# TomasDelaney/A-Deep-Reinforcement-Learning-Enabled-Soft-Exoskeleton-for-Parkinson-s-Patients

Measured on AMD Instinct MI355X. Metric: env steps/sec (batched exo sim) + TD7 grad-steps/sec at 1/2/4/8 MI355X, higher is better.
Workload: dtype f64 sim + bf16 TD7

## Files before the change

### a-deep-reinforcement-learning-enabled-soft-exoskeleton-for-parkinson-s-patients_amd/csrc/lap.hip

```cpp
#include <hip/hip_runtime.h>

#include <algorithm>
#include <cstdint>
#include <cstdlib>
#include <string>

#include "lap_chain.h"
#include "philox.h"
#include "exo_amd.h"

namespace {

constexpr int UPD_THREADS = 1024;

__device__ __forceinline__ float *stratum_tree(float *tree, int s, int cap) { return tree + (size_t)s * 2 * cap; }

constexpr int TOPN = 8192;
template <int NTOP = TOPN>
__device__ bool propagate_top(float *T, int cap, int levels, const int32_t *slot, int n, float *top) {
    int lv = 1;
    for (; lv <= levels && ((2 * cap) >> lv) > NTOP / 2; ++lv) {
        __syncthreads();
        for (int k = threadIdx.x; k < n; k += blockDim.x) {
            const int node = (cap + slot[k]) >> lv;
            T[node] = T[2 * node] + T[2 * node + 1];
        }
    }
    __syncthreads();
    if (lv > levels) return false;
    const int lim = min(NTOP, 2 * cap);
    if (blockDim.x == UPD_THREADS) {
        constexpr int PER = NTOP / UPD_THREADS;
        float v[PER];
#pragma unroll
        for (int j = 0; j < PER; ++j) {
            const int i = threadIdx.x + j * UPD_THREADS;
            v[j] = i < lim ? T[i] : 0.0f;
        }
#pragma unroll
        for (int j = 0; j < PER; ++j) {
            const int i = threadIdx.x + j * UPD_THREADS;
            if (i < lim) top[i] = v[j];
        }
    } else {
        for (int i = threadIdx.x; i < lim; i += blockDim.x) top[i] = T[i];
    }
    for (; lv <= levels; ++lv) {
        __syncthreads();
        for (int k = threadIdx.x; k < n; k += blockDim.x) {
            const int node = (cap + slot[k]) >> lv;
            top[node] = top[2 * node] + top[2 * node + 1];
        }
    }
    __syncthreads();
    const int wb = min(NTOP / 2, cap);
    for (int i = 1 + threadIdx.x; i < wb; i += blockDim.x) T[i] = top[i];
    __syncthreads();
    return true;
}
__device__ void propagate(float *T, int cap, int levels, const int32_t *slot, int n) {
    __shared__ float top[TOPN];
    propagate_top(T, cap, levels, slot, n, top);
}

__device__ void propagate_span(float *T, int cap, int levels, int capacity, int first, int count) {
    __shared__ float top[TOPN];
    if (count <= 0) return;
    int a0 = first, e0 = first + count, a1 = 0, e1 = 0;
    if (count >= capacity) {
        a0 = 0;
        e0 = capacity;
    } else if (e0 > capacity) {
        e1 = e0 - capacity;
        e0 = capacity;
    }
    int lv = 1;
    for (; lv <= levels && ((2 * cap) >> lv) > TOPN / 2; ++lv) {
        __syncthreads();
        const int lo0 = (cap + a0) >> lv, n0 = ((cap + e0 - 1) >> lv) - lo0 + 1;
        const int lo1 = (cap + a1) >> lv, n1 = e1 > a1 ? ((cap + e1 - 1) >> lv) - lo1 + 1 : 0;
        for (int k = threadIdx.x; k < n0 + n1; k += blockDim.x) {
            const int node = k < n0 ? lo0 + k : lo1 + k - n0;
            T[node] = T[2 * node] + T[2 * node + 1];
        }
    }
    __syncthreads();
    if (lv > levels) return;
    const int lim = min(TOPN, 2 * cap);
    for (int i = threadIdx.x; i < lim; i += blockDim.x) top[i] = T[i];
    for (; lv <= levels; ++lv) {
        __syncthreads();
        const int lo0 = (cap + a0) >> lv, n0 = ((cap + e0 - 1) >> lv) - lo0 + 1;
        const int lo1 = (cap + a1) >> lv, n1 = e1 > a1 ? ((cap + e1 - 1) >> lv) - lo1 + 1 : 0;
        for (int k = threadIdx.x; k < n0 + n1; k += blockDim.x) {
            const int node = k < n0 ? lo0 + k : lo1 + k - n0;
            top[node] = top[2 * node] + top[2 * node + 1];
        }
    }
    __syncthreads();
    const int wb = min(TOPN / 2, cap);
    for (int i = 1 + threadIdx.x; i < wb; i += blockDim.x) T[i] = top[i];
    __syncthreads();
}

constexpr int SPAN_LDS = 4096;
constexpr int SPAN_LEVELS = 32;
__device__ bool propagate_span_lds(float *T, int cap, int levels, int capacity, int first, int count,
                                   float *buf , float *edge ) {
    const int a = cap + first, e = cap + first + count - 1;
    if (count <= 0 || first + count > capacity || count > SPAN_LDS - 2 || levels >= SPAN_LEVELS) return false;
    const int t = threadIdx.x;
    if (t < 2 * levels) {
        const int lv = t >> 1, right = t & 1;
        const int lo = a >> lv, hi = e >> lv;
        if (!right && (lo & 1)) edge[t] = T[lo - 1];
        if (right && !(hi & 1)) edge[t] = T[hi + 1];
    }
    float *A = buf, *B = buf + SPAN_LDS;
    {
        const int base = a & ~1;
        for (int c = a + t; c <= e; c += blockDim.x) A[c - base] = T[c];
    }
    __syncthreads();
    if (t == 0) {
        if (a & 1) A[0] = edge[0];
        if (!(e & 1)) A[(e | 1) - (a & ~1)] = edge[1];
    }
    for (int lv = 1; lv <= levels; ++lv) {
        __syncthreads();
        const int lo = a >> lv, hi = e >> lv, cbase = (a >> (lv - 1)) & ~1, nbase = lo & ~1;
        for (int node = lo + t; node <= hi; node += blockDim.x) {
            const int c = 2 * node - cbase;
            const float v = A[c] + A[c + 1];
            T[node] = v;
            B[node - nbase] = v;
        }
        if (t == 0 && lv < levels) {
            if (lo & 1) B[0] = edge[2 * lv];
            if (!(hi & 1)) B[(hi | 1) - nbase] = edge[2 * lv + 1];
        }
        float *tmp = A;
        A = B;
        B = tmp;
    }
    __syncthreads();
    return true;
}

constexpr int ADD_CHUNK = 4096;
__global__ __launch_bounds__(UPD_THREADS) void lap_add_kernel(float *tree, const float *maxp, int cap, int levels,
                                                              int capacity, const int32_t *stratum,
                                                              const int32_t *slot, int n) {
    const int s = blockIdx.x;
    float *T = stratum_tree(tree, s, cap);
    __shared__ int32_t mine[ADD_CHUNK];
    __shared__ int count;
    const float p = *maxp;
    for (int base = 0; base < n; base += ADD_CHUNK) {
        if (threadIdx.x == 0) count = 0;
        __syncthreads();
        const int end = min(n, base + ADD_CHUNK);
        for (int k = base + threadIdx.x; k < end; k += blockDim.x) {
            if (stratum[k] != s) continue;
            const int sl = slot[k];
            if (sl < 0 || sl >= capacity) continue;
            T[cap + sl] = p;
            mine[atomicAdd(&count, 1)] = sl;
        }
        __syncthreads();
        propagate(T, cap, levels, mine, count);
    }
}

constexpr int MAXLV = 24;
template <class At>
__device__ __forceinline__ float prefix_sum(At at, int cap, int levels, int sz) {
    if (sz >= cap) return at(1);
    float v[MAXLV];
#pragma unroll
    for (int j = 0; j < MAXLV; ++j) {
        v[j] = 0.0f;
        if (j < levels) {
            const int lv = levels - 1 - j;
            const float x = at(2 * ((1 << j) | (sz >> (lv + 1))));
            v[j] = ((sz >> lv) & 1) ? x : 0.0f;
        }
    }
    float acc = 0.0f;
#pragma unroll
    for (int j = 0; j < MAXLV; ++j)
        if (j < levels) acc += v[j];
    return acc;
}
__device__ __forceinline__ float prefix_total(const float *T, int cap, int levels, int sz) {
    return prefix_sum([T](int n) { return T[n]; }, cap, levels, sz);
}

__device__ __forceinline__ float sel4(int r, float a, float b, float c, float d) {
    return r == 0 ? a : r == 1 ? b : r == 2 ? c : d;
}

template <class At>
__device__ __forceinline__ int descend_from(At at, float val, int node, int lv, int levels) {
    while (lv < levels) {
        const int k = levels - lv >= 3 ? 3 : levels - lv;
        const int n1 = 2 * node, n2 = 4 * node, n3 = 8 * node;
        const float a0 = at(n1), a1 = at(n1 + 1);
        float b0 = 0.f, b1 = 0.f, b2 = 0.f, b3 = 0.f, c0 = 0.f, c1 = 0.f, c2 = 0.f, c3 = 0.f;
        float c4 = 0.f, c5 = 0.f, c6 = 0.f, c7 = 0.f;
        if (k >= 2) b0 = at(n2), b1 = at(n2 + 1), b2 = at(n2 + 2), b3 = at(n2 + 3);
        if (k >= 3) {
            c0 = at(n3), c1 = at(n3 + 1), c2 = at(n3 + 2), c3 = at(n3 + 3);
            c4 = at(n3 + 4), c5 = at(n3 + 5), c6 = at(n3 + 6), c7 = at(n3 + 7);
        }
        int r;
        if (val <= a0 || a1 <= 0.0f) {
            r = 0;
        } else {
            val -= a0;
            r = 1;
        }
        if (k >= 2) {
            const float l = r ? b2 : b0, rt = r ? b3 : b1;
            if (val <= l || rt <= 0.0f) {
                r = 2 * r;
            } else {
                val -= l;
                r = 2 * r + 1;
            }
            if (k >= 3) {
                const float l3 = sel4(r, c0, c2, c4, c6), r3 = sel4(r, c1, c3, c5, c7);
                if (val <= l3 || r3 <= 0.0f) {
                    r = 2 * r;
                } else {
                    val -= l3;
                    r = 2 * r + 1;
                }
            }
        }
        node = (node << k) + r;
        lv += k;
    }
    return node;
}

__global__ void lap_sample_kernel(const float *tree, int cap, int levels, const float *u, const int32_t *size,
                                  int batch, int32_t *idx) {
    const int s = blockIdx.y;
    const int b = blockIdx.x * blockDim.x + threadIdx.x;
    if (b >= batch) return;
    const float *T = tree + (size_t)s * 2 * cap;
    const int sz = size[s];
    const float val = u[(size_t)s * batch + b] * prefix_total(T, cap, levels, sz);
    const int node = descend_from([T](int n) { return T[n]; }, val, 1, 0, levels);
    int i = node - cap;
    if (i >= sz) i = sz > 0 ? sz - 1 : 0;
    idx[(size_t)s * batch + b] = i;
}

__global__ __launch_bounds__(UPD_THREADS) void lap_update_kernel(float *tree, float *maxp, int cap, int levels,
                                                                 const int32_t *idx, const float *prio,
                                                                 int batch) {
    const int s = blockIdx.x;
    float *T = stratum_tree(tree, s, cap);
    const int32_t *I = idx + (size_t)s * batch;
    const float *P = prio + (size_t)s * batch;
    __shared__ float red[UPD_THREADS / 64];
    __shared__ int32_t li[UPD_THREADS];
    float mx = 0.0f;
    for (int b0 = 0; b0 < batch; b0 += UPD_THREADS) {
        const int nb = min(UPD_THREADS, batch - b0);
        __syncthreads();
        if ((int)threadIdx.x < nb) li[threadIdx.x] = I[b0 + threadIdx.x];
        __syncthreads();
        const int b = b0 + threadIdx.x;
        if (b < batch) {
            const int me = li[threadIdx.x];
            bool last = true;
            for (int k = threadIdx.x + 1; k < nb; ++k) last &= (li[k] != me);
            for (int b2 = b0 + nb; b2 < batch; ++b2) last &= (I[b2] != me);
            if (last) T[cap + me] = P[b];
            mx = fmaxf(mx, P[b]);
        }
    }
    for (int o = 32; o > 0; o >>= 1) mx = fmaxf(mx, __shfl_xor(mx, o, 64));
    if ((threadIdx.x & 63) == 0) red[threadIdx.x >> 6] = mx;
    propagate(T, cap, levels, I, batch);
    if (threadIdx.x == 0) {
        for (int w = 1; w < (int)(blockDim.x >> 6); ++w) mx = fmaxf(mx, red[w]);
        atomicMax(reinterpret_cast<int *>(maxp), __float_as_int(mx));
    }
}

__global__ void lap_reset_max_kernel(const float *tree, float *maxp, int cap, int n_strata) {
    __shared__ float red[16];
    float mx = 0.0f;
    const size_t total = (size_t)n_strata * cap;
    for (size_t k = (size_t)blockIdx.x * blockDim.x + threadIdx.x; k < total; k += (size_t)gridDim.x * blockDim.x) {
        const size_t s = k / cap, i = k % cap;
        mx = fmaxf(mx, tree[s * 2 * cap + cap + i]);
    }
    for (int o = 32; o > 0; o >>= 1) mx = fmaxf(mx, __shfl_xor(mx, o, 64));
    if ((threadIdx.x & 63) == 0) red[threadIdx.x >> 6] = mx;
    __syncthreads();
    if (threadIdx.x == 0) {
        for (int w = 1; w < (int)(blockDim.x >> 6); ++w) mx = fmaxf(mx, red[w]);
        atomicMax(reinterpret_cast<int *>(maxp), __float_as_int(mx));
    }
}

__global__ void lap_totals_kernel(const float *tree, int cap, int n_strata, float *out) {
    const int s = blockIdx.x * blockDim.x + threadIdx.x;
    if (s < n_strata) out[s] = tree[(size_t)s * 2 * cap + 1];
}

__global__ void lap_init_kernel(float *maxp) { *maxp = 1.0f; }


constexpr int STORE_CHUNK = UPD_THREADS * 4;

template <int RANK_RPT>
__global__ __launch_bounds__(UPD_THREADS) void lap_store_rank_kernel(float *tree, const float *maxp, int cap,
                                                                     int levels, int capacity, int32_t *ring_ptr,
                                                                     int32_t *ring_size, const int32_t *strata,
                                                                     const uint8_t *active, int n, int32_t *row_of) {
    const int s = blockIdx.x, t = threadIdx.x, lane = t & 63, wv = t >> 6;
    float *T = stratum_tree(tree, s, cap);
    __shared__ int wsum[UPD_THREADS / 64];
    __shared__ int chunk_total;
    const float p = *maxp;
    const int ptr0 = ring_ptr[s];
    const int row0 = s * (capacity + 1);
    int offset = 0;
    for (int base = 0; base < n; base += RANK_RPT * UPD_THREADS) {
        int st[RANK_RPT], cnt = 0;
        bool f[RANK_RPT];
#pragma unroll
        for (int k = 0; k < RANK_RPT; ++k) {
            const int i = base + RANK_RPT * t + k;
            st[k] = i < n ? strata[i] : -1;
            f[k] = i < n && (!active || active[i]);
        }
#pragma unroll
        for (int k = 0; k < RANK_RPT; ++k) {
            f[k] = f[k] && st[k] == s;
            cnt += f[k];
        }
        int incl = cnt;
#pragma unroll
        for (int o = 1; o < 64; o <<= 1) {
            const int v = __shfl_up(incl, o, 64);
            if (lane >= o) incl += v;
        }
        if (lane == 63) wsum[wv] = incl;
        __syncthreads();
        if (t == 0) {
            int acc = 0;
            for (int k = 0; k < UPD_THREADS / 64; ++k) {
                const int v = wsum[k];
                wsum[k] = acc;
                acc += v;
            }
            chunk_total = acc;
        }
        __syncthreads();
        int rank = offset + wsum[wv] + incl - cnt;
#pragma unroll
        for (int k = 0; k < RANK_RPT; ++k) {
            const int i = base + RANK_RPT * t + k;
            if (i >= n) continue;
            if (s == 0 && (st[k] < 0 || st[k] >= (int)gridDim.x)) row_of[i] = -1;
            if (st[k] != s) continue;
            if (f[k]) {
                const int slot = (ptr0 + rank) % capacity;
                row_of[i] = row0 + slot;
                T[cap + slot] = p;
                ++rank;
            } else {
                row_of[i] = row0 + capacity;
            }
        }
        const int total = chunk_total;
        __syncthreads();
        offset += total;
    }
    propagate_span(T, cap, levels, capacity, ptr0, offset);
    if (t == 0) {
        ring_ptr[s] = (ptr0 + offset) % capacity;
        ring_size[s] = min(ring_size[s] + offset, capacity);
    }
}

__device__ __forceinline__ long long mult_below(long long x, int E) { return (x + E - 1) / E; }

__global__ __launch_bounds__(UPD_THREADS) void lap_store_ref_slots_kernel(int capacity, int E, long long *ref,
                                                                          int32_t *ring_size,
                                                                          const int32_t *strata,
                                                                          const uint8_t *active, int n,
                                                                          int32_t *rank_row, int32_t *slot_of,
                                                                          int32_t *row_of) {
    const int t = threadIdx.x, lane = t & 63, wv = t >> 6;
    __shared__ int wsum[UPD_THREADS / 64];
    __shared__ int chunk_total;
    const long long ptr0 = ref[0], count0 = ref[1], size0 = ref[2];
    const long long m0 = mult_below(count0, E);
    int offset = 0;
    for (int base = 0; base < n; base += STORE_CHUNK) {
        int f[4], cnt = 0;
#pragma unroll
        for (int k = 0; k < 4; ++k) {
            const int i = base + 4 * t + k;
            f[k] = (i < n && strata[i] >= 0 && strata[i] < E && (!active || active[i])) ? 1 : 0;
            cnt += f[k];
        }
        int incl = cnt;
#pragma unroll
        for (int o = 1; o < 64; o <<= 1) {
            const int v = __shfl_up(incl, o, 64);
            if (lane >= o) incl += v;
        }
        if (lane == 63) wsum[wv] = incl;
        __syncthreads();
        if (t == 0) {
            int acc = 0;
            for (int k = 0; k < UPD_THREADS / 64; ++k) {
                const int v = wsum[k];
                wsum[k] = acc;
                acc += v;
            }
            chunk_total = acc;
        }
        __syncthreads();
        int rank = offset + wsum[wv] + incl - cnt;
#pragma unroll
        for (int k = 0; k < 4; ++k) {
            const int i = base + 4 * t + k;
            if (i >= n) continue;
            if (f[k]) {
                rank_row[rank] = strata[i];
                row_of[i] = rank;
                ++rank;
            } else {
                row_of[i] = -1;
                slot_of[i] = -1;
            }
        }
        offset += chunk_total;
        __syncthreads();
    }
    __threadfence_block();
    __syncthreads();
    const int n_act = offset;
    for (int i = t; i < n; i += blockDim.x) {
        const int r = row_of[i];
        if (r < 0) continue;
        const long long mr = mult_below(count0 + r, E);
        const int s = strata[i];
        bool win = true;
        const long long qend = mr * E - count0;
        const int qmax = (int)min((long long)min(r + E, n_act) - 1, qend);
        for (int q = r + 1; q <= qmax; ++q) win &= rank_row[q] != s;
        long long v = ptr0 + (mr - m0);
        if (v >= capacity) v -= capacity;
        if (v >= capacity) v %= capacity;
        const int slot = (int)v;
        slot_of[i] = win ? slot : -1;
        row_of[i] = win ? s * (capacity + 1) + slot : -1;
    }
    __syncthreads();
    const long long adv = mult_below(count0 + n_act, E) - m0;
    const long long size = min(size0 + adv, (long long)capacity);
    for (int s = t; s < E; s += blockDim.x) ring_size[s] = (int32_t)size;
    if (t == 0) {
        ref[0] = (ptr0 + adv) % capacity;
        ref[1] = count0 + n_act;
        ref[2] = size;
    }
}

__device__ __forceinline__ float4 ld4(const float *p) { return *reinterpret_cast<const float4 *>(p); }
__device__ __forceinline__ void st4(float *p, float4 v) { *reinterpret_cast<float4 *>(p) = v; }

template <bool VEC>
__device__ __forceinline__ void copy_rows(const lap_storage_desc &st, const float *state, const float *action,
                                          const float *next_state, const float *reward, const uint8_t *done,
                                          float action_scale, const int32_t *ri, const int32_t *sl, int s,
                                          int capacity, int j0, int step, int m, int t, int nt) {
    const int sd = st.state_dim, ad = st.action_dim;
    const int sdv = VEC ? sd / 4 : sd;
    const int per = 2 * sdv + ad + 2;
    const int nrows = j0 < m ? (m - j0 + step - 1) / step : 0;
    const int items = nrows * per;
    constexpr int U = 4;
    for (int it0 = t; it0 < items; it0 += U * nt) {
        float4 v[U];
        long dst[U];
        int kind[U];
#pragma unroll
        for (int u = 0; u < U; ++u) {
            const int it = it0 + u * nt;
            kind[u] = -1;
            if (it >= items) continue;
            const int q = it / per, c = it - q * per, j = j0 + q * step;
            const int slot = sl[j];
            if (slot < 0) continue;
            const long r = (long)s * (capacity + 1) + slot;
            const long i = ri[j];
            if (c < 2 * sdv) {
                const bool nx = c >= sdv;
                const int e = nx ? c - sdv : c;
                const float *src = (nx ? next_state : state) + i * sd;
                if (VEC) {
                    v[u] = ld4(src + 4 * e);
                    dst[u] = r * sd + 4 * e;
                } else {
                    v[u].x = src[e];
                    dst[u] = r * sd + e;
                }
                kind[u] = nx ? 1 : 0;
            } else if (c < 2 * sdv + ad) {
                const int e = c - 2 * sdv;
                v[u].x = action[i * ad + e] / action_scale;
                dst[u] = r * ad + e;
                kind[u] = 2;
            } else if (c == 2 * sdv + ad) {
                v[u].x = reward[i];
                dst[u] = r;
                kind[u] = 3;
            } else {
                v[u].x = 1.0f - (done[i] ? 1.0f : 0.0f);
                dst[u] = r;
                kind[u] = 4;
            }
        }
#pragma unroll
        for (int u = 0; u < U; ++u) {
            switch (kind[u]) {
            case 0:
                if (VEC) st4(st.state + dst[u], v[u]); else st.state[dst[u]] = v[u].x;
                break;
            case 1:
                if (VEC) st4(st.next_state + dst[u], v[u]); else st.next_state[dst[u]] = v[u].x;
                break;
            case 2: st.action[dst[u]] = v[u].x; break;
            case 3: st.reward[dst[u]] = v[u].x; break;
            case 4: st.not_done[dst[u]] = v[u].x; break;
            default: break;
            }
        }
    }
}

constexpr int STORE_FUSED_MAX = 8192;

template <bool VEC>
__global__ __launch_bounds__(UPD_THREADS) void lap_store_fused_kernel(
    float *tree, const float *maxp, int cap, int levels, int capacity, int32_t *ring_ptr, int32_t *ring_size,
    const int32_t *strata, const uint8_t *active, int n, int32_t *row_of, lap_storage_desc st, const float *state,
    const float *action, const float *next_state, const float *reward, const uint8_t *done, float action_scale) {
    constexpr int RPT = 4;
    const int s = blockIdx.x, t = threadIdx.x, lane = t & 63, wv = t >> 6;
    float *T = stratum_tree(tree, s, cap);
    __shared__ int wsum[UPD_THREADS / 64];
    __shared__ int chunk_total;
    __shared__ int32_t ri[STORE_FUSED_MAX];
    const float p = *maxp;
    const int ptr0 = ring_ptr[s];
    const int row0 = s * (capacity + 1);
    int offset = 0;
    for (int base = 0; base < n; base += RPT * UPD_THREADS) {
        int stk[RPT], cnt = 0;
        bool f[RPT];
#pragma unroll
        for (int k = 0; k < RPT; ++k) {
            const int i = base + RPT * t + k;
            stk[k] = i < n ? strata[i] : -1;
            f[k] = i < n && (!active || active[i]) && stk[k] == s;
            cnt += f[k];
        }
        int incl = cnt;
#pragma unroll
        for (int o = 1; o < 64; o <<= 1) {
            const int v = __shfl_up(incl, o, 64);
            if (lane >= o) incl += v;
        }
        if (lane == 63) wsum[wv] = incl;
        __syncthreads();
        if (t == 0) {
            int acc = 0;
            for (int k = 0; k < UPD_THREADS / 64; ++k) {
                const int v = wsum[k];
                wsum[k] = acc;
                acc += v;
            }
            chunk_total = acc;
        }
        __syncthreads();
        int rank = offset + wsum[wv] + incl - cnt;
#pragma unroll
        for (int k = 0; k < RPT; ++k) {
            const int i = base + RPT * t + k;
            if (i >= n) continue;
            if (s == 0 && (stk[k] < 0 || stk[k] >= (int)gridDim.x)) row_of[i] = -1;
            if (stk[k] != s) continue;
            if (f[k]) {
                const int slot = (ptr0 + rank) % capacity;
                row_of[i] = row0 + slot;
                T[cap + slot] = p;
                ri[rank] = i;
                ++rank;
            } else {
                row_of[i] = row0 + capacity;
            }
        }
        const int total = chunk_total;
        __syncthreads();
        offset += total;
    }
    {
        const int sd = st.state_dim, ad = st.action_dim;
        const int sdv = VEC ? sd / 4 : sd;
        const int per = 2 * sdv + ad + 2;
        const int items = offset * per;
        constexpr int U = 8;
        for (int it0 = t; it0 < items; it0 += U * UPD_THREADS) {
            float4 v[U];
            long dst[U];
            int kind[U];
#pragma unroll
            for (int u = 0; u < U; ++u) {
                const int it = it0 + u * UPD_THREADS;
                kind[u] = -1;
                if (it >= items) continue;
                const int q = it / per, c = it - q * per;
                const long r = (long)row0 + (ptr0 + q) % capacity;
                const long i = ri[q];
                if (c < 2 * sdv) {
                    const bool nx = c >= sdv;
                    const int e = nx ? c - sdv : c;
                    const float *src = (nx ? next_state : state) + i * sd;
                    if (VEC) {
                        v[u] = ld4(src + 4 * e);
                        dst[u] = r * sd + 4 * e;
                    } else {
                        v[u].x = src[e];
                        dst[u] = r * sd + e;
                    }
                    kind[u] = nx ? 1 : 0;
                } else if (c < 2 * sdv + ad) {
                    const int e = c - 2 * sdv;
                    v[u].x = action[i * ad + e] / action_scale;
                    dst[u] = r * ad + e;
                    kind[u] = 2;
                } else if (c == 2 * sdv + ad) {
                    v[u].x = reward[i];
                    dst[u] = r;
                    kind[u] = 3;
                } else {
                    v[u].x = 1.0f - (done[i] ? 1.0f : 0.0f);
                    dst[u] = r;
                    kind[u] = 4;
                }
            }
#pragma unroll
            for (int u = 0; u < U; ++u) {
                switch (kind[u]) {
                case 0:
                    if (VEC) st4(st.state + dst[u], v[u]); else st.state[dst[u]] = v[u].x;
                    break;
                case 1:
                    if (VEC) st4(st.next_state + dst[u], v[u]); else st.next_state[dst[u]] = v[u].x;
                    break;
                case 2: st.action[dst[u]] = v[u].x; break;
                case 3: st.reward[dst[u]] = v[u].x; break;
                case 4: st.not_done[dst[u]] = v[u].x; break;
                default: break;
                }
            }
        }
    }
    propagate_span(T, cap, levels, capacity, ptr0, offset);
    if (t == 0) {
        ring_ptr[s] = (ptr0 + offset) % capacity;
        ring_size[s] = min(ring_size[s] + offset, capacity);
    }
}

struct MaskAdvance {
    const uint8_t *table;
    int rows;
    long long *k;
    uint8_t *active;
    int32_t *count;
// ... 317 lines not shown
    const long long i = (long long)blockIdx.x * blockDim.x + threadIdx.x;
    if (i >= entries) return;
    const int c = plan[i];
    if (c < 0) return;
    const long long ptr0 = ref[0], count0 = ref[1];
    const long long m0 = mult_below(count0, E), mr = mult_below(count0 + c, E);
    const long long qend = min(mr * E - count0, total - 1);
    const int s = add_s[c];
    bool win = true;
    for (long long q = c + 1; q <= qend; ++q) win &= add_s[q] != s;
    long long v = ptr0 + (mr - m0);
    if (v >= capacity) v -= capacity;
    if (v >= capacity) v %= capacity;
    plan[i] = win ? (int32_t)v : -1;
}

__global__ __launch_bounds__(256) void lap_ref_step_kernel(lap_storage_desc st, const int32_t *plan, int rows, int n,
                                                           long long *kk, int par, long long *k_dev,
                                                           const int32_t *strata, int capacity, const float *state,
                                                           const float *action, const float *next_state,
                                                           const float *reward, const uint8_t *done,
                                                           float action_scale, const uint8_t *table,
                                                           uint8_t *active, int32_t *count,
                                                           const int32_t *counts_table, double *score) {
    const long long k = kk[par];
    const long long k1 = k + 1 < rows ? k + 1 : rows - 1;
    const int e = blockIdx.x * 4 + (threadIdx.x >> 6), lane = threadIdx.x & 63;
    if (blockIdx.x == 0 && threadIdx.x == 0) {
        kk[par ^ 1] = k1;
        if (k_dev) *k_dev = k1;
        if (count) *count = counts_table[k1];
    }
    if (e >= n) return;
    const int slot = k < rows ? plan[(size_t)k * n + e] : -1;
    if (slot >= 0) {
        const long r = (long)strata[e] * (capacity + 1) + slot;
        const int sd = st.state_dim, ad = st.action_dim;
        for (int q = lane; q < sd; q += 64) {
            st.state[r * sd + q] = state[(long)e * sd + q];
            st.next_state[r * sd + q] = next_state[(long)e * sd + q];
        }
        for (int q = lane; q < ad; q += 64) st.action[r * ad + q] = action[(long)e * ad + q] / action_scale;
        if (lane == 0) {
            st.reward[r] = reward[e];
            st.not_done[r] = 1.0f - (done[e] ? 1.0f : 0.0f);
        }
    }
    if (lane == 0) {
        if (score) score[e] += active[e] ? (double)reward[e] : 0.0;
        active[e] = table[(size_t)k1 * n + e];
    }
}

__global__ __launch_bounds__(256) void lap_ref_commit_leaves_kernel(const int32_t *plan, long long entries, int n,
                                                                    const int32_t *strata, float *tree, int cap,
                                                                    const float *maxp) {
    const long long i = (long long)blockIdx.x * blockDim.x + threadIdx.x;
    if (i >= entries) return;
    const int slot = plan[i];
    if (slot < 0) return;
    stratum_tree(tree, strata[i % n], cap)[cap + slot] = *maxp;
}

__global__ __launch_bounds__(UPD_THREADS) void lap_ref_commit_tree_kernel(float *tree, int cap, int levels,
                                                                          int capacity, const long long *ref,
                                                                          long long total, int E) {
    const long long ptr0 = ref[0], count0 = ref[1];
    if (total <= 0) return;
    const long long last = mult_below(count0 + total - 1, E) - mult_below(count0, E);
    propagate_span(stratum_tree(tree, blockIdx.x, cap), cap, levels, capacity, (int)ptr0,
                   (int)min(last + 1, (long long)capacity));
}

__global__ void lap_ref_commit_ref_kernel(long long *ref, long long total, int E, int capacity, int32_t *ring_size) {
    const long long ptr0 = ref[0], count0 = ref[1], size0 = ref[2];
    const long long adv = mult_below(count0 + total, E) - mult_below(count0, E);
    const long long size = min(size0 + adv, (long long)capacity);
    for (int s = 0; s < E; ++s) ring_size[s] = (int32_t)size;
    ref[0] = (ptr0 + adv) % capacity;
    ref[1] = count0 + total;
    ref[2] = size;
}

constexpr int GATHER_DRAWS = 16;
__global__ __launch_bounds__(256) void lap_gather_kernel(lap_storage_desc st, int capacity, const int32_t *idx,
                                                         int batch, int total, float *o_state, float *o_action,
                                                         float *o_next, float *o_reward, float *o_not_done) {
    const int sd = st.state_dim, ad = st.action_dim;
    const bool v4 = (sd & 3) == 0 && ((reinterpret_cast<uintptr_t>(st.state) | reinterpret_cast<uintptr_t>(st.next_state) |
                                       reinterpret_cast<uintptr_t>(o_state) | reinterpret_cast<uintptr_t>(o_next)) & 15) == 0;
    const int sv = v4 ? sd / 4 : sd, per = 2 * sv + ad + 2;
    const int d0 = blockIdx.x * GATHER_DRAWS;
    const int nd = min(GATHER_DRAWS, total - d0);
    const int items = nd * per;
    constexpr int GU = 4;
    for (int it0 = threadIdx.x; it0 < items; it0 += GU * 256) {
        float4 v[GU];
        float *dst[GU];
        bool wide[GU];
#pragma unroll
        for (int u = 0; u < GU; ++u) {
            const int it = it0 + u * 256;
            dst[u] = nullptr;
            wide[u] = false;
            if (it >= items) continue;
            const int q = it / per, c = it - q * per;
            const long d = d0 + q;
            const long row = (long)(d / batch) * (capacity + 1) + idx[d];
            if (c < 2 * sv) {
                const bool nx = c >= sv;
                const int e = nx ? c - sv : c;
                const float *src = (nx ? st.next_state : st.state) + row * sd;
                float *o = (nx ? o_next : o_state) + d * sd;
                if (v4) {
                    v[u] = ld4(src + 4 * e);
                    dst[u] = o + 4 * e;
                    wide[u] = true;
                } else {
                    v[u].x = src[e];
                    dst[u] = o + e;
                }
            } else if (c < 2 * sv + ad) {
                const int e = c - 2 * sv;
                v[u].x = st.action[row * ad + e];
                dst[u] = o_action + d * ad + e;
            } else if (c == 2 * sv + ad) {
                v[u].x = st.reward[row];
                dst[u] = o_reward + d;
            } else {
                v[u].x = st.not_done[row];
                dst[u] = o_not_done + d;
            }
        }
#pragma unroll
        for (int u = 0; u < GU; ++u) {
            if (!dst[u]) continue;
            if (wide[u]) st4(dst[u], v[u]);
            else *dst[u] = v[u].x;
        }
    }
}

struct TdPrio {
    const float *td;
    float alpha, minp;
    float *out;
};

__device__ __forceinline__ void gather_picked(const lap_storage_desc &st, int capacity, int s, int batch,
                                              const int32_t *pick, float *o_state, float *o_action, float *o_next,
                                              float *o_reward, float *o_not_done) {
    const int sd = st.state_dim, ad = st.action_dim;
    const bool v4 = (sd & 3) == 0 && ((reinterpret_cast<uintptr_t>(st.state) | reinterpret_cast<uintptr_t>(st.next_state) |
                                       reinterpret_cast<uintptr_t>(o_state) | reinterpret_cast<uintptr_t>(o_next)) & 15) == 0;
    const int sv = v4 ? sd / 4 : sd, per = 2 * sv + ad + 2;
    const int items = min(batch, UPD_THREADS) * per;
    constexpr int GU = 8;
    for (int it0 = threadIdx.x; it0 < items; it0 += GU * UPD_THREADS) {
        float4 v[GU];
        float *dst[GU];
        bool wide[GU];
#pragma unroll
        for (int u = 0; u < GU; ++u) {
            const int it = it0 + u * UPD_THREADS;
            dst[u] = nullptr;
            wide[u] = false;
            if (it >= items) continue;
            const int b = it / per, c = it - b * per;
            const long d = (long)s * batch + b;
            const long row = (long)s * (capacity + 1) + pick[b];
            if (c < 2 * sv) {
                const bool nx = c >= sv;
                const int e = nx ? c - sv : c;
                const float *src = (nx ? st.next_state : st.state) + row * sd;
                float *o = (nx ? o_next : o_state) + d * sd;
                if (v4) {
                    v[u] = ld4(src + 4 * e);
                    dst[u] = o + 4 * e;
                    wide[u] = true;
                } else {
                    v[u].x = src[e];
                    dst[u] = o + e;
                }
            } else if (c < 2 * sv + ad) {
                const int e = c - 2 * sv;
                v[u].x = st.action[row * ad + e];
                dst[u] = o_action + d * ad + e;
            } else if (c == 2 * sv + ad) {
                v[u].x = st.reward[row];
                dst[u] = o_reward + d;
            } else {
                v[u].x = st.not_done[row];
                dst[u] = o_not_done + d;
            }
        }
#pragma unroll
        for (int u = 0; u < GU; ++u) {
            if (!dst[u]) continue;
            if (wide[u]) st4(dst[u], v[u]);
            else *dst[u] = v[u].x;
        }
    }
}

__global__ __launch_bounds__(UPD_THREADS) void lap_update_sample_kernel(float *tree, float *maxp, int cap, int levels,
                                                                        int capacity, const int32_t *idx_in,
                                                                        const float *prio, int batch,
                                                                        const int32_t *size, lap_storage_desc st,
                                                                        SampleRng rng, int32_t *idx_out,
                                                                        float *o_state, float *o_action, float *o_next,
                                                                        float *o_reward, float *o_not_done,
                                                                        TdPrio tp, bool gather) {
    const int s = blockIdx.x;
    float *T = stratum_tree(tree, s, cap);
    const int32_t *I = idx_in + (size_t)s * batch;
    const float *P = prio + (size_t)s * batch;
    __shared__ float red[UPD_THREADS / 64];
    __shared__ int32_t li[UPD_THREADS];
    __shared__ float top[TOPN_US];
    __shared__ int32_t pick[UPD_THREADS];
    const unsigned long long call = *rng.counter;
    float mx = 0.0f;
    for (int b0 = 0; b0 < batch; b0 += UPD_THREADS) {
        const int nb = min(UPD_THREADS, batch - b0);
        __syncthreads();
        if ((int)threadIdx.x < nb) li[threadIdx.x] = I[b0 + threadIdx.x];
        __syncthreads();
        const int b = b0 + threadIdx.x;
        if (b < batch) {
            const int me = li[threadIdx.x];
            bool last = true;
            for (int k = threadIdx.x + 1; k < nb; ++k) last &= (li[k] != me);
            for (int b2 = b0 + nb; b2 < batch; ++b2) last &= (I[b2] != me);
            float pb;
            if (tp.td) {
                const long d = (long)s * batch + b;
                pb = powf(fmaxf(fmaxf(tp.td[2 * d], tp.td[2 * d + 1]), tp.minp), tp.alpha);
                if (tp.out) tp.out[d] = pb;
            } else {
                pb = P[b];
            }
            if (last) T[cap + me] = pb;
            mx = fmaxf(mx, pb);
        }
    }
    for (int o = 32; o > 0; o >>= 1) mx = fmaxf(mx, __shfl_xor(mx, o, 64));
    if ((threadIdx.x & 63) == 0) red[threadIdx.x >> 6] = mx;
    const bool staged = propagate_top<TOPN_US>(T, cap, levels, I, batch, top);
    if (threadIdx.x == 0) {
        for (int w = 1; w < (int)(blockDim.x >> 6); ++w) mx = fmaxf(mx, red[w]);
        atomicMax(reinterpret_cast<int *>(maxp), __float_as_int(mx));
    }
    const int lim = staged ? min(TOPN_US, 2 * cap) : 0;
    auto node_at = [&](int node) { return node < lim ? top[node] : T[node]; };
    const int sz = size[s];
    const float tot = prefix_sum(node_at, cap, levels, sz);
    for (int b = threadIdx.x; b < batch; b += UPD_THREADS) {
        const int d = s * batch + b;
        uint32_t r[4];
        philox_block(rng.seed, rng.tag, call, (uint32_t)d, r);
        float val = u01_open_hi(r[0]) * tot;
        int node = 1, lv = 0;
        for (; lv < levels && 2 * node + 1 < lim; ++lv) {
            const float left = top[2 * node], right = top[2 * node + 1];
            if (val <= left || right <= 0.0f) {
                node = 2 * node;
            } else {
                val -= left;
                node = 2 * node + 1;
            }
        }
        node = descend_from([T](int n) { return T[n]; }, val, node, lv, levels);
        int i = node - cap;
        if (i >= sz) i = sz > 0 ? sz - 1 : 0;
        idx_out[d] = i;
        if (b < UPD_THREADS) pick[b] = i;
    }
    __syncthreads();
    if (!gather) {
        if (threadIdx.x == 0 && atomicAdd(rng.ticket, 1u) == gridDim.x - 1) {
            *rng.counter = call + 1ull;
            *rng.ticket = 0u;
        }
        return;
    }
    gather_picked(st, capacity, s, batch, pick, o_state, o_action, o_next, o_reward, o_not_done);
    __syncthreads();
    if (threadIdx.x == 0) {
        if (atomicAdd(rng.ticket, 1u) == gridDim.x - 1) {
            *rng.counter = call + 1ull;
            *rng.ticket = 0u;
        }
    }
}

constexpr int CHAIN_MAXB = 256;
constexpr int CHAIN_MAXG = 12;
constexpr int CHAIN_ROW = CHAIN_MAXB + 1;
constexpr int CHAIN_TOPLV = 12;
static_assert((2 << CHAIN_TOPLV) >= TOPN_US, "CHAIN_TOPLV: the staged top's levels");
constexpr int CHAIN_PAD = 0x40000000;
constexpr int CHAIN_RNG0 = 640;

__device__ __forceinline__ void lds_barrier() { asm volatile("s_waitcnt lgkmcnt(0)\n\ts_barrier" ::: "memory"); }

__global__ __launch_bounds__(UPD_THREADS) void lap_update_sample_chain_kernel(
    float *tree, float *maxp, int cap, int levels, int capacity, const int32_t *idx_in,
    const float *__restrict__ prio, int batch, const int32_t *__restrict__ size, lap_storage_desc st, SampleRng rng,
    int32_t *idx_out, float *o_state, float *o_action, float *o_next, float *o_reward, float *o_not_done, TdPrio tp,
    bool gather) {
    const int s = blockIdx.x, t = threadIdx.x;
    float *T = stratum_tree(tree, s, cap);
    __shared__ float red[UPD_THREADS / 64];
    __shared__ __attribute__((aligned(16))) int32_t li[CHAIN_MAXB + 4];
    __shared__ int32_t lsz;
    __shared__ float uni[CHAIN_MAXB];
    __shared__ int32_t later[CHAIN_MAXB];
    __shared__ int32_t partner[CHAIN_MAXG * CHAIN_ROW];
    __shared__ float chain[2][CHAIN_MAXB];
    __shared__ float lowval[CHAIN_MAXG];
    __shared__ float top[TOPN_US];
    __shared__ int32_t pick[CHAIN_MAXB];
    const int G = lap_chain::global_levels(levels, TOPN_US);
    const int lim = min(TOPN_US, 2 * cap);
    const bool draw = t < batch;
    const long d = (long)s * batch + (draw ? t : 0);
    const unsigned long long call = *rng.counter;
    const int sz = size[s];
    const int me = idx_in[d];
    const float *pp = tp.td ? tp.td + 2 * d : prio + d;
    const float p0 = pp[0], p1 = pp[tp.td ? 1 : 0];
    constexpr int PER = TOPN_US / UPD_THREADS;
    float stage[PER];
#pragma unroll
    for (int j = 0; j < PER; ++j) stage[j] = T[min(t + j * UPD_THREADS, lim - 1)];
    for (int i = t; i < G * CHAIN_ROW; i += UPD_THREADS) partner[i] = -1;
    if (t < CHAIN_MAXB + 4) li[t] = draw ? me : CHAIN_PAD;
    if (draw) later[t] = 0;
    if (t >= CHAIN_RNG0 && t < CHAIN_RNG0 + batch) {
        uint32_t r[4];
        philox_block(rng.seed, rng.tag, call, (uint32_t)(s * batch + t - CHAIN_RNG0), r);
        uni[t - CHAIN_RNG0] = u01_open_hi(r[0]);
    }
    const int szl = min(sz, cap - 1);
    const int leaf = t == batch ? szl : me;
    if (t == batch) lsz = szl;
    float sib[CHAIN_MAXG];
#pragma unroll
    for (int lv = 0; lv < CHAIN_MAXG; ++lv) sib[lv] = 0.0f;
    if (t <= batch) {
#pragma unroll
        for (int lv = 0; lv < CHAIN_MAXG; ++lv) sib[lv] = T[lap_chain::sibling_of(cap, leaf, min(lv, max(G - 1, 0)))];
    }
    lds_barrier();
    {
        int lp = 0;
        while (((batch + 1) << (lp + 1)) <= UPD_THREADS) ++lp;
        const int b = t >> lp, part = t & ((1 << lp) - 1);
        const int chunk = (((batch + 3) >> 2) + (1 << lp) - 1) >> lp;
        if (b <= batch) {
            const int mine = b < batch ? li[b] : lsz;
            const unsigned near = 1u << G;
            bool sup = false;
            for (int q = part * chunk; q < (part + 1) * chunk && 4 * q < batch; ++q) {
                const int4 o = *reinterpret_cast<const int4 *>(&li[4 * q]);
                const int other[4] = {o.x, o.y, o.z, o.w};
#pragma unroll
                for (int j = 0; j < 4; ++j) {
                    const int k = 4 * q + j;
                    if ((unsigned)(mine ^ other[j]) >= near) continue;
                    const int lv = lap_chain::partner_level(mine, other[j]);
                    if (lv < 0) sup |= b < batch && lap_chain::superseded_by(b, mine, k, other[j]);
                    else atomicMax(&partner[lv * CHAIN_ROW + b], k);
                }
            }
            if (sup) later[b] = 1;
        }
    }
    const float pb = !draw ? 0.0f : tp.td ? powf(fmaxf(fmaxf(p0, p1), tp.minp), tp.alpha) : p0;
    float mx = pb;
    for (int o = 32; o > 0; o >>= 1) mx = fmaxf(mx, __shfl_xor(mx, o, 64));
    if ((t & 63) == 0) red[t >> 6] = mx;
#pragma unroll
    for (int j = 0; j < PER; ++j) {
        const int i = t + j * UPD_THREADS;
        if (i < lim) top[i] = stage[j];
    }
    lds_barrier();
    const bool carry = draw && !later[t];
    if (draw && tp.td && tp.out) tp.out[d] = pb;
    float cur = pb;
    if (carry) {
        T[cap + me] = pb;
        chain[0][t] = pb;
    }
    if (t == batch) {
#pragma unroll
        for (int lv = 0; lv < CHAIN_MAXG; ++lv)
            if (lv < G && partner[lv * CHAIN_ROW + batch] < 0) lowval[lv] = sib[lv];
    }
#pragma unroll
    for (int lv = 0; lv < CHAIN_MAXG; ++lv) {
        if (lv < G) lds_barrier();
        if (lv < G && carry) {
            if (partner[lv * CHAIN_ROW + batch] == t) lowval[lv] = cur;
            const int node = lap_chain::node_of(cap, me, lv), k = partner[lv * CHAIN_ROW + t];
            cur = lap_chain::chain_step(node, cur, k >= 0 ? chain[lv & 1][k] : sib[lv]);
            T[node >> 1] = cur;
            chain[(lv + 1) & 1][t] = cur;
        }
    }
    if (carry) top[lap_chain::node_of(cap, me, G)] = cur;
    for (int lv = G + 1; lv <= levels; ++lv) {
        lds_barrier();
        if (draw) {
            const int node = lap_chain::node_of(cap, me, lv);
            top[node] = top[2 * node] + top[2 * node + 1];
        }
    }
    __syncthreads();
    const int wb = min(TOPN_US / 2, cap);
    for (int i = 1 + t; i < wb; i += UPD_THREADS) T[i] = top[i];
    if (t >= UPD_THREADS - 64) {
        float m = red[t & (UPD_THREADS / 64 - 1)];
        for (int o = UPD_THREADS / 128; o > 0; o >>= 1) m = fmaxf(m, __shfl_xor(m, o, 64));
        if (t == UPD_THREADS - 64) atomicMax(reinterpret_cast<int *>(maxp), __float_as_int(m));
    }
    if (draw) {
        const int ltop = levels - G;
        float tot;
        if (sz >= cap) {
            tot = top[1];
        } else {
            float x[CHAIN_TOPLV];
#pragma unroll
            for (int j = 0; j < CHAIN_TOPLV; ++j) {
                const int lv = levels - 1 - j;
                x[j] = j < ltop ? top[2 * ((1 << j) | (sz >> (lv + 1)))] : 0.0f;
            }
            tot = 0.0f;
#pragma unroll
            for (int j = 0; j < CHAIN_TOPLV; ++j)
                if (j < ltop) tot += ((sz >> (levels - 1 - j)) & 1) ? x[j] : 0.0f;
#pragma unroll
            for (int lv = CHAIN_MAXG - 1; lv >= 0; --lv) {
                if (lv >= G) continue;
                tot += ((sz >> lv) & 1) ? lowval[lv] : 0.0f;
            }
        }
        float val = uni[t] * tot;
        int node = 1;
        for (int lv = 0; lv < ltop; ++lv) {
            const float left = top[2 * node], right = top[2 * node + 1];
            if (val <= left || right <= 0.0f) {
                node = 2 * node;
            } else {
                val -= left;
                node = 2 * node + 1;
            }
        }
        node = descend_from([T](int n) { return T[n]; }, val, node, ltop, levels);
        int i = node - cap;
        if (i >= sz) i = sz > 0 ? sz - 1 : 0;
        idx_out[d] = i;
        pick[t] = i;
    }
    __syncthreads();
    if (gather) {
        gather_picked(st, capacity, s, batch, pick, o_state, o_action, o_next, o_reward, o_not_done);
        __syncthreads();
    }
    if (t == 0 && atomicAdd(rng.ticket, 1u) == gridDim.x - 1) {
        *rng.counter = call + 1ull;
        *rng.ticket = 0u;
    }
}

int rc(hipError_t e) { return e == hipSuccess ? EXO_OK : EXO_EDEVICE; }

int levels_of(const lap_tree_desc *t) {
    int lv = 0;
    while ((1 << lv) < t->cap) ++lv;
    return lv;
}

bool gather_split() {
    static const bool on = [] {
        const char *e = getenv("EXO_LAP_GATHER_SPLIT");
        return !(e && e[0] == '0');
    }();
    return on;
}

void launch_update_sample(const lap_tree_desc *t, const lap_storage_desc *st, const int32_t *idx_in, const float *prio,
                          int batch, SampleRng rng, int32_t *idx_out, float *o_state, float *o_action, float *o_next,
                          float *o_reward, float *o_not_done, TdPrio tp, bool gather, void *stream) {
    const char *e = getenv("EXO_LAP_CHAIN");
    const int levels = levels_of(t);
    const bool chain = !(e && e[0] == '0') && batch <= CHAIN_MAXB && levels >= 1 &&
                       lap_chain::global_levels(levels, TOPN_US) <= CHAIN_MAXG;
    if (chain)
        hipLaunchKernelGGL(lap_update_sample_chain_kernel, dim3(t->n_strata), dim3(UPD_THREADS), 0, (hipStream_t)stream,
                           t->tree, t->max_priority, t->cap, levels, t->capacity, idx_in, prio, batch, st->size, *st,
                           rng, idx_out, o_state, o_action, o_next, o_reward, o_not_done, tp, gather);
    else
        hipLaunchKernelGGL(lap_update_sample_kernel, dim3(t->n_strata), dim3(UPD_THREADS), 0, (hipStream_t)stream,
                           t->tree, t->max_priority, t->cap, levels, t->capacity, idx_in, prio, batch, st->size, *st,
                           rng, idx_out, o_state, o_action, o_next, o_reward, o_not_done, tp, gather);
}

int gather_after(const lap_tree_desc *t, const lap_storage_desc *st, int batch, const int32_t *idx, float *o_state,
                 float *o_action, float *o_next, float *o_reward, float *o_not_done, void *stream) {
    if (hipGetLastError() != hipSuccess) return EXO_EDEVICE;
    if (!gather_split()) return EXO_OK;
    const int total = t->n_strata * batch;
    hipLaunchKernelGGL(lap_gather_kernel, dim3((total + GATHER_DRAWS - 1) / GATHER_DRAWS), dim3(256), 0,
                       (hipStream_t)stream, *st, t->capacity, idx, batch, total, o_state, o_action, o_next, o_reward,
                       o_not_done);
    return hipGetLastError() == hipSuccess ? EXO_OK : EXO_EDEVICE;
}

bool valid(const lap_tree_desc *t) {
    return t && t->tree && t->max_priority && t->n_strata > 0 && t->capacity > 0 && t->cap >= t->capacity &&
           (t->cap & (t->cap - 1)) == 0 && t->cap <= (1 << MAXLV);
}

}

extern "C" {

int32_t lap_tree_floats(int32_t n_strata, int32_t capacity) {
    int cap = 1;
    while (cap < capacity) cap <<= 1;
    return n_strata * 2 * cap;
}

int lap_init(const lap_tree_desc *t, void *stream) {
    if (!valid(t)) return EXO_EINVAL;
    hipError_t e = hipMemsetAsync(t->tree, 0, (size_t)t->n_strata * 2 * t->cap * sizeof(float), (hipStream_t)stream);
    if (e != hipSuccess) return EXO_EDEVICE;
    hipLaunchKernelGGL(lap_init_kernel, dim3(1), dim3(1), 0, (hipStream_t)stream, t->max_priority);
    return rc(hipGetLastError());
}

int lap_add(const lap_tree_desc *t, const int32_t *stratum, const int32_t *slot, int32_t n, void *stream) {
    if (!valid(t) || !stratum || !slot || n < 0) return EXO_EINVAL;
    if (n == 0) return EXO_OK;
    hipLaunchKernelGGL(lap_add_kernel, dim3(t->n_strata), dim3(UPD_THREADS), 0, (hipStream_t)stream, t->tree,
                       t->max_priority, t->cap, levels_of(t), t->capacity, stratum, slot, n);
    return rc(hipGetLastError());
}

int lap_sample(const lap_tree_desc *t, const float *u, const int32_t *size, int32_t batch, int32_t *idx, void *stream) {
    if (!valid(t) || !u || !size || !idx || batch <= 0) return EXO_EINVAL;
    const int th = 128;
    hipLaunchKernelGGL(lap_sample_kernel, dim3((batch + th - 1) / th, t->n_strata), dim3(th), 0, (hipStream_t)stream,
                       t->tree, t->cap, levels_of(t), u, size, batch, idx);
    return rc(hipGetLastError());
}

int lap_update(const lap_tree_desc *t, const int32_t *idx, const float *prio, int32_t batch, void *stream) {
    if (!valid(t) || !idx || !prio || batch <= 0) return EXO_EINVAL;
    hipLaunchKernelGGL(lap_update_kernel, dim3(t->n_strata), dim3(UPD_THREADS), 0, (hipStream_t)stream, t->tree,
                       t->max_priority, t->cap, levels_of(t), idx, prio, batch);
    return rc(hipGetLastError());
}

int lap_reset_max(const lap_tree_desc *t, void *stream) {
    if (!valid(t)) return EXO_EINVAL;
    hipError_t e = hipMemsetAsync(t->max_priority, 0, sizeof(float), (hipStream_t)stream);
    if (e != hipSuccess) return EXO_EDEVICE;
    hipLaunchKernelGGL(lap_reset_max_kernel, dim3(256), dim3(1024), 0, (hipStream_t)stream, t->tree, t->max_priority,
                       t->cap, t->n_strata);
    return rc(hipGetLastError());
}

int lap_totals(const lap_tree_desc *t, float *out, void *stream) {
    if (!valid(t) || !out) return EXO_EINVAL;
    hipLaunchKernelGGL(lap_totals_kernel, dim3((t->n_strata + 63) / 64), dim3(64), 0, (hipStream_t)stream, t->tree,
                       t->cap, t->n_strata, out);
    return rc(hipGetLastError());
}

int lap_store_batch(const lap_tree_desc *t, const lap_storage_desc *st, const float *state, const float *action,
                    const float *next_state, const float *reward, const uint8_t *done, const int32_t *strata,
                    const uint8_t *active, float action_scale, int32_t n, int32_t *row_ws, void *stream) {
    if (!valid(t) || !st || !st->state || !st->action || !st->next_state || !st->reward || !st->not_done ||
        !st->ptr || !st->size || st->state_dim <= 0 || st->action_dim <= 0 || !state || !action || !next_state ||
        !reward || !done || !strata || !row_ws || n < 0 || action_scale == 0.0f)
        return EXO_EINVAL;
    if (n == 0) return EXO_OK;
    const char *fused_var = getenv("EXO_LAP_STORE_FUSED");
    const bool fused_env = fused_var && fused_var[0] == '1';
    if (fused_env && n <= STORE_FUSED_MAX && n <= t->capacity) {
        const bool vec = (st->state_dim & 3) == 0 &&
                         ((reinterpret_cast<uintptr_t>(state) | reinterpret_cast<uintptr_t>(next_state) |
                           reinterpret_cast<uintptr_t>(st->state) | reinterpret_cast<uintptr_t>(st->next_state)) &
                          15) == 0;
        if (vec)
            hipLaunchKernelGGL(lap_store_fused_kernel<true>, dim3(t->n_strata), dim3(UPD_THREADS), 0,
                               (hipStream_t)stream, t->tree, t->max_priority, t->cap, levels_of(t), t->capacity,
                               st->ptr, st->size, strata, active, n, row_ws, *st, state, action, next_state, reward,
                               done, action_scale);
        else
            hipLaunchKernelGGL(lap_store_fused_kernel<false>, dim3(t->n_strata), dim3(UPD_THREADS), 0,
                               (hipStream_t)stream, t->tree, t->max_priority, t->cap, levels_of(t), t->capacity,
                               st->ptr, st->size, strata, active, n, row_ws, *st, state, action, next_state, reward,
                               done, action_scale);
        return rc(hipGetLastError());
    }
    if (n > 4 * STORE_CHUNK)
        hipLaunchKernelGGL(lap_store_rank_kernel<16>, dim3(t->n_strata), dim3(UPD_THREADS), 0, (hipStream_t)stream,
                           t->tree, t->max_priority, t->cap, levels_of(t), t->capacity, st->ptr, st->size, strata,
                           active, n, row_ws);
    else
        hipLaunchKernelGGL(lap_store_rank_kernel<4>, dim3(t->n_strata), dim3(UPD_THREADS), 0, (hipStream_t)stream,
                           t->tree, t->max_priority, t->cap, levels_of(t), t->capacity, st->ptr, st->size, strata,
                           active, n, row_ws);
    if (hipGetLastError() != hipSuccess) return EXO_EDEVICE;
    hipLaunchKernelGGL(lap_store_copy_kernel, dim3((n + 3) / 4), dim3(256), 0, (hipStream_t)stream, *st, state,
                       action, next_state, reward, done, action_scale, n, row_ws);
    return rc(hipGetLastError());
}

int lap_store_batch_ref(const lap_tree_desc *t, const lap_storage_desc *st, int64_t *ref_dev, const float *state,
                        const float *action, const float *next_state, const float *reward, const uint8_t *done,
                        const int32_t *strata, const uint8_t *active, float action_scale, int32_t n,
                        int32_t *ws_dev, void *stream) {
    if (!valid(t) || !st || !st->state || !st->action || !st->next_state || !st->reward || !st->not_done ||
        !st->size || st->state_dim <= 0 || st->action_dim <= 0 || !ref_dev || !state || !action || !next_state ||
        !reward || !done || !strata || !ws_dev || n < 0 || action_scale == 0.0f)
        return EXO_EINVAL;
    if (n == 0) return EXO_OK;
    int32_t *rank_row = ws_dev, *slot_of = ws_dev + n, *row_of = ws_dev + 2 * n;
    hipLaunchKernelGGL(lap_store_ref_slots_kernel, dim3(1), dim3(UPD_THREADS), 0, (hipStream_t)stream, t->capacity,
                       t->n_strata, (long long *)ref_dev, st->size, strata, active, n, rank_row, slot_of, row_of);
    if (hipGetLastError() != hipSuccess) return EXO_EDEVICE;
    hipLaunchKernelGGL(lap_add_kernel, dim3(t->n_strata), dim3(UPD_THREADS), 0, (hipStream_t)stream, t->tree,
                       t->max_priority, t->cap, levels_of(t), t->capacity, strata, slot_of, n);
    if (hipGetLastError() != hipSuccess) return EXO_EDEVICE;
    hipLaunchKernelGGL(lap_store_copy_kernel, dim3((n + 3) / 4), dim3(256), 0, (hipStream_t)stream, *st, state,
                       action, next_state, reward, done, action_scale, n, row_of);
    return rc(hipGetLastError());
}

static int store_ref_fused(const lap_tree_desc *t, const lap_storage_desc *st, int64_t *ref_dev,
                           const float *state, const float *action, const float *next_state, const float *reward,
                           const uint8_t *done, const int32_t *strata, const uint8_t *active, float action_scale,
                           int32_t n, uint32_t *ticket_dev, const MaskAdvance &adv, void *stream) {
    if (!valid(t) || !st || !st->state || !st->action || !st->next_state || !st->reward || !st->not_done ||
        !st->size || st->state_dim <= 0 || st->action_dim <= 0 || !ref_dev || !state || !action || !next_state ||
        !reward || !done || !strata || !ticket_dev || n < 0 || action_scale == 0.0f)
        return EXO_EINVAL;
    if (n == 0) return EXO_OK;
    const int E = t->n_strata;
    const int K = 1 + std::max(1, std::min(15, (n + E * 64 - 1) / (E * 64)));
    auto al16 = [](const void *p) { return ((uintptr_t)p & 15u) == 0; };
    const bool vec = st->state_dim % 4 == 0 && al16(state) && al16(next_state) && al16(st->state) &&
                     al16(st->next_state);
    if (vec)
        hipLaunchKernelGGL(lap_store_ref_fused_kernel<true>, dim3(E, K), dim3(UPD_THREADS), 0, (hipStream_t)stream,
                           t->tree, t->max_priority, t->cap, levels_of(t), t->capacity, E, (long long *)ref_dev,
                           st->size, *st, state, action, next_state, reward, done, action_scale, strata, active, n,
                           ticket_dev, adv);
    else
        hipLaunchKernelGGL(lap_store_ref_fused_kernel<false>, dim3(E, K), dim3(UPD_THREADS), 0, (hipStream_t)stream,
                           t->tree, t->max_priority, t->cap, levels_of(t), t->capacity, E, (long long *)ref_dev,
                           st->size, *st, state, action, next_state, reward, done, action_scale, strata, active, n,
                           ticket_dev, adv);
    return rc(hipGetLastError());
}

int lap_store_batch_ref_fused(const lap_tree_desc *t, const lap_storage_desc *st, int64_t *ref_dev,
                              const float *state, const float *action, const float *next_state, const float *reward,
                              const uint8_t *done, const int32_t *strata, const uint8_t *active, float action_scale,
                              int32_t n, uint32_t *ticket_dev, void *stream) {
    return store_ref_fused(t, st, ref_dev, state, action, next_state, reward, done, strata, active, action_scale, n,
                           ticket_dev, MaskAdvance{}, stream);
}

int lap_store_batch_ref_fused_adv(const lap_tree_desc *t, const lap_storage_desc *st, int64_t *ref_dev,
                                  const float *state, const float *action, const float *next_state,
                                  const float *reward, const uint8_t *done, const int32_t *strata, uint8_t *active,
                                  float action_scale, int32_t n, uint32_t *ticket_dev, const uint8_t *table,
                                  int32_t rows, int64_t *k_dev, int32_t *count_dev, double *score_dev, void *stream) {
    if (!table || rows <= 0 || !k_dev || !active) return EXO_EINVAL;
    return store_ref_fused(t, st, ref_dev, state, action, next_state, reward, done, strata, active, action_scale, n,
                           ticket_dev, MaskAdvance{table, rows, (long long *)k_dev, active, count_dev, score_dev},
                           stream);
}

int lap_sample_gather(const lap_tree_desc *t, const lap_storage_desc *st, const float *u, int32_t batch,
                      int32_t *idx, float *out_state, float *out_action, float *out_next_state, float *out_reward,
                      float *out_not_done, void *stream) {
    if (!valid(t) || !st || !st->size || !u || !idx || batch <= 0 || !out_state || !out_action ||
        !out_next_state || !out_reward || !out_not_done)
        return EXO_EINVAL;
    const int total = t->n_strata * batch;
    hipLaunchKernelGGL(lap_sample_gather_kernel, dim3((total + 3) / 4), dim3(256), 0, (hipStream_t)stream, t->tree,
                       t->cap, levels_of(t), t->capacity, u, st->size, batch, total, idx, *st, out_state, out_action,
                       out_next_state, out_reward, out_not_done, SampleRng{0, 0, nullptr, nullptr});
    return rc(hipGetLastError());
}

int lap_update_sample_rng(const lap_tree_desc *t, const lap_storage_desc *st, const int32_t *idx_in,
                          const float *prio, int32_t batch, uint64_t seed, uint32_t tag, unsigned long long *counter,
                          uint32_t *ticket, int32_t *idx_out, float *out_state, float *out_action,
                          float *out_next_state, float *out_reward, float *out_not_done, void *stream) {
    if (!valid(t) || !st || !st->size || !idx_in || !prio || !counter || !ticket || !idx_out || batch <= 0 ||
        batch > UPD_THREADS || !out_state || !out_action || !out_next_state || !out_reward || !out_not_done)
        return EXO_EINVAL;
    launch_update_sample(t, st, idx_in, prio, batch, SampleRng{seed, tag, counter, ticket}, idx_out, out_state,
                         out_action, out_next_state, out_reward, out_not_done, TdPrio{nullptr, 0.f, 0.f, nullptr},
                         !gather_split(), stream);
    return gather_after(t, st, batch, idx_out, out_state, out_action, out_next_state, out_reward, out_not_done, stream);
}

int lap_update_sample_idx(const lap_tree_desc *t, const lap_storage_desc *st, const int32_t *idx_in,
                          const float *prio, int32_t batch, uint64_t seed, uint32_t tag, unsigned long long *counter,
                          uint32_t *ticket, int32_t *idx_out, void *stream) {
    if (!valid(t) || !st || !st->size || !idx_in || !prio || !counter || !ticket || !idx_out || batch <= 0 ||
        batch > UPD_THREADS)
        return EXO_EINVAL;
    launch_update_sample(t, st, idx_in, prio, batch, SampleRng{seed, tag, counter, ticket}, idx_out, nullptr, nullptr,
                         nullptr, nullptr, nullptr, TdPrio{nullptr, 0.f, 0.f, nullptr}, false, stream);
    return rc(hipGetLastError());
}

int lap_gather_rows(const lap_tree_desc *t, const lap_storage_desc *st, int32_t batch, const int32_t *idx,
                    float *out_state, float *out_action, float *out_next_state, float *out_reward,
                    float *out_not_done, void *stream) {
    if (!valid(t) || !st || !st->state || !st->action || !st->next_state || !st->reward || !st->not_done || !idx ||
        batch <= 0 || !out_state || !out_action || !out_next_state || !out_reward || !out_not_done)
        return EXO_EINVAL;
    const int total = t->n_strata * batch;
    hipLaunchKernelGGL(lap_gather_kernel, dim3((total + GATHER_DRAWS - 1) / GATHER_DRAWS), dim3(256), 0,
                       (hipStream_t)stream, *st, t->capacity, idx, batch, total, out_state, out_action,
                       out_next_state, out_reward, out_not_done);
    return rc(hipGetLastError());
}

int lap_update_sample_td(const lap_tree_desc *t, const lap_storage_desc *st, const int32_t *idx_in, const float *td,
                         float alpha, float min_priority, float *prio_out, int32_t batch, uint64_t seed, uint32_t tag,
                         unsigned long long *counter, uint32_t *ticket, int32_t *idx_out, float *out_state,
                         float *out_action, float *out_next_state, float *out_reward, float *out_not_done,
                         void *stream) {
    if (!valid(t) || !st || !st->size || !idx_in || !td || !counter || !ticket || !idx_out || batch <= 0 ||
        batch > UPD_THREADS || !out_state || !out_action || !out_next_state || !out_reward || !out_not_done)
        return EXO_EINVAL;
    launch_update_sample(t, st, idx_in, nullptr, batch, SampleRng{seed, tag, counter, ticket}, idx_out, out_state,
                         out_action, out_next_state, out_reward, out_not_done,
                         TdPrio{td, alpha, min_priority, prio_out}, !gather_split(), stream);
    return gather_after(t, st, batch, idx_out, out_state, out_action, out_next_state, out_reward, out_not_done, stream);
}

int lap_sample_gather_rng(const lap_tree_desc *t, const lap_storage_desc *st, uint64_t seed, uint32_t tag,
                          unsigned long long *counter, uint32_t *ticket, int32_t batch, int32_t *idx,
                          float *out_state, float *out_action, float *out_next_state, float *out_reward,
                          float *out_not_done, void *stream) {
    if (!valid(t) || !st || !st->size || !counter || !ticket || !idx || batch <= 0 || !out_state || !out_action ||
        !out_next_state || !out_reward || !out_not_done)
        return EXO_EINVAL;
    const int total = t->n_strata * batch;
    hipLaunchKernelGGL(lap_sample_gather_kernel, dim3((total + 3) / 4), dim3(256), 0, (hipStream_t)stream, t->tree,
                       t->cap, levels_of(t), t->capacity, nullptr, st->size, batch, total, idx, *st, out_state,
                       out_action, out_next_state, out_reward, out_not_done, SampleRng{seed, tag, counter, ticket});
    return rc(hipGetLastError());
}


int lap_ref_plan(const lap_tree_desc *t, const int64_t *ref_dev, const uint8_t *table_dev, int32_t rows, int32_t n,
                 const int32_t *strata_dev, const int64_t *offs_dev, int64_t total, int32_t *add_ws_dev,
                 int32_t *plan_dev, void *stream) {
    if (!valid(t) || !ref_dev || !table_dev || rows <= 0 || n <= 0 || !strata_dev || !offs_dev || total < 0 ||
        (total > 0 && !add_ws_dev) || !plan_dev)
        return EXO_EINVAL;
    hipStream_t s = (hipStream_t)stream;
    hipLaunchKernelGGL(lap_ref_plan_scan_kernel, dim3(rows), dim3(UPD_THREADS), 0, s, table_dev, n, strata_dev,
                       t->n_strata, (const long long *)offs_dev, add_ws_dev, plan_dev);
    if (hipGetLastError() != hipSuccess) return EXO_EDEVICE;
    const long long entries = (long long)rows * n;
    hipLaunchKernelGGL(lap_ref_plan_slots_kernel, dim3((unsigned)((entries + 255) / 256)), dim3(256), 0, s, plan_dev,
                       entries, add_ws_dev, (long long)total, (const long long *)ref_dev, t->n_strata, t->capacity);
    return rc(hipGetLastError());
}

int lap_ref_step(const lap_tree_desc *t, const lap_storage_desc *st, const int32_t *plan_dev, int32_t rows,
                 int32_t n, int64_t *kk_dev, int32_t par, int64_t *k_dev, const int32_t *strata_dev,
                 const float *state, const float *action, const float *next_state, const float *reward,
                 const uint8_t *done, float action_scale, const uint8_t *table_dev, uint8_t *active_dev,
                 int32_t *count_dev, const int32_t *counts_table_dev, double *score_dev, void *stream) {
    if (!valid(t) || !st || !st->state || !st->action || !st->next_state || !st->reward || !st->not_done ||
        !plan_dev || rows <= 0 || n <= 0 || !kk_dev || (par != 0 && par != 1) || !strata_dev || !state || !action ||
        !next_state || !reward || !done || action_scale == 0.0f || !table_dev || !active_dev ||
        (count_dev && !counts_table_dev))
        return EXO_EINVAL;
    hipLaunchKernelGGL(lap_ref_step_kernel, dim3((n + 3) / 4), dim3(256), 0, (hipStream_t)stream, *st, plan_dev,
                       rows, n, (long long *)kk_dev, par, (long long *)k_dev, strata_dev, t->capacity, state, action,
                       next_state, reward, done, action_scale, table_dev, active_dev, count_dev, counts_table_dev,
                       score_dev);
    return rc(hipGetLastError());
}

int lap_ref_commit(const lap_tree_desc *t, const lap_storage_desc *st, int64_t *ref_dev, const int32_t *plan_dev,
                   int32_t rows, int32_t n, const int32_t *strata_dev, int64_t total, void *stream) {
    if (!valid(t) || !st || !st->size || !ref_dev || !plan_dev || rows <= 0 || n <= 0 || !strata_dev || total < 0)
        return EXO_EINVAL;
    hipStream_t s = (hipStream_t)stream;
    const long long entries = (long long)rows * n;
    hipLaunchKernelGGL(lap_ref_commit_leaves_kernel, dim3((unsigned)((entries + 255) / 256)), dim3(256), 0, s,
                       plan_dev, entries, n, strata_dev, t->tree, t->cap, t->max_priority);
    hipLaunchKernelGGL(lap_ref_commit_tree_kernel, dim3(t->n_strata), dim3(UPD_THREADS), 0, s, t->tree, t->cap,
                       levels_of(t), t->capacity, (const long long *)ref_dev, (long long)total, t->n_strata);
    hipLaunchKernelGGL(lap_ref_commit_ref_kernel, dim3(1), dim3(1), 0, s, (long long *)ref_dev, (long long)total,
                       t->n_strata, t->capacity, st->size);
    return rc(hipGetLastError());
}

}
```

### a-deep-reinforcement-learning-enabled-soft-exoskeleton-for-parkinson-s-patients_amd/exo_amd/_native.py

```python
import ctypes
import os
import subprocess

import torch

HERE = os.path.dirname(os.path.abspath(__file__))
PKG_ROOT = os.path.dirname(HERE)
LIB_PATH = os.path.join(HERE, "_lib", os.environ.get("EXO_AMD_LIB", "libexo_amd.so"))
CSRC = os.path.join(PKG_ROOT, "csrc")

EXO_OK = 0
ERRORS = {-22: "EINVAL", -12: "ENOMEM", -5: "EDEVICE", -34: "ERANGE"}

c_int32, c_double, c_void_p, c_uint64 = ctypes.c_int32, ctypes.c_double, ctypes.c_void_p, ctypes.c_uint64
c_long = ctypes.c_long
P = ctypes.POINTER


class LapTreeDesc(ctypes.Structure):
    _fields_ = [("tree", c_void_p), ("max_priority", c_void_p), ("n_strata", c_int32), ("capacity", c_int32),
                ("cap", c_int32)]


class LapStorageDesc(ctypes.Structure):
    _fields_ = [("state", c_void_p), ("action", c_void_p), ("next_state", c_void_p), ("reward", c_void_p),
                ("not_done", c_void_p), ("state_dim", c_int32), ("action_dim", c_int32), ("ptr", c_void_p),
                ("size", c_void_p)]


class ExoEnvConfig(ctypes.Structure):
    _fields_ = [("motion", c_int32), ("tremor_sequence", c_int32 * 7),
                ("tremor_amplitude_range", c_double * 2), ("first_harmonics_interval", c_double * 2),
                ("second_harmonics_interval", c_double * 2), ("max_force_shoulder", c_double),
                ("max_force_elbow", c_double), ("dr_actuator_end_pos_shift", c_double),
                ("dr_actuator_range", c_double), ("matrix_noise_fraction", c_double)]


class ExoMbParams(ctypes.Structure):
    _fields_ = [(n, c_double) for n in ("gravity", "kp", "kd", "motor_impulse", "passive_impulse", "limit_impulse",
                                        "erp", "lin_damp", "ang_damp", "max_vel")] + [("iters", c_int32)]


class TD7FLin(ctypes.Structure):
    _fields_ = [("wf", c_void_p), ("wb", c_void_p), ("b", c_void_p), ("n_out", c_int32), ("n_in", c_int32),
                ("ksf", c_int32), ("ksb", c_int32), ("w", c_void_p), ("ldw", ctypes.c_int64)]


class TD7FPackJob(ctypes.Structure):
    _fields_ = [("w", c_void_p), ("ld", ctypes.c_int64), ("n_out", c_int32), ("n_in", c_int32), ("wf", c_void_p),
                ("wb", c_void_p), ("ksf", c_int32), ("ntf", c_int32), ("ksb", c_int32), ("ntb", c_int32)]


class TD7FNoise(ctypes.Structure):
    _fields_ = [("seed", c_uint64), ("tag", ctypes.c_uint32), ("pad0", ctypes.c_uint32), ("counter", c_void_p),
                ("ticket", c_void_p), ("sigma", c_void_p), ("sigma_dec", ctypes.c_float), ("clip", ctypes.c_float),
                ("scale", ctypes.c_float), ("pad1", c_int32), ("z", c_void_p),
                ("dec_count", c_void_p)]


class TD7FNoiseRow(ctypes.Structure):
    _fields_ = [("seed", c_uint64), ("tag", ctypes.c_uint32), ("pad0", ctypes.c_uint32), ("counter", c_void_p),
                ("sigma", c_void_p), ("sigma_dec", ctypes.c_float), ("clip", ctypes.c_float)]


class TD7FXT(ctypes.Structure):
    _fields_ = [("x", c_void_p), ("dp", c_void_p), ("part", c_void_p)]


class TD7FActorBufs(ctypes.Structure):
    _fields_ = [("act_out", c_void_p), ("zsa_out", c_void_p), ("h0", c_void_p), ("mean0", c_void_p),
                ("ya", c_void_p * 2), ("yz", c_void_p * 2), ("yc", c_void_p * 2), ("da", c_void_p),
                ("dzsa", c_void_p)]


class TD7FWgJob(ctypes.Structure):
    _fields_ = [("dp", c_void_p), ("x", c_void_p), ("part", c_void_p), ("dw", c_void_p), ("db", c_void_p),
                ("n", c_int32), ("k", c_int32), ("row_tiles", c_int32)]


class TD7FWgAdam(ctypes.Structure):
    _fields_ = [("opt", c_int32), ("w_off", ctypes.c_int64), ("b_off", ctypes.c_int64), ("wf", c_void_p),
                ("wb", c_void_p), ("ksf", c_int32), ("ksb", c_int32)]


EXPORTS = {
    "exo_create": (c_int32, [P(ExoEnvConfig), c_int32, P(c_double), P(c_int32), c_int32, c_int32, c_uint64, c_int32,
                             P(c_void_p)]),
    "exo_reset": (c_int32, [c_void_p, c_void_p, c_void_p, c_void_p]),
    "exo_reset_from_draws": (c_int32, [c_void_p, P(c_int32), c_int32, P(c_double), c_void_p, c_void_p]),
    "exo_step": (c_int32, [c_void_p] * 8),
    "exo_num_envs": (c_int32, [c_void_p]),
    "exo_episode_length": (c_int32, [c_void_p, c_int32, P(c_int32)]),
    "exo_tremor_host": (c_int32, [c_void_p, c_int32, P(c_double)]),
    "exo_original_joint_angles_host": (c_int32, [c_void_p, c_int32, P(c_double)]),
    "exo_episode_host": (c_int32, [c_void_p, c_int32, P(c_double), P(c_double), P(c_double), P(c_double),
                                   P(c_double)]),
    "exo_get_state_host": (c_int32, [c_void_p, c_int32, P(c_double)]),
    "exo_set_state_host": (c_int32, [c_void_p, c_int32, P(c_double)]),
    "exo_set_seed": (c_int32, [c_void_p, c_uint64]),
    "exo_restart": (c_int32, [c_void_p, c_uint64, c_void_p]),
    "exo_set_step_variant": (c_int32, [c_void_p, c_int32]),
    "exo_set_step_budget": (c_int32, [c_void_p, c_int32]),
    "exo_step_carry": (c_int32, [c_void_p] * 9),
    "exo_budget_advance": (c_int32, [c_void_p] * 6),
    "exo_episode_advance": (c_int32, [c_void_p] * 7),
    "exo_reset_mask": (c_int32, [c_void_p] * 4),
    "exo_multibody_default_params": (None, [P(ExoMbParams)]),
    "exo_set_physics": (c_int32, [c_void_p, c_int32, P(ExoMbParams)]),
    "exo_multibody_advance": (c_int32, [c_void_p, c_void_p, c_void_p, c_void_p]),
    "exo_get_multibody_state_host": (c_int32, [c_void_p, c_int32, P(c_double), P(c_double)]),
    "exo_set_multibody_state_host": (c_int32, [c_void_p, c_int32, P(c_double), P(c_double)]),
    "exo_last_error": (ctypes.c_char_p, [c_void_p]),
    "exo_destroy": (None, [c_void_p]),
    "exo_tremor_metrics": (c_int32, [c_void_p, c_void_p, c_void_p, c_double, c_double, c_double, c_int32, c_void_p,
                                     c_void_p, c_void_p]),
    "exo_set_tremor_model": (c_int32, [c_void_p, c_void_p, c_int32]),
    "exo_set_step_clock": (c_int32, [c_void_p, c_void_p, c_void_p]),
    "exo_active_advance": (c_int32, [c_void_p, c_int32, c_int32, c_void_p, c_void_p, c_void_p, c_void_p]),
    "exo_active_advance_score": (c_int32, [c_void_p, c_int32, c_int32, c_void_p, c_void_p, c_void_p, c_void_p, c_void_p,
                                           c_void_p]),
    "exo_eval_metrics": (c_int32, [c_void_p, c_void_p, c_void_p, c_double, c_double, c_void_p, c_void_p]),
    "lap_tree_floats": (c_int32, [c_int32, c_int32]),
    "lap_init": (c_int32, [c_void_p, c_void_p]),
    "lap_add": (c_int32, [c_void_p, c_void_p, c_void_p, c_int32, c_void_p]),
    "lap_sample": (c_int32, [c_void_p, c_void_p, c_void_p, c_int32, c_void_p, c_void_p]),
    "lap_update": (c_int32, [c_void_p, c_void_p, c_void_p, c_int32, c_void_p]),
    "lap_reset_max": (c_int32, [c_void_p, c_void_p]),
    "lap_totals": (c_int32, [c_void_p, c_void_p, c_void_p]),
    "exo_stream_ballast": (c_int32, [c_int32]),
    "td7_dense_set_xl": (c_int32, [c_int32]),
    "exo_graph_branch_bound": (c_int32, [c_void_p, c_void_p]),
    "lap_store_batch": (c_int32, [c_void_p, c_void_p, c_void_p, c_void_p, c_void_p, c_void_p, c_void_p, c_void_p,
                                  c_void_p, ctypes.c_float, c_int32, c_void_p, c_void_p]),
    "lap_store_batch_ref": (c_int32, [c_void_p, c_void_p, c_void_p, c_void_p, c_void_p, c_void_p, c_void_p,
                                      c_void_p, c_void_p, c_void_p, ctypes.c_float, c_int32, c_void_p, c_void_p]),
    "lap_store_batch_ref_fused": (c_int32, [c_void_p, c_void_p, c_void_p, c_void_p, c_void_p, c_void_p, c_void_p,
                                            c_void_p, c_void_p, c_void_p, ctypes.c_float, c_int32, c_void_p,
                                            c_void_p]),
    "lap_store_batch_ref_fused_adv": (c_int32, [c_void_p] * 10 + [ctypes.c_float, c_int32, c_void_p, c_void_p,
                                                                 c_int32, c_void_p, c_void_p, c_void_p, c_void_p]),
    "lap_ref_plan": (c_int32, [c_void_p, c_void_p, c_void_p, c_int32, c_int32, c_void_p, c_void_p, ctypes.c_int64,
                               c_void_p, c_void_p, c_void_p]),
    "lap_ref_step": (c_int32, [c_void_p, c_void_p, c_void_p, c_int32, c_int32, c_void_p, c_int32, c_void_p, c_void_p]
                     + [c_void_p] * 5 + [ctypes.c_float, c_void_p, c_void_p, c_void_p, c_void_p, c_void_p, c_void_p]),
    "lap_ref_commit": (c_int32, [c_void_p, c_void_p, c_void_p, c_void_p, c_int32, c_int32, c_void_p, ctypes.c_int64,
                                 c_void_p]),
    "lap_update_sample_rng": (c_int32, [c_void_p, c_void_p, c_void_p, c_void_p, c_int32, ctypes.c_uint64,
                                        ctypes.c_uint32, c_void_p, c_void_p, c_void_p, c_void_p, c_void_p, c_void_p,
                                        c_void_p, c_void_p, c_void_p]),
    "lap_update_sample_idx": (c_int32, [c_void_p, c_void_p, c_void_p, c_void_p, c_int32, ctypes.c_uint64,
                                        ctypes.c_uint32, c_void_p, c_void_p, c_void_p, c_void_p]),
    "lap_gather_rows": (c_int32, [c_void_p, c_void_p, c_int32, c_void_p, c_void_p, c_void_p, c_void_p, c_void_p,
                                  c_void_p, c_void_p]),
    "lap_update_sample_td": (c_int32, [c_void_p, c_void_p, c_void_p, c_void_p, ctypes.c_float, ctypes.c_float,
                                       c_void_p, c_int32, ctypes.c_uint64, ctypes.c_uint32, c_void_p, c_void_p,
                                       c_void_p, c_void_p, c_void_p, c_void_p, c_void_p, c_void_p, c_void_p]),
    "lap_sample_gather_rng": (c_int32, [c_void_p, c_void_p, ctypes.c_uint64, ctypes.c_uint32, c_void_p, c_void_p,
                                        c_int32, c_void_p, c_void_p, c_void_p, c_void_p, c_void_p, c_void_p,
                                        c_void_p]),
    "lap_sample_gather": (c_int32, [c_void_p, c_void_p, c_void_p, c_int32, c_void_p, c_void_p, c_void_p, c_void_p,
                                    c_void_p, c_void_p, c_void_p]),
    "td7_adam_step": (c_int32, [c_void_p, c_void_p, c_void_p, c_void_p, c_void_p, c_void_p, ctypes.c_int64,
                                ctypes.c_float, ctypes.c_float, ctypes.c_float, ctypes.c_float, ctypes.c_float,
                                ctypes.c_float, c_void_p]),
    "td7_q_target": (c_int32, [c_void_p, c_long, c_long, c_void_p, c_void_p, ctypes.c_float, c_void_p, c_void_p,
                               c_void_p, c_void_p, c_void_p, c_int32, c_void_p]),
    "td7_critic_loss": (c_int32, [c_void_p, c_long, c_long, c_void_p, c_void_p, c_void_p, c_void_p, ctypes.c_float,
                                  ctypes.c_float, c_int32, c_void_p]),
    "td7_critic_loss_strided": (c_int32, [c_void_p, c_long, c_long, c_void_p, c_void_p, c_void_p, c_void_p, c_long,
                                          c_long, ctypes.c_float, ctypes.c_float, c_int32, c_void_p]),
    "td7_noisy_action": (c_int32, [c_void_p, c_void_p, c_void_p, ctypes.c_float, ctypes.c_float, ctypes.c_float,
                                   c_void_p, c_int32, c_void_p]),
    "td7_mse_fwd": (c_int32, [c_void_p, c_void_p, ctypes.c_int64, c_void_p, c_void_p, c_void_p]),
    "td7_mse_bwd": (c_int32, [c_void_p, c_void_p, c_void_p, ctypes.c_int64, c_void_p, c_void_p]),
    "td7_avgl1norm_fwd": (c_int32, [c_void_p, c_void_p, c_void_p, c_int32, c_int32, ctypes.c_float, c_void_p]),
    "td7_avgl1norm_fwd_h": (c_int32, [c_void_p, c_void_p, c_void_p, c_int32, c_int32, ctypes.c_float, c_int32,
                                      c_void_p]),
    "td7_avgl1norm_bwd": (c_int32, [c_void_p, c_void_p, c_void_p, c_void_p, c_int32, c_int32, ctypes.c_float,
                                    c_void_p]),
    "td7_dense_fwd": (c_int32, [c_void_p, c_long, c_long, c_void_p, c_void_p, c_void_p, c_long, c_long,
                                c_int32, c_int32, c_int32, c_int32, c_int32, c_void_p]),
    "td7_dense_bwd_data": (c_int32, [c_void_p, c_long, c_long, c_void_p, c_long, c_long, c_void_p, c_void_p,
                                     c_long, c_long, c_int32, c_int32, c_int32, c_int32, c_int32, c_int32,
                                     c_void_p]),
    "td7_dense_bwd_data_cols": (c_int32, [c_void_p, c_long, c_long, c_void_p, c_long, c_long, c_void_p, c_void_p,
                                          c_long, c_long, c_int32, c_int32, c_int32, c_int32, c_int32, c_int32, c_int32,
                                          c_int32, c_void_p]),
    "td7_dense_fwd_cat": (c_int32, [c_int32, c_void_p, c_void_p, c_void_p, c_void_p, c_void_p, c_void_p, c_void_p,
                                    c_long, c_long, c_int32, c_int32, c_int32, c_int32, c_void_p]),
    "td7_dense_fwd_w16": (c_int32, [c_void_p, c_long, c_long, c_void_p, c_void_p, c_void_p, c_long, c_long,
                                    c_int32, c_int32, c_int32, c_int32, c_int32, c_void_p, c_void_p]),
    "td7_dense_fwd_cat_w16": (c_int32, [c_int32, c_void_p, c_void_p, c_void_p, c_void_p, c_void_p, c_void_p,
                                        c_void_p, c_long, c_long, c_int32, c_int32, c_int32, c_int32, c_void_p,
                                        c_void_p]),
    "td7_dense_fwd_h": (c_int32, [c_void_p, c_void_p, c_long, c_long, c_void_p, c_void_p, c_void_p, c_void_p,
                                  c_long, c_long, c_int32, c_int32, c_int32, c_int32, c_int32, c_void_p, c_void_p]),
    "td7_dense_fwd_cat_h": (c_int32, [c_int32, c_void_p, c_int32, c_void_p, c_void_p, c_void_p, c_void_p, c_void_p,
                                      c_void_p, c_long, c_long, c_int32, c_int32, c_int32, c_int32, c_void_p,
                                      c_void_p]),
    "td7_dense_bwd_weight_cat": (c_int32, [c_void_p, c_long, c_long, c_void_p, c_long, c_long, c_int32, c_void_p,
                                           c_void_p, c_void_p, c_void_p, c_void_p, c_void_p, c_int32, c_int32, c_int32,
                                           c_int32, c_void_p]),
    "td7_adam_step_multi": (c_int32, [c_int32, c_void_p, c_void_p, c_void_p, c_void_p, c_void_p, c_void_p, c_void_p,
                                      c_void_p, c_void_p, c_int32, c_void_p, c_void_p, c_void_p, c_void_p, c_void_p,
                                      c_void_p]),
    "td7_dense_fwd_norm": (c_int32, [c_void_p, c_long, c_long, c_void_p, c_void_p, c_void_p, c_void_p, c_void_p,
                                     c_long, c_long, c_int32, c_int32, c_int32, c_int32, c_int32, ctypes.c_float,
                                     c_void_p]),
    "td7_dense_fwd_norm_cat": (c_int32, [c_int32, c_void_p, c_void_p, c_void_p, c_void_p, c_void_p, c_void_p, c_void_p,
                                         c_void_p, c_void_p, c_long, c_long, c_int32, c_int32, c_int32, c_int32,
                                         ctypes.c_float, c_void_p]),
    "td7_noisy_action_rng": (c_int32, [c_void_p, ctypes.c_uint64, ctypes.c_uint32, c_void_p, c_void_p, c_void_p,
                                       ctypes.c_float, ctypes.c_float, ctypes.c_float, c_void_p, c_int32, c_void_p,
                                       c_void_p]),
    "td7_dense_bwd_weight": (c_int32, [c_void_p, c_long, c_long, c_void_p, c_long, c_long, c_void_p, c_long,
                                       c_long, c_void_p, c_void_p, c_int32, c_int32, c_int32, c_int32, c_int32,
                                       c_void_p]),
    "td7f_pack": (c_int32, [c_int32, c_int32, P(TD7FPackJob), c_void_p]),
    "td7f_adam_pack": (c_int32, [c_int32, c_int32, c_void_p, c_void_p, c_void_p, c_void_p, c_void_p, c_void_p,
                                 c_void_p, c_void_p, c_void_p, c_int32, c_void_p, c_void_p, c_void_p, c_void_p,
                                 c_int32, P(TD7FPackJob), c_void_p, c_void_p, c_void_p]),
    "td7f_probe": (c_int32, [c_int32]),
    "td7f_select": (c_int32, [c_int32, P(c_int32), P(TD7FLin), P(TD7FLin), c_void_p, c_int32, P(TD7FNoise), c_void_p,
                              c_int32, c_int32, c_void_p]),
    "td7f_select_part": (c_int32, [c_int32, P(c_int32), P(TD7FLin), P(TD7FLin), c_void_p, c_int32, P(TD7FNoise),
                                   c_void_p, c_int32, c_int32, c_void_p, c_int32, c_void_p]),
    "td7f_select_seq": (c_int32, [c_int32, P(c_int32), P(TD7FLin), P(TD7FLin), c_void_p, c_int32, P(TD7FNoise),
                                  c_void_p, c_void_p, c_int32, c_void_p, c_int32, c_int32, c_void_p, c_int32,
                                  c_void_p]),
    "td7f_select_multi": (c_int32, [c_int32, P(c_int32), c_int32, P(TD7FLin), P(TD7FLin), c_void_p, P(c_int32),
                                    c_void_p, c_int32, c_void_p, c_int32, P(TD7FNoise), c_void_p, ctypes.c_float,
                                    c_void_p]),
    "td7f_multi_tiles": (c_int32, [c_int32, P(c_int32), P(c_int32), c_int32]),
    "td7f_multi_policy_table": (c_int32, [c_int32, P(TD7FLin), P(TD7FLin), P(TD7FLin)]),
    "td7f_select_multi_noise": (c_int32, [c_int32, P(c_int32), c_int32, P(TD7FLin), P(TD7FLin), c_void_p, P(c_int32),
                                          c_void_p, c_int32, c_void_p, c_int32, P(TD7FNoiseRow), c_void_p, c_void_p,
                                          c_void_p, c_void_p, c_void_p, ctypes.c_float, c_void_p]),
    "td7f_multi_noise_table": (c_int32, [c_int32, P(TD7FNoise), P(TD7FNoiseRow)]),
    "td7f_pink_advance": (c_int32, [c_int32, P(c_int32), c_int32, c_int32, c_int32, c_int32, P(c_int32)]
                          + [c_void_p] * 9 + [P(TD7FNoiseRow)] + [c_void_p] * 6),
    "td7f_select_multi_seq": (c_int32, [c_int32, P(c_int32), c_int32, P(TD7FLin), P(TD7FLin), c_void_p, P(c_int32),
                                        c_void_p, c_int32, c_void_p, c_int32, P(TD7FNoiseRow), c_void_p, c_void_p,
                                        c_void_p, c_void_p, c_void_p, c_int32, c_void_p, ctypes.c_float, c_void_p]),
    "td7f_target": (c_int32, [c_int32, P(c_int32), P(TD7FLin), P(TD7FLin), P(TD7FLin), c_void_p, c_int32,
                              P(TD7FNoise), c_void_p, c_void_p, c_void_p]),
    "td7f_fixed": (c_int32, [c_int32, P(c_int32), P(TD7FLin), c_void_p, c_void_p, c_int32, c_void_p, c_void_p,
                             c_void_p]),
    "td7f_critic": (c_int32, [c_int32, P(c_int32), P(TD7FLin)] + [c_void_p] * 7 + [ctypes.c_float]
                    + [c_void_p] * 4 + [c_int32] * 3 + [c_void_p] * 4 + [P(TD7FXT), ctypes.c_int64, c_void_p]),
    "td7f_critic_phase": (c_int32, [c_int32, c_int32, P(c_int32), P(TD7FLin)] + [c_void_p] * 7 + [ctypes.c_float]
                          + [c_void_p] * 4 + [c_int32] * 3 + [c_void_p] * 4
                          + [P(TD7FXT), ctypes.c_int64, c_void_p, c_void_p, c_void_p, c_void_p]),
    "td7f_encoder": (c_int32, [c_int32, P(c_int32), P(TD7FLin), c_void_p, c_void_p, c_void_p, c_int32, P(c_void_p),
                               P(TD7FXT), ctypes.c_int64, c_void_p, c_void_p, c_void_p]),
    "td7f_actor": (c_int32, [c_int32, c_int32, P(c_int32), P(TD7FLin), P(TD7FLin), P(TD7FLin), c_void_p, c_void_p,
                             c_int32, P(TD7FActorBufs), P(TD7FXT), ctypes.c_int64, c_void_p]),
    "td7f_actor_bc": (c_int32, [c_int32, c_int32, P(c_int32), P(TD7FLin), P(TD7FLin), P(TD7FLin), c_void_p, c_void_p,
                                c_void_p, ctypes.c_float, c_void_p, c_int32, P(TD7FActorBufs), P(TD7FXT),
                                ctypes.c_int64, c_void_p]),
    "td7f_wgrad": (c_int32, [c_int32, c_int32, P(TD7FWgJob), ctypes.c_int64, c_int32, c_void_p, c_void_p, c_int32,
                             ctypes.c_float, ctypes.c_float, c_void_p]),
    "td7f_wgrad_adam": (c_int32, [c_int32, c_int32, P(TD7FWgJob), ctypes.c_int64, c_int32, c_void_p, c_void_p,
                                  c_int32, ctypes.c_float, ctypes.c_float, c_int32, c_void_p, c_void_p, c_void_p,
                                  c_void_p, c_void_p, c_void_p, c_void_p, c_void_p, c_void_p, P(TD7FWgAdam), c_void_p,
                                  c_void_p]),
}

_lib = None


def build(force=False):
    if force:
        subprocess.run(["make", "-s", "-C", CSRC, "clean"], check=True)
    subprocess.run(["make", "-s", "-j4", "-C", CSRC], check=True)


def lib():
    global _lib
    if _lib is None:
        if not os.path.exists(LIB_PATH):
            raise ImportError(f"{LIB_PATH} is missing: build it with `make -C {CSRC}` (hipcc, gfx950)")
        L = ctypes.CDLL(LIB_PATH)
        for name, (res, args) in EXPORTS.items():
            fn = getattr(L, name)
            fn.restype, fn.argtypes = res, args
        _lib = L
    return _lib


def check(rc, what, ctx=None):
    if rc != EXO_OK:
        msg = ""
        if ctx is not None:
            m = lib().exo_last_error(ctx)
            msg = m.decode() if m else ""
        raise RuntimeError(f"{what} failed: {ERRORS.get(rc, rc)} {msg}")


def require_gpu(device):
    if not torch.cuda.is_available():
        raise RuntimeError("exo_amd runs on an MI355X (HIP) device; no GPU is visible and there is no CPU fallback")
    dev = torch.device(device if device is not None else "cuda")
    if dev.type != "cuda":
        raise RuntimeError(f"exo_amd tensors live on the GPU, got device {dev}")
    if dev.index is None:
        dev = torch.device("cuda", torch.cuda.current_device())
    return dev


def stream_ptr(device):
    return ctypes.c_void_p(torch.cuda.current_stream(device).cuda_stream)


def ptr(t):
    return ctypes.c_void_p(t.data_ptr()) if t is not None else None
```

### a-deep-reinforcement-learning-enabled-soft-exoskeleton-for-parkinson-s-patients_amd/exo_amd/replay.py

```python
import ctypes
import os

import numpy as np
import torch

from . import _native as nat


class LAP:
    def __init__(self, state_dim, action_dim, device, num_envs, max_size=1e6, batch_size=64, max_action=1,
                 normalize_actions=True, prioritized=True):
        if not prioritized:
            raise NotImplementedError("only the prioritized LAP buffer of the TD7 agent is implemented")
        self.device = nat.require_gpu(device)
        self.max_size = int(max_size)
        self.max_action = max_action
        self.batch_size = int(batch_size)
        self.num_envs = int(num_envs)
        self.state_dim, self.action_dim = state_dim, action_dim
        self.normalize_actions = max_action if normalize_actions else 1
        self.prioritized = True
        E, C = self.num_envs, self.max_size
        if C > 1 << 24:
            raise ValueError(f"LAP: max_size {C} above 2^24 rows per stratum")
        f32 = dict(device=self.device, dtype=torch.float32)
        self.state = torch.zeros((E, C + 1, state_dim), **f32)
        self.action = torch.zeros((E, C + 1, action_dim), **f32)
        self.next_state = torch.zeros((E, C + 1, state_dim), **f32)
        self.reward = torch.zeros((E, C + 1, 1), **f32)
        self.not_done = torch.zeros((E, C + 1, 1), **f32)
        cap = 1
        while cap < C:
            cap <<= 1
        self._tree = torch.zeros((E, 2 * cap), **f32)
        self._maxp = torch.ones((1,), **f32)
        self._desc = nat.LapTreeDesc(self._tree.data_ptr(), self._maxp.data_ptr(), E, C, cap)
        self._cap = cap
        self.ptr = 0
        self.count = 0
        self.size = 0
        i32 = dict(device=self.device, dtype=torch.int32)
        self.ptr_s = torch.zeros((E,), **i32)
        self.size_s = torch.zeros((E,), **i32)
        self._row0 = (torch.arange(E, device=self.device, dtype=torch.int64) * (C + 1))
        self.ind = None
        self.ref_state = torch.zeros((3,), dtype=torch.int64, device=self.device)
        self._ref_ws = None
        self.ref_insert_fused = os.environ.get("EXO_REF_INSERT_FUSED", "1") != "0"
        self._u = torch.empty((E, self.batch_size), **f32)
        from .ops import DeviceRNG
        self.device_rng = os.environ.get("EXO_DEVICE_RNG", "1") != "0"
        self._rng = DeviceRNG(self.device, 3)
        self._idx = torch.empty((E, self.batch_size), **i32)
        self._store = nat.LapStorageDesc(self.state.data_ptr(), self.action.data_ptr(), self.next_state.data_ptr(),
                                         self.reward.data_ptr(), self.not_done.data_ptr(), state_dim, action_dim,
                                         self.ptr_s.data_ptr(), self.size_s.data_ptr())
        B = E * self.batch_size
        sn = torch.empty((2, B, state_dim), **f32)
        self._batch = (sn[0], torch.empty((B, action_dim), **f32), sn[1], torch.empty((B, 1), **f32),
                       torch.empty((B, 1), **f32))
        self._row_ws = None
        self._init_tree()

    def _stream(self):
        return nat.stream_ptr(self.device)

    def _init_tree(self):
        nat.check(nat.lib().lap_init(ctypes.byref(self._desc), self._stream()), "lap_init")

    @property
    def priority(self):
        return self._tree[:, self._cap:self._cap + self.max_size]

    @property
    def max_priority(self):
        return float(self._maxp)

    @property
    def totals(self):
        return self._tree[:, 1]

    def add(self, state, action, next_state, reward, done, tremor_num):
        s, p = int(tremor_num), self.ptr
        dev = self.device
        self.state[s, p] = torch.as_tensor(np.asarray(state, dtype=np.float32), device=dev)
        self.action[s, p] = torch.as_tensor(np.asarray(action, dtype=np.float32) / self.normalize_actions, device=dev)
        self.next_state[s, p] = torch.as_tensor(np.asarray(next_state, dtype=np.float32), device=dev)
        self.reward[s, p] = float(reward)
        self.not_done[s, p] = 1.0 - float(done)
        st = torch.tensor([s], dtype=torch.int32, device=dev)
        sl = torch.tensor([p], dtype=torch.int32, device=dev)
        nat.check(nat.lib().lap_add(ctypes.byref(self._desc), nat.ptr(st), nat.ptr(sl), 1, self._stream()), "lap_add")
        if self.count % self.num_envs == 0:
            self.ptr = (self.ptr + 1) % self.max_size
            self.size = min(self.size + 1, self.max_size)
        self.count += 1
        self.size_s.fill_(self.size)

    def add_batch(self, state, action, next_state, reward, done, strata, active=None):
        n = state.shape[0]
        if self._row_ws is None or self._row_ws.numel() < n:
            self._row_ws = torch.empty((n,), dtype=torch.int32, device=self.device)

        def f32(t, shape):
            t = t.to(device=self.device, dtype=torch.float32).reshape(shape)
            return t if t.is_contiguous() else t.contiguous()

        st = f32(state, (n, self.state_dim))
        nx = f32(next_state, (n, self.state_dim))
        ac = f32(action, (n, self.action_dim))
        rw = f32(reward, (n,))
        dn = done if done.dtype == torch.uint8 else (done.view(torch.uint8) if done.dtype == torch.bool
                                                     else done.to(torch.uint8))
        dn = dn.reshape(n).contiguous()
        sr = strata if strata.dtype == torch.int32 else strata.to(torch.int32)
        act = None
        if active is not None:
            act = active.view(torch.uint8) if active.dtype == torch.bool else active.to(torch.uint8)
            act = act.contiguous()
        nat.check(nat.lib().lap_store_batch(ctypes.byref(self._desc), ctypes.byref(self._store), nat.ptr(st),
                                            nat.ptr(ac), nat.ptr(nx), nat.ptr(rw), nat.ptr(dn), nat.ptr(sr.contiguous()),
                                            nat.ptr(act), float(self.normalize_actions), n, nat.ptr(self._row_ws),
                                            self._stream()), "lap_store_batch")

    def load_dataset(self, state, action, next_state, reward, done, strata, chunk=65536):
        cpu = lambda t: torch.as_tensor(t)
        sr = cpu(strata).to(torch.int64).reshape(-1).cpu()
        n = sr.numel()
        if n and (int(sr.min()) < 0 or int(sr.max()) >= self.num_envs):
            raise ValueError(f"load_dataset: strata outside 0..{self.num_envs - 1}")
        cols = [cpu(state).reshape(n, self.state_dim), cpu(action).reshape(n, self.action_dim),
                cpu(next_state).reshape(n, self.state_dim), cpu(reward).reshape(n), cpu(done).reshape(n)]
        cols[4] = cols[4].to(torch.uint8) if cols[4].dtype != torch.bool else cols[4]
        for lo, hi in self._dataset_chunks(sr, int(chunk)):
            s, a, s2, r, d = (c[lo:hi].to(self.device) for c in cols)
            self.add_batch(s, a, s2, r, d, sr[lo:hi].to(device=self.device, dtype=torch.int32))
        empty = (self.size_s == 0).nonzero().reshape(-1).tolist()
        if empty:
            raise ValueError(f"load_dataset: no rows for strata {empty} (every stratum is sampled)")

    def _dataset_chunks(self, strata, chunk):
        n, C = strata.numel(), self.max_size
        if n == 0:
            return []
        rank = torch.zeros(n, dtype=torch.int64)
        for s in range(self.num_envs):
            m = strata == s
            rank[m] = torch.arange(int(m.sum()))
        out, lo = [], 0
        base = torch.zeros(self.num_envs, dtype=torch.int64)
        while lo < n:
            hi = min(lo + max(chunk, 1), n)
            over = (rank[lo:hi] - base[strata[lo:hi]] >= C).nonzero()
            if over.numel():
                hi = lo + int(over[0])
            out.append((lo, hi))
            base.scatter_reduce_(0, strata[lo:hi], rank[lo:hi] + 1, "amax")
            lo = hi
        return out

    def export_dataset(self):
        C = self.max_size
        size, ptr = self.size_s.cpu().tolist(), self.ptr_s.cpu().tolist()
        rows, strata = [], []
        for s in range(self.num_envs):
            slots = (ptr[s] - size[s] + torch.arange(size[s], dtype=torch.int64)) % C
            rows.append(s * (C + 1) + slots)
            strata.append(torch.full((size[s],), s, dtype=torch.int32))
        rows = torch.cat(rows).to(self.device)
        take = lambda t: t.reshape(-1, t.shape[-1]).index_select(0, rows).cpu()
        return dict(state=take(self.state), action=take(self.action) * self.normalize_actions,
                    next_state=take(self.next_state), reward=take(self.reward).reshape(-1),
                    done=(1.0 - take(self.not_done).reshape(-1)).to(torch.uint8), strata=torch.cat(strata))

    def add_batch_ref(self, state, action, next_state, reward, done, strata, active=None, advance=None):
        n = state.shape[0]
        if self._ref_ws is None or self._ref_ws.numel() < 3 * n:
            self._ref_ws = torch.zeros((3 * n,), dtype=torch.int32, device=self.device)

        def f32(t, shape):
            t = t.to(device=self.device, dtype=torch.float32).reshape(shape)
            return t if t.is_contiguous() else t.contiguous()

        st = f32(state, (n, self.state_dim))
        nx = f32(next_state, (n, self.state_dim))
        ac = f32(action, (n, self.action_dim))
        rw = f32(reward, (n,))
        dn = done if done.dtype == torch.uint8 else (done.view(torch.uint8) if done.dtype == torch.bool
                                                     else done.to(torch.uint8))
        dn = dn.reshape(n).contiguous()
        sr = (strata if strata.dtype == torch.int32 else strata.to(torch.int32)).contiguous()
        act = None
        if active is not None:
            act = (active.view(torch.uint8) if active.dtype == torch.bool else active.to(torch.uint8)).contiguous()
        if advance is not None:
            if not self.ref_insert_fused or act is None or act.data_ptr() != active.data_ptr():
                raise ValueError("add_batch_ref(advance=...): the fused insert and an in-place uint8/bool mask only")
            table, k, count, score = advance
            nat.check(nat.lib().lap_store_batch_ref_fused_adv(
                ctypes.byref(self._desc), ctypes.byref(self._store), nat.ptr(self.ref_state), nat.ptr(st),
                nat.ptr(ac), nat.ptr(nx), nat.ptr(rw), nat.ptr(dn), nat.ptr(sr), nat.ptr(act),
                float(self.normalize_actions), n, nat.ptr(self._ref_ws), nat.ptr(table), table.shape[0], nat.ptr(k),
                nat.ptr(count), nat.ptr(score), self._stream()), "lap_store_batch_ref_fused_adv")
            return
        fn = "lap_store_batch_ref_fused" if self.ref_insert_fused else "lap_store_batch_ref"
        nat.check(getattr(nat.lib(), fn)(ctypes.byref(self._desc), ctypes.byref(self._store),
                                         nat.ptr(self.ref_state), nat.ptr(st), nat.ptr(ac), nat.ptr(nx),
                                         nat.ptr(rw), nat.ptr(dn), nat.ptr(sr), nat.ptr(act),
                                         float(self.normalize_actions), n, nat.ptr(self._ref_ws),
                                         self._stream()), fn)

    def ref_plan(self, table, strata, offs, total, plan):
        rows, n = table.shape
        if getattr(self, "_ref_add_ws", None) is None or self._ref_add_ws.numel() < max(int(total), 1):
            self._ref_add_ws = torch.empty((max(int(total), 1),), dtype=torch.int32, device=self.device)
        tb = table.view(torch.uint8) if table.dtype == torch.bool else table
        sr = (strata if strata.dtype == torch.int32 else strata.to(torch.int32)).contiguous()
        nat.check(nat.lib().lap_ref_plan(ctypes.byref(self._desc), nat.ptr(self.ref_state), nat.ptr(tb), rows, n,
                                         nat.ptr(sr), nat.ptr(offs), int(total), nat.ptr(self._ref_add_ws),
                                         nat.ptr(plan), self._stream()), "lap_ref_plan")

    def ref_step(self, plan, table, kk, par, state, action, next_state, reward, done, strata, active,
                 k_dev=None, count=None, counts_table=None, score=None):
        rows, n = plan.shape
        tb = table.view(torch.uint8) if table.dtype == torch.bool else table
        dn = done.view(torch.uint8) if done.dtype == torch.bool else done.to(torch.uint8)
        act = active.view(torch.uint8) if active.dtype == torch.bool else active
        nat.check(nat.lib().lap_ref_step(
            ctypes.byref(self._desc), ctypes.byref(self._store), nat.ptr(plan), rows, n, nat.ptr(kk), int(par),
            nat.ptr(k_dev), nat.ptr(strata), nat.ptr(state.contiguous()), nat.ptr(action.contiguous()),
            nat.ptr(next_state.contiguous()), nat.ptr(reward.contiguous()), nat.ptr(dn.contiguous()),
            float(self.normalize_actions), nat.ptr(tb), nat.ptr(act), nat.ptr(count), nat.ptr(counts_table),
            nat.ptr(score), self._stream()), "lap_ref_step")

    def ref_commit(self, plan, strata, total):
        rows, n = plan.shape
        nat.check(nat.lib().lap_ref_commit(ctypes.byref(self._desc), ctypes.byref(self._store),
                                           nat.ptr(self.ref_state), nat.ptr(plan), rows, n, nat.ptr(strata),
                                           int(total), self._stream()), "lap_ref_commit")

    def ref_pointer(self):
        return tuple(int(v) for v in self.ref_state.cpu())

    def _slot(self, slot):
        if slot is None:
            return self._batch, self._idx
        if not hasattr(self, "_slots"):
            self._slots = {}
        if slot not in self._slots:
            f32 = dict(device=self.device, dtype=torch.float32)
            B, (S, A) = self._batch[0].shape[0], (self._batch[0].shape[1], self._batch[1].shape[1])
            sn = torch.empty((2, B, S), **f32)
            self._slots[slot] = ((sn[0], torch.empty((B, A), **f32), sn[1], torch.empty((B, 1), **f32),
                                  torch.empty((B, 1), **f32)), torch.empty_like(self._idx))
        return self._slots[slot]

    def sample(self, slot=None):
        batch, idx = self._slot(slot)
        if self.device_rng:
            r = self._rng
            nat.check(nat.lib().lap_sample_gather_rng(ctypes.byref(self._desc), ctypes.byref(self._store), r.seed,
                                                      r.tag, r.counter_ptr, r.ticket_ptr, self.batch_size,
                                                      nat.ptr(idx), *[nat.ptr(t) for t in batch],
                                                      self._stream()), "lap_sample_gather_rng")
        else:
            self._u.uniform_()
            nat.check(nat.lib().lap_sample_gather(ctypes.byref(self._desc), ctypes.byref(self._store),
                                                  nat.ptr(self._u), self.batch_size, nat.ptr(idx),
                                                  *[nat.ptr(t) for t in batch], self._stream()),
                      "lap_sample_gather")
        self.ind = idx
        return batch

    def sample_indices(self, u):
        u = u.to(device=self.device, dtype=torch.float32).contiguous()
        idx = torch.empty(u.shape, dtype=torch.int32, device=self.device)
        nat.check(nat.lib().lap_sample(ctypes.byref(self._desc), nat.ptr(u), nat.ptr(self.size_s), u.shape[1],
                                       nat.ptr(idx), self._stream()), "lap_sample")
        return idx

    def update_priority(self, priority, ind=None):
        ind = self.ind if ind is None else ind
        pr = priority.detach().to(torch.float32).reshape(-1).contiguous()
        assert pr.numel() == ind.numel()
        nat.check(nat.lib().lap_update(ctypes.byref(self._desc), nat.ptr(ind), nat.ptr(pr), ind.shape[1],
                                       self._stream()), "lap_update")

    fuse_update_sample = os.environ.get("EXO_LAP_FUSED", "1") != "0"

    def update_priority_and_sample(self, priority, ind=None, slot=None, before_gather=None):
        ind = self.ind if ind is None else ind
        if not (self.device_rng and self.fuse_update_sample and self.batch_size <= 1024):
            self.update_priority(priority, ind)
            if before_gather is not None:
                before_gather()
            return self.sample(slot)
        pr = priority.detach().to(torch.float32).reshape(-1).contiguous()
        assert pr.numel() == ind.numel()
        batch, idx = self._slot(slot)
        r = self._rng
        if before_gather is not None:
            nat.check(nat.lib().lap_update_sample_idx(ctypes.byref(self._desc), ctypes.byref(self._store), nat.ptr(ind),
                                                      nat.ptr(pr), ind.shape[1], r.seed, r.tag, r.counter_ptr,
                                                      r.ticket_ptr, nat.ptr(idx), self._stream()),
                      "lap_update_sample_idx")
            before_gather()
            nat.check(nat.lib().lap_gather_rows(ctypes.byref(self._desc), ctypes.byref(self._store), ind.shape[1],
                                                nat.ptr(idx), *[nat.ptr(t) for t in batch], self._stream()),
                      "lap_gather_rows")
            self.ind = idx
            return batch
        nat.check(nat.lib().lap_update_sample_rng(ctypes.byref(self._desc), ctypes.byref(self._store), nat.ptr(ind),
                                                  nat.ptr(pr), ind.shape[1], r.seed, r.tag, r.counter_ptr,
                                                  r.ticket_ptr, nat.ptr(idx), *[nat.ptr(t) for t in batch],
                                                  self._stream()), "lap_update_sample_rng")
        self.ind = idx
        return batch

    def update_priority_and_sample_td(self, td, alpha, min_priority, ind, slot, prio_out=None):
        if not (self.device_rng and self.batch_size <= 1024):
            raise RuntimeError("update_priority_and_sample_td: the device RNG and batch <= 1024 only")
        batch, idx = self._slot(slot)
        r = self._rng
        nat.check(nat.lib().lap_update_sample_td(ctypes.byref(self._desc), ctypes.byref(self._store), nat.ptr(ind),
                                                 nat.ptr(td), float(alpha), float(min_priority), nat.ptr(prio_out),
                                                 ind.shape[1], r.seed, r.tag, r.counter_ptr, r.ticket_ptr,
                                                 nat.ptr(idx), *[nat.ptr(t) for t in batch], self._stream()),
                  "lap_update_sample_td")
        self.ind = idx
        return batch

    def reset_max_priority(self):
        nat.check(nat.lib().lap_reset_max(ctypes.byref(self._desc), self._stream()), "lap_reset_max")

    def reset_buffer(self):
        self.ptr = self.count = self.size = 0
        for t in (self.state, self.action, self.next_state, self.reward, self.not_done):
            t.zero_()
        self.ptr_s.zero_()
        self.size_s.zero_()
        self.ref_state.zero_()
        self._init_tree()
```

### a-deep-reinforcement-learning-enabled-soft-exoskeleton-for-parkinson-s-patients_amd/exo_amd/rollout.py

```python
import contextlib
import os
import threading

import numpy as np
import torch

from . import _native as nat
from .graphs import capture, new_graph
from . import td7 as _td7
from .td7 import ENC_STEP_BRANCH


def graph_reductions_ok(device, rows=1024, cols=300, replays=3):
    gen = torch.Generator(device=device).manual_seed(0)
    x = torch.randn(rows, cols, device=device, generator=gen)
    s = torch.cuda.Stream(device=device)
    s.wait_stream(torch.cuda.current_stream(device))
    with torch.cuda.stream(s):
        x.sum(0)
        g = new_graph()
        with capture(g, stream=s):
            out = x.sum(0)
    torch.cuda.current_stream(device).wait_stream(s)
    for _ in range(replays):
        x.mul_(1.5)
        g.replay()
        if not torch.allclose(out, x.sum(0), rtol=1e-4, atol=1e-3):
            raise RuntimeError(
                "HIP graph replay of torch reductions is wrong in this process (ROCm CLR graph packet "
                "capture). Set DEBUG_CLR_GRAPH_PACKET_CAPTURE=0 before the first GPU call -- importing "
                "exo_amd before touching the GPU does it -- or use VecTrainer(use_graphs=False).")
    return True


def retire_graphs(trainer):
    from .graphs import release_graphs
    objs = []
    for name in ("graphs", "_round_graphs"):
        g = getattr(trainer, name, None)
        if isinstance(g, dict) and g:
            objs.append(dict(g))
            g.clear()
    if trainer.__dict__.get("_refresh_graph") is not None:
        objs.append(trainer._refresh_graph)
        trainer._refresh_graph = None
    return release_graphs(*objs)


def _np_median(x):
    v = x.sort().values
    n = v.numel()
    return v[n // 2] if n % 2 else (v[n // 2 - 1] + v[n // 2]) / 2


class CaptureForkError(RuntimeError):
    pass


def unjoined_streams(events, origin):
    def key(st):
        return st.cuda_stream
    captured, last_use = {key(origin)}, {}
    joins = {}
    objs = {}
    for t, ev in enumerate(events):
        if ev[0] == "wait":
            _, w, x = ev
            objs[key(w)], objs[key(x)] = w, x
            if key(x) in captured and key(w) not in captured:
                captured.add(key(w))
                last_use.setdefault(key(w), t)
            if key(x) in captured and key(x) != key(origin):
                joins.setdefault(key(x), []).append((t, key(w)))
        else:
            objs[key(ev[1])] = ev[1]
            if key(ev[1]) in captured:
                last_use[key(ev[1])] = t

    def ordered(s, t, seen=()):
        if s == key(origin):
            return True
        return any(tj >= t and w not in seen and ordered(w, tj, seen + (s,)) for tj, w in joins.get(s, ()))

    return [objs[s] for s in captured if s != key(origin) and not ordered(s, last_use.get(s, 0))]


class ForkJoinAudit:

    _lock = threading.Lock()
    _depth = 0
    _orig = None
    _open = []

    def __init__(self, origin):
        self.origin = origin
        self.events = []
        self._thread = None

    @classmethod
    def _record(cls, ev):
        me = threading.get_ident()
        for audit in list(cls._open):
            if audit._thread == me:
                audit.events.append(ev)

    def __enter__(self):
        cls = ForkJoinAudit
        self._thread = threading.get_ident()
        with cls._lock:
            if cls._depth == 0:
                wait0, exit0 = torch.cuda.Stream.wait_stream, torch.cuda.StreamContext.__exit__
                cls._orig = (wait0, exit0)

                def wait_stream(st, other):
                    cls._record(("wait", st, other))
                    return wait0(st, other)

                def ctx_exit(ctx, *a):
                    if ctx.stream is not None:
                        cls._record(("use", ctx.stream))
                    return exit0(ctx, *a)

                torch.cuda.Stream.wait_stream = wait_stream
                torch.cuda.StreamContext.__exit__ = ctx_exit
            cls._depth += 1
            cls._open.append(self)
        return self

    def __exit__(self, exc_type, exc, tb):
        cls = ForkJoinAudit
        with cls._lock:
            cls._open.remove(self)
            cls._depth -= 1
            if cls._depth == 0:
                torch.cuda.Stream.wait_stream, torch.cuda.StreamContext.__exit__ = cls._orig
                cls._orig = None
        if exc_type is not None:
            return False
        bad = unjoined_streams(self.events, self.origin)
        if bad:
            for st in bad:
                self.origin.wait_stream(st)
            raise CaptureForkError(f"{len(bad)} stream(s) forked from the capture stream were not joined back "
                                   "before capture end")
        return False


ROLLOUT_AFTER = os.environ.get("EXO_ROLLOUT_AFTER", "")
TRAIN_FIRST = os.environ.get("EXO_TRAIN_FIRST", "1") == "1"
EARLY_LAP = os.environ.get("EXO_EARLY_LAP", "1") == "1"
PAIR_CRITIC_AFTER_SELECT = os.environ.get("EXO_PAIR_CRITIC_AFTER_SELECT", "0") == "1"


class VecTrainer:
    def __init__(self, env, agent, strata=None, use_graphs=True, warmup_eager=3, exploration="gaussian",
                 shared_step=True, episodes=None):
        self.env, self.agent = env, agent
        self.device = env.device
        self.n = env.n
        Ls = env.lengths_host
        self.round_len = int(Ls.max()) - 3
        self.active_table = torch.as_tensor(np.stack([Ls - 3 > k for k in range(self.round_len)]),
                                            device=self.device)
        self.active_counts = self.active_table.sum(1).cpu().numpy()
        self.strata = (torch.as_tensor(env.motions % agent.env_num, dtype=torch.int32, device=self.device)
                       if strata is None else strata)
        o0 = env.reset()
        self._obs = [o0, torch.empty_like(o0)]
        outs = [env.new_outputs(True), env.new_outputs(True)]
        self._outs = [(self._obs[1], *outs[0][1:]), (self._obs[0], *outs[1][1:])]
        self._cur = 0
        self._table_ext = torch.cat([self.active_table, torch.zeros_like(self.active_table[:1])]).contiguous()
        self.active = self.active_table[0].clone()
        self.active_count = torch.full((1,), int(self.active_counts[0]), dtype=torch.int32, device=self.device)
        self.k = 0
        self.use_graphs = use_graphs
        self.warmup_eager = warmup_eager
        self.iters = 0
        self.resets = 0
        self.graphs = {}
        self.dp = agent.sync.active
        self.dp_inline = bool(self.dp and use_graphs and agent.sync.graph_capturable(self.device))
        if (shared_step and getattr(env, "step_variant", None) == "auto" and env.n <= 16384
                and os.environ.get("EXO_TRAIN_STEP_SHARED", "0") == "1"):
            env.set_step_variant("rows_shared")
        self.last_actions = None
        if exploration not in ("gaussian", "pink", "pink_env"):
            raise ValueError(f"exploration must be 'gaussian', 'pink' or 'pink_env', not {exploration!r}")
        self.exploration = exploration
        self.k_dev = torch.zeros((1,), dtype=torch.int64, device=self.device)
        self.budget = int(getattr(env, "step_budget", 0))
        if self.budget:
            if exploration == "pink":
                raise ValueError("Pink exploration indexes its noise by the round's step: not with a step budget")
            self._remaining = torch.zeros((1,), dtype=torch.int32, device=self.device)
            self._steps_total = torch.zeros((1,), dtype=torch.int64, device=self.device)
        if episodes is None:
            episodes = os.environ.get("EXO_EPISODES", "sync")
        if episodes not in ("sync", "async"):
            raise ValueError(f"episodes must be 'sync' or 'async', not {episodes!r}")
        self.episodes = episodes
        if episodes == "async":
            if exploration == "pink":
                raise ValueError("Pink exploration indexes its noise by the round's step: not with async episodes")
            self.active.fill_(True)
            self.active_count.fill_(self.n)
            if not self.budget:
                self._steps_total = torch.zeros((1,), dtype=torch.int64, device=self.device)
        if exploration == "pink":
            agent.init_episode_noise_device(self.round_len)
        self.pink = None
        if exploration == "pink_env":
            if episodes != "async":
                raise ValueError("exploration='pink_env' keeps a noise sequence per env and episode: it needs "
                                 "episodes='async' (synchronous rounds: exploration='pink')")
            if self.dp:
                raise ValueError("exploration='pink_env' is not available under data parallelism")
            if agent.learner.fused is None or self.device.type != "cuda":
                raise ValueError("exploration='pink_env' needs a learner with the fused passes on the GPU")
            from .fused import PinkNoise
            self.pink = PinkNoise.for_learner(agent.learner.fused, Ls)
            self._pink_stepped = torch.ones(self.n, dtype=torch.bool, device=self.device)
            self._pink_done = torch.zeros(self.n, dtype=torch.bool, device=self.device)
        if use_graphs and os.environ.get("EXO_GRAPH_CHECK", "1") != "0":
            graph_reductions_ok(self.device)

    def _select_cap(self):
        env = os.environ.get("EXO_LOOP_SELECT_CAP")
        if env is not None:
            return int(env)
        return 128 if self.agent.learner.precision == "fp32" else None

    loop_select_rt = int(os.environ.get("EXO_LOOP_SELECT_RT", "2"))

    def _select_rt(self):
        if self.agent.learner.precision == "fp32":
            return None
        return self.loop_select_rt or None

    split_select = os.environ.get("EXO_SPLIT_SELECT", "auto")

    def _split_select_ok(self):
        L = self.agent.learner
        on = self.split_select == "1" or (self.split_select == "auto" and L.precision == "fp32")
        return on and L.fused is not None and self.exploration in ("gaussian", "pink_env") and self.obs.is_cuda

    def _select_zs(self):
        cap = os.environ.get("EXO_SPLIT_ZS_CAP")
        return self.agent.learner.fused.select_zs(self.obs, wg_cap=int(cap) if cap is not None else self._select_cap(),
                                                  rt=self._select_rt())

    def _rollout(self, zs_img=None):
        ag = self.agent
        obs = self.obs
        act = ag.select_action_batch(obs, timestep=self.k_dev if self.exploration == "pink" else None,
                                     dec_count=self.active_count, wg_cap=self._select_cap(), rt=self._select_rt(),
                                     zs_img=zs_img, pink=self.pink)
        if self._overlap_wait is not None and PAIR_CRITIC_AFTER_SELECT:
            self._select_done = torch.cuda.Event()
            self._select_done.record(torch.cuda.current_stream(self.device))
        nobs, rew, done, info = self.env.step(act, active=self.active, out=self._outs[self._cur],
                                              obs_cur=obs if self.budget else None)
        ag.replay_buffer.add_batch(obs, act, nobs, rew, done, self.strata, self.active)
        if self._early_on:
            self._ins_ev = torch.cuda.Event()
            self._ins_ev.record(torch.cuda.current_stream(self.device))
        if self.pink is None:
            self._advance()
        elif not self.budget:
            self.pink.advance(self.active, done)
            self._advance()
        else:
            self._pink_stepped.copy_(self.active)
            self._advance()
            self.env.reset_mask(self._pink_done)
            self.pink.advance(self._pink_stepped, self._pink_done)
        self.last_actions = act

    def _advance(self, rew=None, score=None):
        if self.episodes == "async":
            self.env.episode_advance(self.active, self.active_count, self._outs[self._cur][0], self._steps_total)
            return
        if self.budget:
            self.env.budget_advance(self.active, self.active_count, self._remaining, self._steps_total)
            return
        if score is not None:
            nat.check(nat.lib().exo_active_advance_score(
                nat.ptr(self._table_ext), self._table_ext.shape[0], self.n, nat.ptr(self.k_dev), nat.ptr(self.active),
                nat.ptr(self.active_count), nat.ptr(rew), nat.ptr(score), nat.stream_ptr(self.device)),
                "exo_active_advance_score")
            return
        nat.check(nat.lib().exo_active_advance(nat.ptr(self._table_ext), self._table_ext.shape[0], self.n,
                                               nat.ptr(self.k_dev), nat.ptr(self.active), nat.ptr(self.active_count),
                                               nat.stream_ptr(self.device)), "exo_active_advance")

    def _round_start(self):
        self.k = 0
        self.k_dev.zero_()
        self.active.copy_(self.active_table[0])
        self.active_count.fill_(int(self.active_counts[0]))

    @property
    def obs(self):
        return self._obs[self._cur]

    @property
    def out(self):
        return self._outs[self._cur]

    overlap_rollout = os.environ.get("EXO_ROLLOUT_OVERLAP", "1") == "1"
    prefetch_sample = os.environ.get("EXO_SAMPLE_PREFETCH", "1") == "1"

    def _prefetching(self):
        return self.prefetch_sample and self.overlap_rollout

    prefetch_targets = os.environ.get("EXO_TARGET_PREFETCH", "0") == "1"
    _pre_in = _pre_out = False

    def _target_prefetch_flags(self):
        L = self.agent.learner
        ok = (self.prefetch_targets and self._prefetching() and L.fused_train and self.iters > 0
              and (not self.dp or self.dp_inline))
        pre_in = ok and L.prefetch_ready(self._cur)
        pre_out = ok and L.training_steps % L.hp.target_update_rate != 0
        return pre_in, pre_out

    def _pre(self, rollout=True):
        ag = self.agent
        self._early_on = False
        ag.learner.defer_side_join = ENC_STEP_BRANCH and (not self.dp or self.dp_inline)
        rb = ag.replay_buffer
        if not rollout:
            if self._train_pin:
                self._batch, self._ind = rb._slot(self._bslot)
            else:
                self._batch = rb.sample(self._bslot if self._train_pout else None)
                self._ind = rb.ind
            self._prio = ag.learner.phase_grads(*self._batch)
            return
        slot = self._cur if self._prefetching() else None
        if self.iters == 0 or not self.overlap_rollout:
            self._rollout()
            self._batch = rb.sample(slot)
            self._ind = rb.ind
            self._prio = ag.learner.phase_grads(*self._batch)
            return
        self._early_on = self._early_lap()
        if self._prefetching():
            self._batch, self._ind = rb._slot(slot)
            if self._pre_in:
                ag.learner.pre_in = slot
        else:
            self._batch = rb.sample()
            self._ind = rb.ind
        cur = torch.cuda.current_stream(self.device)
        if getattr(self, "_rollout_stream", None) is None:
            self._rollout_stream = torch.cuda.Stream(device=self.device)
        br = self._rollout_stream

        split = self._overlap_wait is not None and self._split_select_ok()

        def rollout_branch(cur=cur, br=br):
            br.wait_stream(cur)
            zimg = None
            if split:
                with torch.cuda.stream(br):
                    zimg = self._select_zs()
            if self._overlap_wait is not None:
                br.wait_stream(self._overlap_wait)
            with torch.cuda.stream(br):
                self._rollout(zs_img=zimg)
        L = ag.learner
        late = (ROLLOUT_AFTER == "fixed" and L.fused_train and L.pre_in is None and not self._pre_in
                and not _td7.TARGET_ON_MAIN)
        first = (TRAIN_FIRST and not late and L.fused_train and L.pre_in is None and not self._pre_in
                 and not _td7.TARGET_ON_MAIN and L.overlap)
        if late:
            L.after_fixed = rollout_branch
        elif first:
            ev0 = torch.cuda.Event()
            ev0.record(cur)

            def rollout_from_start(ev0=ev0, br=br):
                br.wait_event(ev0)
                zimg = None
                if split:
                    with torch.cuda.stream(br):
                        zimg = self._select_zs()
                if self._overlap_wait is not None:
                    br.wait_stream(self._overlap_wait)
                with torch.cuda.stream(br):
                    self._rollout(zs_img=zimg)
            L.after_target = rollout_from_start
        else:
            rollout_branch()
        if self._overlap_wait is not None and PAIR_CRITIC_AFTER_SELECT:
            def critic_after_select():
                torch.cuda.current_stream(self.device).wait_event(self._select_done)
            L.before_critic = critic_after_select
        self._us_done = False
        if self._us_after_critic():
            def fork(td, cur=cur, br=br):
                L = ag.learner
                ps = self._prio_stream_get()
                ps.wait_stream(cur)
                ps.wait_stream(br)
                with torch.cuda.stream(ps):
                    ag.replay_buffer.update_priority_and_sample_td(td, L.hp.alpha, L.hp.min_priority, self._ind,
                                                                   1 - self._cur)
                self._pside = ps
                self._us_done = True
            ag.learner.after_critic = fork
        self._prio = ag.learner.phase_grads(*self._batch)
        ag.learner.after_critic = None
        if ag.learner.after_fixed is not None or ag.learner.after_target is not None:
            raise RuntimeError("VecTrainer: the rollout branch was not forked (no fixed / target pass in phase_grads)")
        ag.learner.before_critic = None
        if self._early_on:
            self._br_pending = br
        else:
            cur.wait_stream(br)

    prio_branch = os.environ.get("EXO_PRIO_BRANCH", "1") == "1"
    prio_branch_all = os.environ.get("EXO_PRIO_BRANCH_ALL", "0") == "1"

    us_after_critic = os.environ.get("EXO_US_AFTER_CRITIC", "0") == "1"
    _us_done = False

    def _us_after_critic(self):
        L = self.agent.learner
        rb = self.agent.replay_buffer
        return (self.us_after_critic and not self.dp and self._prefetching() and not self._pre_out
                and L.fused_train and rb.device_rng and rb.batch_size <= 1024)

    def _prio_stream_get(self):
        if getattr(self, "_prio_stream", None) is None:
            self._prio_stream = torch.cuda.Stream(device=self.device)
        return self._prio_stream

    _early_on = False
    _br_pending = None
    _ins_ev = None

    def _early_lap(self):
        rb = self.agent.replay_buffer
        return (EARLY_LAP and not self.dp and self._prefetching() and not self._us_after_critic()
                and not self._pre_out and rb.device_rng and rb.fuse_update_sample and rb.batch_size <= 1024)

    def _join_rollout(self):
        if self._br_pending is not None:
            torch.cuda.current_stream(self.device).wait_stream(self._br_pending)
            self._br_pending = None

    def _mid(self, update_actor, flat_grad=None, grad_scale=1.0, rollout=True):
        ag = self.agent
        self._mid_rollout = rollout
        if update_actor:
            self._join_rollout()
        if self._us_done:
            self._us_done = False
            ag.learner.phase_steps(flat_grad, grad_scale)
            if update_actor:
                with self._actor_ctx():
                    ag.learner.phase_actor_grads(self._batch[0], self._batch[1])
            return
        self._pside = None
        if update_actor and self._actor_stream is not None:
            ag.learner.phase_steps(flat_grad, grad_scale)
            with self._actor_ctx():
                ag.learner.phase_actor_grads(self._batch[0], self._batch[1])
            cur = torch.cuda.current_stream(self.device)
            if getattr(self, "_prio_stream", None) is None:
                self._prio_stream = torch.cuda.Stream(device=self.device)
            self._pside = self._prio_stream
            self._pside.wait_stream(cur)
            with torch.cuda.stream(self._pside):
                self._update_and_sample_next()
            return
        if self.prio_branch and not self.dp and (update_actor or self.prio_branch_all):
            cur = torch.cuda.current_stream(self.device)
            if getattr(self, "_prio_stream", None) is None:
                self._prio_stream = torch.cuda.Stream(device=self.device)
            self._pside = self._prio_stream
            self._pside.wait_stream(cur)
            with torch.cuda.stream(self._pside):
                self._update_and_sample_next()
            ag.learner.phase_steps(flat_grad, grad_scale)
        else:
            ag.learner.phase_steps(flat_grad, grad_scale)
            self._update_and_sample_next()
        if update_actor:
            with self._actor_ctx():
                ag.learner.phase_actor_grads(self._batch[0], self._batch[1])

    _actor_stream = None
    _overlap_wait = None

    def _actor_ctx(self):
        st = self._actor_stream
        cur = torch.cuda.current_stream(self.device)
        if st is None or cur.cuda_stream == st.cuda_stream:
            return contextlib.nullcontext()
        st.wait_stream(cur)
        return torch.cuda.stream(st)

    def _update_and_sample_next(self):
        rb = self.agent.replay_buffer
        if not self._mid_rollout and self._train_pout:
            rb.update_priority_and_sample(self._prio, self._ind, 1 - self._bslot)
        elif self._prefetching() and self._mid_rollout:
            if self._br_pending is not None and self._ins_ev is not None:
                torch.cuda.current_stream(self.device).wait_event(self._ins_ev)
                rb.update_priority_and_sample(self._prio, self._ind, 1 - self._cur, before_gather=self._join_rollout)
            else:
                self._join_rollout()
                rb.update_priority_and_sample(self._prio, self._ind, 1 - self._cur)
            if self._pre_out:
                b = rb._slot(1 - self._cur)[0]
                self.agent.learner.prefetch_targets(b[0], b[1], b[2], 1 - self._cur)
        else:
            rb.update_priority(self._prio, self._ind)

    def _join_prio(self):
        self._join_rollout()
        if getattr(self, "_pside", None) is not None:
            torch.cuda.current_stream(self.device).wait_stream(self._pside)
            self._pside = None
        L = self.agent.learner
        L.join_side()
        L.join_prefetch()
        L.defer_side_join = False

    def _post(self, update_actor, flat_grad=None, grad_scale=1.0):
        if update_actor:
            with self._actor_ctx():
                self.agent.learner.phase_actor_step(flat_grad, grad_scale)

    def _inline(self, update_actor, rollout=True):
        ag, L, S = self.agent, self.agent.learner, self.agent.sync
        L.dp_inline = True
        try:
            self._pre(rollout)
            self._mid_rollout = rollout
            cur = torch.cuda.current_stream(self.device)
            if getattr(self, "_prio_stream", None) is None:
                self._prio_stream = torch.cuda.Stream(device=self.device)
            self._pside = self._prio_stream
            if update_actor and self._actor_stream is not None:
                flat_c = L.allreduce_phase_grads(self._batch[0].shape[0])
                L.phase_steps(flat_c, 1.0)
                with self._actor_ctx():
                    L.phase_actor_grads(self._batch[0], self._batch[1])
                    flat_a = L.allreduce_actor_grads()
                    self._post(update_actor, flat_a, 1.0)
                self._pside.wait_stream(cur)
                with torch.cuda.stream(self._pside):
                    self._update_and_sample_next()
                    S.max_(ag.replay_buffer._maxp)
                self._join_prio()
                return
            self._pside.wait_stream(cur)
            with torch.cuda.stream(self._pside):
                self._update_and_sample_next()
            flat_c = L.allreduce_phase_grads(self._batch[0].shape[0])
            with torch.cuda.stream(self._pside):
                S.max_(ag.replay_buffer._maxp)
            L.phase_steps(flat_c, 1.0)
            flat_a = None
            if update_actor:
                L.phase_actor_grads(self._batch[0], self._batch[1])
                flat_a = L.allreduce_actor_grads()
            self._post(update_actor, flat_a, 1.0)
            self._join_prio()
        finally:
            L.dp_inline = False

    def _eager(self, update_actor, rollout=True):
        if self.dp_inline:
            self._inline(update_actor, rollout)
            return
        L = self.agent.learner
        self._pre(rollout)
        L.sync.allreduce_grads(L.grad_params())
        self._mid(update_actor, rollout=rollout)
        self.agent.sync.max_(self.agent.replay_buffer._maxp)
        if update_actor:
            L.sync.allreduce_grads(L.grad_params(actor=True))
        self._post(update_actor)
        self._join_prio()

    def _key(self, update_actor, rollout):
        if rollout:
            return update_actor, self._cur, self._pre_in, self._pre_out
        if self._train_pin or self._train_pout:
            return "train", update_actor, self._train_pin, self._train_pout, self._bslot
        return "train", update_actor

    _train_pin = _train_pout = False
    _bslot = 0

    def _capture(self, update_actor, rollout=True):
        self._capture_graph(update_actor, rollout)
        self._replay(update_actor, rollout)

    def _capture_graph(self, update_actor, rollout=True):
        s = torch.cuda.Stream(device=self.device)
        s.wait_stream(torch.cuda.current_stream(self.device))
        pool = None
        parts = []
        with torch.cuda.stream(s):
            if not self.dp or self.dp_inline:
                g = new_graph()
                with capture(g, pool=pool, stream=s), ForkJoinAudit(s):
                    if self.dp_inline:
                        self._inline(update_actor, rollout)
                    else:
                        self._pre(rollout)
                        self._mid(update_actor, rollout=rollout)
                        self._post(update_actor)
                        self._join_prio()
                parts = [g]
            else:
                L, S = self.agent.learner, self.agent.sync
                g1, g2, g3 = new_graph(), new_graph(), new_graph()
                with capture(g1, pool=pool, stream=s), ForkJoinAudit(s):
                    self._pre(rollout)
                    flat_c = S.pack(L.grad_params())
                pool = g1.pool()
                flat_a = None
                scale = 1.0 / S.world
                with capture(g2, pool=pool, stream=s), ForkJoinAudit(s):
                    self._mid(update_actor, flat_c, scale, rollout)
                    if update_actor:
                        flat_a = S.pack(L.grad_params(actor=True))
                if update_actor:
                    with capture(g3, pool=pool, stream=s), ForkJoinAudit(s):
                        self._post(update_actor, flat_a, scale)
                else:
                    g3 = None
                parts = [g1, g2, g3, flat_c, flat_a]
        torch.cuda.current_stream(self.device).wait_stream(s)
        self.graphs[self._key(update_actor, rollout)] = parts
        if self._graph_refresh() and self._refresh_graph is None:
            self._capture_refresh()

    def _replay(self, update_actor, rollout=True):
        parts = self.graphs[self._key(update_actor, rollout)]
        if not self.dp or self.dp_inline:
            parts[0].replay()
            return
        S = self.agent.sync
        g1, g2, g3, flat_c, flat_a = parts
        g1.replay()
        S.allreduce_flat(flat_c)
        g2.replay()
        S.max_(self.agent.replay_buffer._maxp)
        if update_actor:
            S.allreduce_flat(flat_a)
            g3.replay()

    pair_graphs = os.environ.get("EXO_PAIR_GRAPHS", "0") == "1"
    overlap_pairs = os.environ.get("EXO_OVERLAP_PAIRS", "1") == "1"
    _pair_second = False

    def _pair_ok(self):
        L = self.agent.learner
        if self.overlap_pairs and not self.pair_graphs:
            if not (L.fused_train and L.training_steps % L.hp.policy_freq == 0 and L.hp.policy_freq == 2):
                return False
        elif not self.pair_graphs:
            return False
        return (self.use_graphs and (not self.dp or (self.dp_inline and self.overlap_pairs and not self.pair_graphs))
                and self.iters >= self.warmup_eager
                and not (self._pre_in or self._pre_out)
                and L.training_steps % L.hp.target_update_rate != 0
                and (self.episodes == "async" or self.k + 1 < self.round_len))

    def _pair_key(self, ua, ua2, overlap=False):
        return ("pair", ua, ua2, self._cur) + (("overlap",) if overlap else ())

    def _run_pair(self, ua, ua2, overlap=False):
        g = self.graphs.get(self._pair_key(ua, ua2, overlap))
        if g is None:
            g = self._capture_pair(ua, ua2, overlap)
        g.replay()

    def _capture_pair(self, ua, ua2, overlap=False):
        L = self.agent.learner
        key = self._pair_key(ua, ua2, overlap)
        s = torch.cuda.Stream(device=self.device)
        s.wait_stream(torch.cuda.current_stream(self.device))
        g = new_graph()
        cur0 = self._cur
        keep = []
        if overlap and getattr(self, "_astream", None) is None:
            self._astream = torch.cuda.Stream(device=self.device)
        if overlap and self._split_select_ok():
            L.fused.zs_image(self.n)
        try:
            with torch.cuda.stream(s):
                with capture(g, stream=s), ForkJoinAudit(s):
                    for i, u in enumerate((ua, ua2)):
                        L.prefetch_actor = u
                        if overlap and i == 0:
                            self._actor_stream = self._astream
                        if overlap and i == 1:
                            self._actor_stream = None
                            self._overlap_wait = self._astream
                            L.before_critic_step = lambda st=self._astream: (
                                torch.cuda.current_stream(self.device).wait_stream(st))
                        if self.dp_inline:
                            self._inline(u, True)
                        else:
                            self._pre(True)
                            self._mid(u, rollout=True)
                            self._post(u)
                            self._join_prio()
                        if i == 0:
                            keep.append(L._fixed_zs)
                            self._cur ^= 1
                            self.iters += 1
                    if overlap:
                        s.wait_stream(self._astream)
        finally:
            self._actor_stream = self._overlap_wait = None
            L.before_critic_step = None
        torch.cuda.current_stream(self.device).wait_stream(s)
        self._cur = cur0
        self.iters -= 1
        L.prefetch_actor = ua
        self.graphs[key] = g
        self._pair_keep = getattr(self, "_pair_keep", []) + keep
        return g

    def next_step_resets(self):
        if self.episodes == "async" or self.k < self.round_len:
            return False
        return not self.budget or int(self._remaining.item()) == 0

    def env_steps_total(self):
        return int(self._steps_total.item())

    _horizon = None

    def plan(self, n):
        self._horizon = None if n is None else int(n)

    def prepare(self):
        L = self.agent.learner
        if (not self.use_graphs or self.iters < self.warmup_eager or self._pair_second
                or self.prefetch_targets):
            return 0
        pf = L.hp.policy_freq
        saved = (L.training_steps, L.prefetch_actor, self._pre_in, self._pre_out, self._cur, self.iters, self.k)
        made = 0
        try:
            self._pre_in = self._pre_out = False
            for _ in range(2):
                L.training_steps += 1
                ua = L.training_steps % pf == 0
                L.prefetch_actor = ua
                if self._key(ua, True) not in self.graphs:
                    self._capture_graph(ua)
                    made += 1
                self._cur ^= 1
                self.iters += 1
            L.training_steps, self._cur, self.iters = saved[0], saved[4], saved[5]
            L.training_steps += 1
            ua, ua2 = L.training_steps % pf == 0, (L.training_steps + 1) % pf == 0
            if self._horizon is not None and self._horizon >= 2 and self._pair_ok():
                overlap = self.overlap_pairs and ua and not ua2 and L.fused_train
                if self._pair_key(ua, ua2, overlap) not in self.graphs:
                    L.prefetch_actor = ua
                    self._capture_pair(ua, ua2, overlap)
                    made += 1
        finally:
            (L.training_steps, L.prefetch_actor, self._pre_in, self._pre_out, self._cur, self.iters,
             self.k) = saved
        return made

    def step(self):
        ag = self.agent
        L = ag.learner
        horizon = self._horizon
        if horizon is not None:
            self._horizon = horizon - 1
        if self._pair_second:
            self._pair_second = False
            L.training_steps += 1
            return self._step_tail()
        if self.next_step_resets():
            self.env.reset(obs_out=self.obs)
            self._round_start()
            self.resets += 1
            if self.exploration == "pink":
                ag.init_episode_noise_device(self.round_len)
        L.training_steps += 1
        update_actor = L.training_steps % ag.hp.policy_freq == 0
        L.prefetch_actor = update_actor
        self._pre_in, self._pre_out = self._target_prefetch_flags()
        if not self.use_graphs or self.iters < self.warmup_eager:
            self._eager(update_actor)
        elif (horizon is not None and horizon >= 2 and self._pair_ok() and self._key(update_actor, True) in self.graphs
              and ((L.training_steps + 1) % ag.hp.policy_freq == 0, 1 - self._cur, False, False) in self.graphs):
            ua2 = (L.training_steps + 1) % ag.hp.policy_freq == 0
            self._run_pair(update_actor, ua2,
                           overlap=self.overlap_pairs and update_actor and not ua2 and L.fused_train)
            self._pair_second = True
        elif self._key(update_actor, True) not in self.graphs:
            self._capture(update_actor)
        else:
            self._replay(update_actor)
        if self._pre_in or self._pre_out:
            if not isinstance(L._pre_ready, list):
                L._pre_ready = [False, False]
            if self._pre_in:
                L._pre_ready[self._cur] = False
            if self._pre_out:
                L._pre_ready[1 - self._cur] = True
        L.pre_in = None
        return self._step_tail()

    _refresh_graph = None

    def _graph_refresh(self):
        return self.use_graphs and (not self.dp or self.dp_inline)

    def _refresh_targets(self):
        ag = self.agent
        L = ag.learner
        if L.training_steps % L.hp.target_update_rate != 0:
            return False
        if not self._graph_refresh():
            L.maybe_update_targets()
            ag.replay_buffer.reset_max_priority()
            ag.sync.max_(ag.replay_buffer._maxp)
            return True
        L.drop_prefetch()
        if self._refresh_graph is None:
            self._capture_refresh()
        self._refresh_graph.replay()
        return True

    def _capture_refresh(self):
        ag, L = self.agent, self.agent.learner
        s = torch.cuda.Stream(device=self.device)
        s.wait_stream(torch.cuda.current_stream(self.device))
        g = new_graph()
        with torch.cuda.stream(s):
            with capture(g, stream=s, capture_error_mode="thread_local"), ForkJoinAudit(s):
                L.update_targets_device()
                ag.replay_buffer.reset_max_priority()
                ag.sync.max_(ag.replay_buffer._maxp)
        torch.cuda.current_stream(self.device).wait_stream(s)
        self._refresh_graph = g

    def _step_tail(self):
        ag = self.agent
        L = ag.learner
        self._refresh_targets()
        if self.budget:
            n_active = 0
        elif self.episodes == "async":
            n_active = self.n
        else:
            n_active = int(self.active_counts[self.k])
        self.k += 1
        self.iters += 1
        self._cur ^= 1
        return n_active


class RefScheduleTrainer(VecTrainer):

    def __init__(self, env, agent, warmup=25_000, strata=None, use_graphs=True, ref_replay=True,
                 action_source=None, reset_source=None, warmup_eager=2, round_graph=None, stats=None,
                 save_prefix=None):
        if getattr(env, "step_budget", 0):
            raise ValueError("RefScheduleTrainer steps the script's synchronous episodes: no step budget")
        super().__init__(env, agent, strata=strata, use_graphs=use_graphs, warmup_eager=warmup_eager,
                         shared_step=False, episodes="sync")
        if getattr(env, "step_variant", None) == "rows_shared":
            env.set_step_variant("auto")
        self.warmup = int(warmup)
        self.ref_replay = ref_replay
        self.action_source, self.reset_source = action_source, reset_source
        self.world = agent.sync.world
        self.steps_count = 0
        self.allow_train = False
        self.rounds = 0
        self.updates = 0
        dev = self.device
        self.score = torch.zeros(self.n, dtype=torch.float64, device=dev)
        self._rand_act = torch.zeros((self.n, 7), dtype=torch.float32, device=dev)
        self._rand_acts = torch.zeros((2, self.n, 7), dtype=torch.float32, device=dev)
        Ls = env.lengths_host
        self.ep_len = Ls - 2
        self.round_env_steps = int((Ls - 3).sum())
        self.active_host = np.stack([Ls - 3 > k for k in range(self.round_len)])
        self._train_iters = 0
        self._roll_iters = 0
        self.trace = []
        if round_graph is None:
            round_graph = {"1": True, "2": "serial"}.get(os.environ.get("EXO_REF_ROUND_GRAPH", "2"), False)
        self.round_graph = bool(round_graph)
        self.round_overlap = round_graph != "serial"
        self._ins_stream = None
        self._ins_pending = False
        self._act_prev = torch.zeros((2, self.n), dtype=torch.bool, device=dev)
        self._round_graphs = {}
        self._eager_kinds = set()
        self.fused_score = os.environ.get("EXO_REF_FUSED_SCORE", "1") == "1"
        self.insert_advance = os.environ.get("EXO_REF_INSERT_ADVANCE", "1") == "1"
        self.burst_prefetch = os.environ.get("EXO_BURST_PREFETCH", "0") == "1"
        self._burst_i = 0
        self.stats = (os.environ.get("EXO_REF_STATS", "0") == "1") if stats is None else bool(stats)
        self.round_stats = []
        self._stat_bufs = None
        self.save_prefix = save_prefix
        self.saves = 0
        self.save_seconds = 0.0
        self.planned = os.environ.get("EXO_REF_PLANNED", "1") == "1" and ref_replay
        if self.planned:
            rows = self._table_ext.shape[0]
            counts = self._table_ext.sum(1).to(torch.int64)
            self._offs = torch.cumsum(counts, 0) - counts
            self._plan_total = int(counts.sum())
            self._counts_tab = counts.to(torch.int32)
            self._plan = torch.full((rows, self.n), -1, dtype=torch.int32, device=dev)
            self._kk = torch.zeros((2,), dtype=torch.int64, device=dev)

    def _use_plan(self):
        return (self.planned and self.ref_replay and self.fused_score and self.active.dtype == torch.bool
                and not (self.round_graph and self.round_overlap))

    def _seen_eager(self, random):
        return (bool(random), self.stats) in self._eager_kinds

    def _stats_buffers(self):
        if self._stat_bufs is None:
            f32 = dict(dtype=torch.float32, device=self.device)
            self._stat_bufs = (torch.zeros((self.n, 16), **f32), torch.zeros((self.round_len, self.n, 16), **f32),
                               torch.zeros((self.n, 6), **f32))
            self._pct_hist = []
        return self._stat_bufs

    def _step_stats(self, info):
        step, rec, ctr = self._stats_buffers()
        self.env.tremor_metrics(info, stepped=self.active, counters=ctr, out=step)
        rec.index_copy_(0, self.k_dev, step.unsqueeze(0))

    @torch.no_grad()
    def compute_round_stats(self):
        step, rec, ctr = self._stats_buffers()
        dev = self.device
        Ls = torch.as_tensor(self.env.lengths_host, device=dev)
        T = self.round_len
        inlen = torch.arange(T, device=dev)[:, None] < Ls[None, :]
        tred = rec[..., 0:7].double()
        ared = rec[..., 7:14].double()
        tot = rec[..., 14].double()
        v = torch.where(inlen[..., None] & (tred != 0), tred, torch.nan)
        v = v.permute(1, 0, 2).reshape(self.n, -1)
        cnt = (~v.isnan()).sum(1)
        sup_avg = v.nansum(1) / cnt
        srt = torch.sort(torch.where(v.isnan(), torch.inf, v), dim=1).values
        lo = ((cnt - 1).clamp(min=0) // 2)[:, None]
        hi = (cnt // 2).clamp(max=v.shape[1] - 1)[:, None]
        sup_med = torch.where(cnt > 0, (srt.gather(1, lo)[:, 0] + srt.gather(1, hi)[:, 0]) / 2, torch.nan)
        ep_len = torch.as_tensor(self.ep_len, device=dev, dtype=torch.float64)
        gotten = self.score - 2.0
        pct = gotten / ep_len * 100
        self._pct_hist = (self._pct_hist + [pct])[-100:]
        avg_r = torch.stack(self._pct_hist).mean(0)
        nz_a, nz_t = ared[ared != 0], tot[tot != 0]
        c = ctr.double().sum(0)
        vals = torch.stack([
            gotten.mean(), pct.mean(), avg_r.mean(), _np_median(avg_r),
            c[1] / (c[0] + c[1]) * 100, c[2] / float(Ls.sum()) * 100,
            sup_avg.nanmean(), sup_med.nanmean(),
            nz_a.mean() if nz_a.numel() else torch.zeros((), dtype=torch.float64, device=dev),
            c[4] / (c[3] + c[4]) * 100,
            nz_t.mean() if nz_t.numel() else torch.zeros((), dtype=torch.float64, device=dev)]).cpu().tolist()
        keys = ("avg_reward", "reward_pct", "avg_rewards_pct", "median_rewards_pct", "tremor_reduction_occurrence",
                "any_axis_reduction_pct", "overall_suppression_avg", "overall_suppression_median",
                "angle_suppression", "amplitude_reduction_occurrence", "total_amplitude_suppression")
        out = dict(zip(keys, vals))
        out["suppression_avg_per_env"] = sup_avg.cpu().numpy()
        out["suppression_median_per_env"] = sup_med.cpu().numpy()
        return out

    def _rollout_ref(self, random, injected=False, overlap=False):
        ag = self.agent
        obs = self.obs
        if injected:
            act = self._rand_act
        elif random:
            act = self._rand_acts[self._cur].uniform_(-1.0, 1.0)
        else:
            act = ag.select_action_batch(obs, dec_count=self.active_count)
        cur = torch.cuda.current_stream(self.device) if overlap else None
        if self._ins_pending:
            cur.wait_stream(self._ins_stream)
            self._ins_pending = False
        nobs, rew, done, info = self.env.step(act, active=self.active, out=self._outs[self._cur])
        if self.stats:
            self._step_stats(info)
        if not self.fused_score:
            self.score.add_(rew.where(self.active, 0.0))
        add = ag.replay_buffer.add_batch_ref if self.ref_replay else ag.replay_buffer.add_batch
        rb = ag.replay_buffer
        if self._use_plan():
            rb.ref_step(self._plan, self._table_ext, self._kk, self._cur, obs, act, nobs, rew, done, self.strata,
                        self.active, k_dev=self.k_dev, count=self.active_count, counts_table=self._counts_tab,
                        score=self.score)
            self.last_actions = act
            return
        if (self.insert_advance and self.fused_score and self.ref_replay and not overlap and rb.ref_insert_fused
                and self.active.dtype == torch.bool):
            rb.add_batch_ref(obs, act, nobs, rew, done, self.strata, self.active,
                             advance=(self._table_ext, self.k_dev, self.active_count, self.score))
            self.last_actions = act
            return
        if overlap:
            mask = self._act_prev[self._cur]
            mask.copy_(self.active)
            if self._ins_stream is None:
                self._ins_stream = torch.cuda.Stream(device=self.device)
            self._ins_stream.wait_stream(cur)
            with torch.cuda.stream(self._ins_stream):
                add(obs, act, nobs, rew, done, self.strata, mask)
            self._ins_pending = True
        else:
            add(obs, act, nobs, rew, done, self.strata, self.active)
        if self.fused_score:
            self._advance(rew, self.score)
        else:
            self._advance()
        self.last_actions = act

    def _roll_round(self, random):
        key = ("round", bool(random), self._cur, self.stats)
        g = self._round_graphs.get(key)
        if g is None:
            s = torch.cuda.Stream(device=self.device)
            s.wait_stream(torch.cuda.current_stream(self.device))
            g = new_graph()
            cur0 = self._cur
            with torch.cuda.stream(s):
                with capture(g, stream=s), ForkJoinAudit(s):
                    for _ in range(self.round_len):
                        self._rollout_ref(random, overlap=self.round_overlap)
                        self._cur ^= 1
                    if self._ins_pending:
                        s.wait_stream(self._ins_stream)
                        self._ins_pending = False
            torch.cuda.current_stream(self.device).wait_stream(s)
            self._cur = cur0
            self._round_graphs[key] = g
        g.replay()
        self._roll_iters += self.round_len
        self.k += self.round_len
        self._cur ^= self.round_len & 1

    def _roll_step(self, random):
        if self.action_source is not None:
            a = np.asarray(self.action_source(self, random), dtype=np.float32).reshape(self.n, -1)
            self._rand_act.copy_(torch.as_tensor(a, device=self.device))
            self._rollout_ref(random, injected=True)
        elif not self.use_graphs or self._roll_iters < self.warmup_eager:
            self._rollout_ref(random)
        else:
            key = ("roll", bool(random), self._cur, self.stats)
            g = self.graphs.get(key)
            if g is None:
                s = torch.cuda.Stream(device=self.device)
                s.wait_stream(torch.cuda.current_stream(self.device))
                g = new_graph()
                with torch.cuda.stream(s):
                    with capture(g, stream=s), ForkJoinAudit(s):
                        self._rollout_ref(random)
                torch.cuda.current_stream(self.device).wait_stream(s)
                self.graphs[key] = g
            g.replay()
        self._roll_iters += 1
        self.k += 1
        self._cur ^= 1

    def _burst_flags(self, burst):
        self._train_pin = self.burst_prefetch and self._burst_i > 0
        self._train_pout = self.burst_prefetch and self._burst_i + 1 < burst
        if self._train_pin:
            self._bslot ^= 1

    _tpair_second = False

    def train_step(self):
        ag, L = self.agent, self.agent.learner
        L.training_steps += 1
        if self._tpair_second:
            self._tpair_second = False
            self._burst_i += 1
            self._refresh_targets()
            self._train_iters += 1
            return
        update_actor = L.training_steps % ag.hp.policy_freq == 0
        L.prefetch_actor = update_actor
        self._pre_in = self._pre_out = False
        L.drop_prefetch()
        burst = int(ag.timesteps_since_update)
        bslot0 = self._bslot
        self._burst_flags(burst)
        if not self.use_graphs or self._train_iters < max(2, self.warmup_eager):
            self._eager(update_actor, rollout=False)
        elif self._key(update_actor, False) not in self.graphs:
# ... 244 lines not shown
```

### include/exo_amd.h

```cpp
#ifndef EXO_AMD_H
#define EXO_AMD_H

#include <stddef.h>
#include <stdint.h>

#ifdef __cplusplus
extern "C" {
#endif

#define EXO_OK 0
#define EXO_EINVAL (-22)
#define EXO_ENOMEM (-12)
#define EXO_EDEVICE (-5)
#define EXO_ERANGE (-34)

#define EXO_OBS_DIM 80
#define EXO_ACT_DIM 7
#define EXO_INFO_DIM 40
#define EXO_STATE_DOUBLES 53

#define EXO_DRAWS_PER_EPISODE(L) (208 + 8 * (L))

typedef struct {
    int32_t motion;
    int32_t tremor_sequence[7];
    double tremor_amplitude_range[2];
    double first_harmonics_interval[2];
    double second_harmonics_interval[2];
    double max_force_shoulder;
    double max_force_elbow;
    double dr_actuator_end_pos_shift;
    double dr_actuator_range;
    double matrix_noise_fraction;
} exo_env_config;

typedef struct exo_ctx exo_ctx;

int exo_create(const exo_env_config *cfgs_host, int32_t n_envs, const double *motion_angles_host,
               const int32_t *motion_lengths_host, int32_t n_motions, int32_t max_len, uint64_t seed,
               int32_t device, exo_ctx **out);

int exo_reset(exo_ctx *ctx, const uint8_t *mask_dev, float *obs_dev, void *stream);

int exo_reset_from_draws(exo_ctx *ctx, const int32_t *env_ids_host, int32_t n, const double *draws_host,
                         float *obs_dev, void *stream);

int exo_step(exo_ctx *ctx, const float *act_dev, float *obs_dev, float *rew_dev, uint8_t *done_dev,
             float *info_dev, const uint8_t *active_dev, void *stream);

int32_t exo_num_envs(const exo_ctx *ctx);
int exo_episode_length(const exo_ctx *ctx, int32_t env, int32_t *L_out);
int exo_tremor_host(exo_ctx *ctx, int32_t env, double *tremor_out );
int exo_original_joint_angles_host(exo_ctx *ctx, int32_t env, double *out7);

int exo_episode_host(exo_ctx *ctx, int32_t env, double *D49, double *S49, double *Iinv49, double *shift42,
                     double *maxSE2);

int exo_get_state_host(exo_ctx *ctx, int32_t env, double *out);
int exo_set_state_host(exo_ctx *ctx, int32_t env, const double *in);

#define EXO_STEP_AUTO 0
#define EXO_STEP_LANES 1
#define EXO_STEP_ROWS 2
#define EXO_STEP_ROWS_SHARED 3
int exo_set_step_variant(exo_ctx *ctx, int32_t variant);

int exo_set_step_budget(exo_ctx *ctx, int32_t budget);
int exo_step_carry(exo_ctx *ctx, const float *act_dev, float *obs_dev, float *rew_dev, uint8_t *done_dev,
                   float *info_dev, const uint8_t *active_dev, const float *obs_cur_dev, void *stream);
int exo_budget_advance(exo_ctx *ctx, uint8_t *active_dev, int32_t *count_dev, int32_t *remaining_dev,
                       int64_t *steps_total_dev, void *stream);

int exo_episode_advance(exo_ctx *c, uint8_t *active_dev, int32_t *count_dev, int32_t *reset_ws_dev,
                        int64_t *steps_total_dev, float *obs_dev, void *stream);
int exo_reset_mask(exo_ctx *c, const int32_t *reset_ws_dev, uint8_t *mask_dev, void *stream);

int exo_set_step_clock(exo_ctx *ctx, unsigned long long *clock_dev, double *ticks_per_ms);

#define EXO_TREMOR_SIGN_PER_SAMPLE 0
#define EXO_TREMOR_SIGN_PER_AXIS 1
#define EXO_TREMOR_SIGN_NONE 2
int exo_set_tremor_model(exo_ctx *ctx, const double *jmax7, int32_t sign_mode);

#define EXO_PHYS_IDEAL 0
#define EXO_PHYS_MULTIBODY 1
typedef struct {
    double gravity;
    double kp, kd;
    double motor_impulse;
    double passive_impulse;
    double limit_impulse;
    double erp;
    double lin_damp, ang_damp;
    double max_vel;
    int32_t iters;
} exo_mb_params;
void exo_multibody_default_params(exo_mb_params *out);
int exo_set_physics(exo_ctx *ctx, int32_t mode, const exo_mb_params *params);
int exo_multibody_advance(exo_ctx *ctx, const double *targets_dev, const uint8_t *mask_dev, void *stream);
int exo_get_multibody_state_host(exo_ctx *ctx, int32_t env, double *q19, double *qd19);
int exo_set_multibody_state_host(exo_ctx *ctx, int32_t env, const double *q19, const double *qd19);

int exo_set_seed(exo_ctx *ctx, uint64_t seed);
int exo_restart(exo_ctx *ctx, uint64_t seed, void *stream);

const char *exo_last_error(const exo_ctx *ctx);
void exo_destroy(exo_ctx *ctx);

int exo_tremor_metrics(exo_ctx *c, const float *info_dev, const uint8_t *stepped_dev, double humerus_length,
                       double forearm_length, double hand_length, int32_t disregard, float *metrics_dev,
                       float *counters_dev, void *stream);

int exo_active_advance(const uint8_t *table_dev, int32_t rows, int32_t n, int64_t *k_dev, uint8_t *active_dev,
                       int32_t *count_dev, void *stream);
int exo_active_advance_score(const uint8_t *table_dev, int32_t rows, int32_t n, int64_t *k_dev, uint8_t *active_dev,
                             int32_t *count_dev, const float *reward_dev, double *score_dev, void *stream);

int exo_eval_metrics(exo_ctx *c, const float *info_dev, const uint8_t *stepped_dev, double humerus_length,
                     double forearm_length, float *counters_dev, void *stream);

typedef struct {
    float *tree;
    float *max_priority;
    int32_t n_strata;
    int32_t capacity;
    int32_t cap;
} lap_tree_desc;

int32_t lap_tree_floats(int32_t n_strata, int32_t capacity);

int lap_init(const lap_tree_desc *t, void *stream);

int lap_add(const lap_tree_desc *t, const int32_t *stratum_dev, const int32_t *slot_dev, int32_t n, void *stream);

int lap_sample(const lap_tree_desc *t, const float *u_dev, const int32_t *size_dev, int32_t batch, int32_t *idx_dev,
               void *stream);

int lap_update(const lap_tree_desc *t, const int32_t *idx_dev, const float *prio_dev, int32_t batch, void *stream);

int lap_reset_max(const lap_tree_desc *t, void *stream);

int lap_totals(const lap_tree_desc *t, float *out_dev, void *stream);

typedef struct {
    float *state, *action, *next_state, *reward, *not_done;
    int32_t state_dim, action_dim;
    int32_t *ptr, *size;
} lap_storage_desc;

int lap_store_batch(const lap_tree_desc *t, const lap_storage_desc *st, const float *state_dev,
                    const float *action_dev, const float *next_state_dev, const float *reward_dev,
                    const uint8_t *done_dev, const int32_t *strata_dev, const uint8_t *active_dev, float action_scale,
                    int32_t n, int32_t *row_ws_dev, void *stream);

int lap_store_batch_ref(const lap_tree_desc *t, const lap_storage_desc *st, int64_t *ref_dev,
                        const float *state_dev, const float *action_dev, const float *next_state_dev,
                        const float *reward_dev, const uint8_t *done_dev, const int32_t *strata_dev,
                        const uint8_t *active_dev, float action_scale, int32_t n, int32_t *ws_dev, void *stream);

int lap_store_batch_ref_fused(const lap_tree_desc *t, const lap_storage_desc *st, int64_t *ref_dev,
                              const float *state_dev, const float *action_dev, const float *next_state_dev,
                              const float *reward_dev, const uint8_t *done_dev, const int32_t *strata_dev,
                              const uint8_t *active_dev, float action_scale, int32_t n, uint32_t *ticket_dev,
                              void *stream);

int lap_store_batch_ref_fused_adv(const lap_tree_desc *t, const lap_storage_desc *st, int64_t *ref_dev,
                                  const float *state, const float *action, const float *next_state,
                                  const float *reward, const uint8_t *done, const int32_t *strata, uint8_t *active,
                                  float action_scale, int32_t n, uint32_t *ticket_dev, const uint8_t *table,
                                  int32_t rows, int64_t *k_dev, int32_t *count_dev, double *score_dev, void *stream);

int lap_ref_plan(const lap_tree_desc *t, const int64_t *ref_dev, const uint8_t *table_dev, int32_t rows, int32_t n,
                 const int32_t *strata_dev, const int64_t *offs_dev, int64_t total, int32_t *add_ws_dev,
                 int32_t *plan_dev, void *stream);
int lap_ref_step(const lap_tree_desc *t, const lap_storage_desc *st, const int32_t *plan_dev, int32_t rows,
                 int32_t n, int64_t *kk_dev, int32_t par, int64_t *k_dev, const int32_t *strata_dev,
                 const float *state, const float *action, const float *next_state, const float *reward,
                 const uint8_t *done, float action_scale, const uint8_t *table_dev, uint8_t *active_dev,
                 int32_t *count_dev, const int32_t *counts_table_dev, double *score_dev, void *stream);
int lap_ref_commit(const lap_tree_desc *t, const lap_storage_desc *st, int64_t *ref_dev, const int32_t *plan_dev,
                   int32_t rows, int32_t n, const int32_t *strata_dev, int64_t total, void *stream);

int lap_sample_gather(const lap_tree_desc *t, const lap_storage_desc *st, const float *u_dev, int32_t batch,
                      int32_t *idx_dev, float *out_state, float *out_action, float *out_next_state,
                      float *out_reward, float *out_not_done, void *stream);
int lap_update_sample_rng(const lap_tree_desc *t, const lap_storage_desc *st, const int32_t *idx_in_dev,
                          const float *prio_dev, int32_t batch, uint64_t seed, uint32_t tag,
                          unsigned long long *counter_dev, uint32_t *ticket_dev, int32_t *idx_dev, float *out_state,
                          float *out_action, float *out_next_state, float *out_reward, float *out_not_done,
                          void *stream);

int lap_update_sample_idx(const lap_tree_desc *t, const lap_storage_desc *st, const int32_t *idx_in,
                          const float *prio, int32_t batch, uint64_t seed, uint32_t tag, unsigned long long *counter,
                          uint32_t *ticket, int32_t *idx_out, void *stream);
int lap_gather_rows(const lap_tree_desc *t, const lap_storage_desc *st, int32_t batch, const int32_t *idx,
                    float *out_state, float *out_action, float *out_next_state, float *out_reward,
                    float *out_not_done, void *stream);
int lap_update_sample_td(const lap_tree_desc *t, const lap_storage_desc *st, const int32_t *idx_in, const float *td,
                         float alpha, float min_priority, float *prio_out, int32_t batch, uint64_t seed, uint32_t tag,
                         unsigned long long *counter, uint32_t *ticket, int32_t *idx_out, float *out_state,
                         float *out_action, float *out_next_state, float *out_reward, float *out_not_done,
                         void *stream);
int lap_sample_gather_rng(const lap_tree_desc *t, const lap_storage_desc *st, uint64_t seed, uint32_t tag,
                          unsigned long long *counter_dev, uint32_t *ticket_dev, int32_t batch, int32_t *idx_dev,
                          float *out_state, float *out_action, float *out_next_state, float *out_reward,
                          float *out_not_done, void *stream);

int td7_avgl1norm_fwd(const float *x_dev, float *y_dev, float *mean_out_dev, int32_t rows, int32_t cols, float eps,
                      void *stream);
int td7_avgl1norm_fwd_h(const float *x_dev, uint16_t *y16_dev, float *mean_out_dev, int32_t rows, int32_t cols,
                        float eps, int32_t prec, void *stream);
int td7_avgl1norm_bwd(const float *x_dev, const float *mean_dev, const float *gy_dev, float *gx_dev, int32_t rows,
                      int32_t cols, float eps, void *stream);

int td7_adam_step(float *p_dev, const float *g_dev, float *m_dev, float *v_dev, float *step_dev, uint32_t *ticket_dev,
                  int64_t n, float lr, float beta1, float beta2, float eps, float weight_decay, float grad_scale,
                  void *stream);

#define TD7_ADAM_MAX_OPT 3
#define TD7_ADAM_MAX_SEG 40
int td7_adam_step_multi(int32_t nopt, float *const *p_dev, float *const *m_dev, float *const *v_dev,
                        float *const *step_dev, const float *lr, const float *beta1, const float *beta2,
                        const float *eps, const float *weight_decay, int32_t nseg, const float *const *g_dev,
                        const int64_t *off, const int32_t *n, const int32_t *opt, uint32_t *ticket_dev, void *stream);

int td7_q_target(const float *qt_dev, long qs_b, long qs_h, const float *reward_dev, const float *not_done_dev,
                 float discount, const float *min_target_dev, const float *max_target_dev, float *run_max_dev,
                 float *run_min_dev, float *out_dev, int32_t batch, void *stream);
int td7_critic_loss(const float *q_dev, long qs_b, long qs_h, const float *q_target_dev, float *loss_dev,
                    float *priority_dev, float *dq_dev, float alpha, float min_priority, int32_t batch, void *stream);
int td7_critic_loss_strided(const float *q_dev, long qs_b, long qs_h, const float *q_target_dev, float *loss_dev,
                            float *priority_dev, float *dq_dev, long dqs_b, long dqs_h, float alpha,
                            float min_priority, int32_t batch, void *stream);

int td7_noisy_action(const float *a_dev, const float *noise_dev, float *sigma_dev, float sigma_dec, float clip,
                     float scale, float *out_dev, int32_t n, void *stream);
int td7_noisy_action_rng(const float *a_dev, uint64_t seed, uint32_t tag, unsigned long long *counter_dev,
                         uint32_t *ticket_dev, float *sigma_dev, float sigma_dec, float clip, float scale,
                         float *out_dev, int32_t n, const int32_t *dec_count_dev, void *stream);
#define TD7_MSE_WS 257
int td7_mse_fwd(const float *x_dev, const float *y_dev, int64_t n, float *loss_dev, float *ws_dev, void *stream);
int td7_mse_bwd(const float *x_dev, const float *y_dev, const float *g_dev, int64_t n, float *dx_dev, void *stream);

int td7_dense_fwd(const float *x_dev, long xsg, long ldx, const float *w_dev, const float *b_dev, float *y_dev,
                  long ysg, long ldy, int32_t groups, int32_t m, int32_t n, int32_t k, int32_t act, void *stream);
int td7_dense_bwd_data(const float *dy_dev, long dysg, long lddy, const float *y_dev, long ysg, long ldy,
                       const float *w_dev, float *dx_dev, long dxsg, long lddx, int32_t groups, int32_t shared_input,
                       int32_t m, int32_t n, int32_t k, int32_t act, void *stream);
int td7_dense_fwd_cat(int32_t nseg, const float *const *xs_dev, const long *xsg, const long *ldx,
                      const int32_t *widths, const float *w_dev, const float *b_dev, float *y_dev, long ysg, long ldy,
                      int32_t groups, int32_t m, int32_t n, int32_t act, void *stream);
int td7_dense_fwd_w16(const float *x_dev, long xsg, long ldx, const float *w_dev, const float *b_dev, float *y_dev,
                      long ysg, long ldy, int32_t groups, int32_t m, int32_t n, int32_t k, int32_t act,
                      const uint16_t *w16_dev, void *stream);
int td7_dense_fwd_cat_w16(int32_t nseg, const float *const *xs_dev, const long *xsg, const long *ldx,
                          const int32_t *widths, const float *w_dev, const float *b_dev, float *y_dev, long ysg,
                          long ldy, int32_t groups, int32_t m, int32_t n, int32_t act, const uint16_t *w16_dev,
                          void *stream);
int td7_dense_fwd_h(const float *x_dev, const uint16_t *x16_dev, long xsg, long ldx, const float *w_dev,
                    const float *b_dev, float *y_dev, uint16_t *y16_dev, long ysg, long ldy, int32_t groups, int32_t m,
                    int32_t n, int32_t k, int32_t act, const uint16_t *w16_dev, void *stream);
int td7_dense_set_xl(int32_t variant);
int td7_dense_fwd_cat_h(int32_t nseg, const void *const *xs_dev, int32_t xs16, const long *xsg, const long *ldx,
                        const int32_t *widths, const float *w_dev, const float *b_dev, uint16_t *y16_dev, long ysg,
                        long ldy, int32_t groups, int32_t m, int32_t n, int32_t act, const uint16_t *w16_dev,
                        void *stream);

int td7_dense_fwd_norm(const float *x_dev, long xsg, long ldx, const float *w_dev, const float *b_dev, float *y_dev,
                       float *h_dev, float *mean_dev, long ysg, long ldy, int32_t groups, int32_t m, int32_t n,
                       int32_t k, int32_t prec, float eps, void *stream);
int td7_dense_fwd_norm_cat(int32_t nseg, const float *const *xs_dev, const long *xsg, const long *ldx,
                           const int32_t *widths, const float *w_dev, const float *b_dev, float *y_dev, float *h_dev,
                           float *mean_dev, long ysg, long ldy, int32_t groups, int32_t m, int32_t n, int32_t prec,
                           float eps, void *stream);

int td7_dense_bwd_weight_cat(const float *dy_dev, long dysg, long lddy, const float *y_dev, long ysg, long ldy,
                             int32_t nseg, const float *const *xs_dev, const long *xsg, const long *ldx,
                             const int32_t *widths, float *dw_dev, float *db_dev, int32_t groups, int32_t m, int32_t n,
                             int32_t act, void *stream);

int td7_dense_bwd_data_cols(const float *dy_dev, long dysg, long lddy, const float *y_dev, long ysg, long ldy,
                            const float *w_dev, float *dx_dev, long dxsg, long lddx, int32_t groups,
                            int32_t shared_input, int32_t m, int32_t n, int32_t k, int32_t c0, int32_t c1, int32_t act,
                            void *stream);
int td7_dense_bwd_weight(const float *dy_dev, long dysg, long lddy, const float *y_dev, long ysg, long ldy,
                         const float *x_dev, long xsg, long ldx, float *dw_dev, float *db_dev, int32_t groups,
                         int32_t m, int32_t n, int32_t k, int32_t act, void *stream);

#define TD7F_PD 5
#define TD7F_MAX_PACK 32

typedef struct {
    const void *wf;
    const void *wb;
    const float *b;
    int32_t n_out, n_in, ksf, ksb;
    const float *w;
    int64_t ldw;
} td7f_lin;

typedef struct {
    const float *w;
    int64_t ld;
    int32_t n_out, n_in;
    void *wf;
    void *wb;
    int32_t ksf, ntf, ksb, ntb;
} td7f_pack_job;

typedef struct {
    uint64_t seed;
    uint32_t tag, pad0;
    unsigned long long *counter;
    uint32_t *ticket;
    float *sigma;
    float sigma_dec, clip, scale;
    int32_t pad1;
    const float *z;
    const int32_t *dec_count;
} td7f_noise;

int td7f_pack(int32_t prec, int32_t njobs, const td7f_pack_job *jobs, void *stream);
#define TD7F_MAX_ADAM_PACK 16
int td7f_adam_pack(int32_t prec, int32_t nopt, float *const *p_dev, float *const *m_dev, float *const *v_dev,
                   float *const *step_dev, const float *lr, const float *beta1, const float *beta2, const float *eps,
                   const float *weight_decay, int32_t nseg, const float *const *g_dev, const int64_t *off,
                   const int32_t *n, const int32_t *opt, int32_t njobs, const td7f_pack_job *jobs,
                   const int32_t *job_seg, uint32_t *ticket_dev, void *stream);
int td7f_probe(int32_t on);
int td7f_select(int32_t prec, const int32_t *act, const td7f_lin *enc, const td7f_lin *actor, const float *obs_dev,
                int32_t n, const td7f_noise *noise, float *act_out_dev, int32_t wg_cap, int32_t rt, void *stream);
int td7f_select_part(int32_t prec, const int32_t *act, const td7f_lin *enc, const td7f_lin *actor,
                     const float *obs_dev, int32_t n, const td7f_noise *noise, float *act_out_dev, int32_t wg_cap,
                     int32_t rt, void *zs_img_dev, int32_t mode, void *stream);
int td7f_select_seq(int32_t prec, const int32_t *act, const td7f_lin *enc, const td7f_lin *actor,
                    const float *obs_dev, int32_t n, const td7f_noise *noise, const float *seq_dev,
                    const int32_t *t_dev, int32_t Lmax, float *act_out_dev, int32_t wg_cap, int32_t rt,
                    void *zs_img_dev, int32_t mode, void *stream);
int td7f_select_multi(int32_t prec, const int32_t *act, int32_t npol, const td7f_lin *enc, const td7f_lin *actor,
                      const void *policies_dev, const int32_t *seg, const int32_t *tiles_dev, int32_t ntiles,
                      const float *obs_dev, int32_t n, const td7f_noise *noise, float *act_out_dev, float scale,
                      void *stream);
int td7f_multi_tiles(int32_t npol, const int32_t *seg, int32_t *tiles, int32_t cap);
int td7f_multi_policy_table(int32_t npol, const td7f_lin *enc, const td7f_lin *actor, td7f_lin *table);
typedef struct {
    uint64_t seed;
    uint32_t tag, pad0;
    unsigned long long *counter;
    float *sigma;
    float sigma_dec, clip;
} td7f_noise_row;
int td7f_select_multi_noise(int32_t prec, const int32_t *act, int32_t npol, const td7f_lin *enc,
                            const td7f_lin *actor, const void *policies_dev, const int32_t *seg,
                            const int32_t *tiles_dev, int32_t ntiles, const float *obs_dev, int32_t n,
                            const td7f_noise_row *noise, const void *noise_dev, const int32_t *seg_dev,
                            uint32_t *ticket_dev, const float *z_dev, float *act_out_dev, float scale,
                            void *stream);
int td7f_multi_noise_table(int32_t npol, const td7f_noise *noise, td7f_noise_row *table);
int td7f_pink_advance(int32_t npol, const int32_t *seg, int32_t n, int32_t A, int32_t Lmax, int32_t ncls,
                      const int32_t *cls_len, const uint8_t *stepped_dev, const uint8_t *done_dev, int32_t *t_dev,
                      int32_t *epi_dev, float *seq_dev, const int32_t *len_cls_dev, const int32_t *cls_len_dev,
                      const float *cls_norm_dev, const float *cls_scale_dev, const td7f_noise_row *noise,
                      const void *noise_dev, const int32_t *seg_dev, const float *spectrum_dev, float *spec_out_dev,
                      float *peak_out_dev, void *stream);
int td7f_select_multi_seq(int32_t prec, const int32_t *act, int32_t npol, const td7f_lin *enc, const td7f_lin *actor,
                          const void *policies_dev, const int32_t *seg, const int32_t *tiles_dev, int32_t ntiles,
                          const float *obs_dev, int32_t n, const td7f_noise_row *noise, const void *noise_dev,
                          const int32_t *seg_dev, uint32_t *ticket_dev, const float *seq_dev, const int32_t *t_dev,
                          int32_t Lmax, float *act_out_dev, float scale, void *stream);
int td7f_target(int32_t prec, const int32_t *act, const td7f_lin *tenc, const td7f_lin *tactor,
                const td7f_lin *tcritic, const float *next_state_dev, int32_t B, const td7f_noise *noise,
                void *tgt_img_dev, float *qt_dev, void *stream);
int td7f_fixed(int32_t prec, const int32_t *act, const td7f_lin *fenc, const float *state_dev,
               const float *action_dev, int32_t B, float *zs_dev, float *zsa_dev, void *stream);

typedef struct {
    void *x;
    void *dp;
    float *part;
} td7f_xt;
int td7f_critic(int32_t prec, const int32_t *act, const td7f_lin *critic, const float *s_dev, const float *a_dev,
                const float *zs_dev, const float *zsa_dev, const float *qt_dev, const float *reward_dev,
                const float *not_done_dev, float discount, const float *lo_dev, const float *hi_dev,
                float *run_max_dev, float *run_min_dev, int32_t B, int32_t state_dim, int32_t action_dim,
                float *td_dev, float *q_dev, float *y1_dev, float *y2_dev, const td7f_xt *xt, int64_t ld,
                void *stream);
int td7f_critic_phase(int32_t phase, int32_t prec, const int32_t *act, const td7f_lin *critic, const float *s_dev,
                      const float *a_dev, const float *zs_dev, const float *zsa_dev, const float *qt_dev,
                      const float *reward_dev, const float *not_done_dev, float discount, const float *lo_dev,
                      const float *hi_dev, float *run_max_dev, float *run_min_dev, int32_t B, int32_t state_dim,
                      int32_t action_dim, float *td_dev, float *q_dev, float *y1_dev, float *y2_dev,
                      const td7f_xt *xt, int64_t ld, float *q_ws, float *h0_ws, float *mean_ws, void *stream);
int td7f_encoder(int32_t prec, const int32_t *act, const td7f_lin *enc, const float *s_dev, const float *a_dev,
                 const float *ns_dev, int32_t B, float *const *y, const td7f_xt *xt, int64_t ld, float *nz_ws,
                 int32_t *flag_ws, void *stream);
typedef struct {
    float *act_out;
    float *zsa_out;
    float *h0;
    float *mean0;
    float *ya[2];
    float *yz[2];
    float *yc[2];
    float *da;
    float *dzsa;
} td7f_actor_bufs;
int td7f_actor(int32_t prec, int32_t phase, const int32_t *act, const td7f_lin *actor, const td7f_lin *fenc,
               const td7f_lin *critic, const float *s_dev, const float *zs_dev, int32_t B,
               const td7f_actor_bufs *bufs, const td7f_xt *xt, int64_t ld, void *stream);
int td7f_actor_bc(int32_t prec, int32_t phase, const int32_t *act, const td7f_lin *actor, const td7f_lin *fenc,
                  const td7f_lin *critic, const float *s_dev, const float *zs_dev, const float *a_dev, float lmbda,
                  float *qabs_dev, int32_t B, const td7f_actor_bufs *bufs, const td7f_xt *xt, int64_t ld,
                  void *stream);
#define TD7F_MAX_WG 16
typedef struct {
    const void *dp;
    const void *x;
    const float *part;
    float *dw;
    float *db;
    int32_t n, k, row_tiles;
} td7f_wg_job;
int td7f_wgrad(int32_t prec, int32_t njobs, const td7f_wg_job *jobs, int64_t ld, int32_t rows, const float *td_dev,
               float *prio_dev, int32_t B, float alpha, float min_priority, void *stream);
typedef struct {
    int32_t opt;
    int64_t w_off, b_off;
    void *wf;
    void *wb;
    int32_t ksf, ksb;
} td7f_wg_adam;
int td7f_wgrad_adam(int32_t prec, int32_t njobs, const td7f_wg_job *jobs, int64_t ld, int32_t rows,
                    const float *td_dev, float *prio_dev, int32_t B, float alpha, float min_priority, int32_t nopt,
                    float *const *p_dev, float *const *m_dev, float *const *v_dev, float *const *step_dev,
                    const float *lr, const float *beta1, const float *beta2, const float *eps,
                    const float *weight_decay, const td7f_wg_adam *adam, uint32_t *ticket_dev, void *stream);

int exo_stream_ballast(int32_t n);
int exo_graph_branch_bound(void *graph, int32_t *out);

#ifdef __cplusplus
}
#endif
#endif
```

Baseline: 18.54 million.

## Fuse next-step replay store ranking into the priority update/sample chain kernel

Splits replay-buffer insertion into a rank phase (reserve ring slots, write leaf priorities, propagate the sum tree) and a row-copy phase. The rank phase can now run at the tail of the update/sample chain kernel for the next step, reusing its LDS buffers and computing the new max priority in-block, which removes a separate kernel launch and tree pass. The store-rank path also tries an LDS-resident span propagation with lighter lgkmcnt barriers before the older path. Python graph capture logic is extended to track pending pre-ranked buffers across single and paired graphs, which adds considerable state-handling complexity and the risk of ordering bugs.

```diff
diff --git a/a-deep-reinforcement-learning-enabled-soft-exoskeleton-for-parkinson-s-patients_amd/csrc/lap.hip b/a-deep-reinforcement-learning-enabled-soft-exoskeleton-for-parkinson-s-patients_amd/csrc/lap.hip
--- a/a-deep-reinforcement-learning-enabled-soft-exoskeleton-for-parkinson-s-patients_amd/csrc/lap.hip
+++ b/a-deep-reinforcement-learning-enabled-soft-exoskeleton-for-parkinson-s-patients_amd/csrc/lap.hip
@@ -63,8 +63,7 @@
     propagate_top(T, cap, levels, slot, n, top);
 }
 
-__device__ void propagate_span(float *T, int cap, int levels, int capacity, int first, int count) {
-    __shared__ float top[TOPN];
+__device__ void propagate_span_top(float *T, int cap, int levels, int capacity, int first, int count, float *top) {
     if (count <= 0) return;
     int a0 = first, e0 = first + count, a1 = 0, e1 = 0;
     if (count >= capacity) {
@@ -102,9 +101,16 @@
     for (int i = 1 + threadIdx.x; i < wb; i += blockDim.x) T[i] = top[i];
     __syncthreads();
 }
+__device__ void propagate_span(float *T, int cap, int levels, int capacity, int first, int count) {
+    __shared__ float top[TOPN];
+    propagate_span_top(T, cap, levels, capacity, first, count, top);
+}
 
 constexpr int SPAN_LDS = 4096;
 constexpr int SPAN_LEVELS = 32;
+
+__device__ __forceinline__ void lds_barrier() { asm volatile("s_waitcnt lgkmcnt(0)\n\ts_barrier" ::: "memory"); }
+
 __device__ bool propagate_span_lds(float *T, int cap, int levels, int capacity, int first, int count,
                                    float *buf , float *edge ) {
     const int a = cap + first, e = cap + first + count - 1;
@@ -127,7 +133,7 @@
         if (!(e & 1)) A[(e | 1) - (a & ~1)] = edge[1];
     }
     for (int lv = 1; lv <= levels; ++lv) {
-        __syncthreads();
+        lds_barrier();
         const int lo = a >> lv, hi = e >> lv, cbase = (a >> (lv - 1)) & ~1, nbase = lo & ~1;
         for (int node = lo + t; node <= hi; node += blockDim.x) {
             const int c = 2 * node - cbase;
@@ -319,16 +325,15 @@
 
 constexpr int STORE_CHUNK = UPD_THREADS * 4;
 
+static_assert(2 * SPAN_LDS == TOPN, "one LDS buffer serves propagate_span_lds and propagate_span_top");
 template <int RANK_RPT>
-__global__ __launch_bounds__(UPD_THREADS) void lap_store_rank_kernel(float *tree, const float *maxp, int cap,
-                                                                     int levels, int capacity, int32_t *ring_ptr,
-                                                                     int32_t *ring_size, const int32_t *strata,
-                                                                     const uint8_t *active, int n, int32_t *row_of) {
-    const int s = blockIdx.x, t = threadIdx.x, lane = t & 63, wv = t >> 6;
-    float *T = stratum_tree(tree, s, cap);
-    __shared__ int wsum[UPD_THREADS / 64];
-    __shared__ int chunk_total;
-    const float p = *maxp;
+__device__ __forceinline__ void store_rank(float *T, const float p, const int s, const int n_strata, int cap,
+                                           int levels, int capacity, int32_t *ring_ptr, int32_t *ring_size,
+                                           const int32_t *strata, const uint8_t *active, int n, int32_t *row_of,
+                                           int *wsum, int *chunk_total_p, float *span_buf, float *span_edge,
+                                           bool span_lds) {
+    const int t = threadIdx.x, lane = t & 63, wv = t >> 6;
+    int &chunk_total = *chunk_total_p;
     const int ptr0 = ring_ptr[s];
     const int row0 = s * (capacity + 1);
     int offset = 0;
@@ -369,7 +374,7 @@
         for (int k = 0; k < RANK_RPT; ++k) {
             const int i = base + RANK_RPT * t + k;
             if (i >= n) continue;
-            if (s == 0 && (st[k] < 0 || st[k] >= (int)gridDim.x)) row_of[i] = -1;
+            if (s == 0 && (st[k] < 0 || st[k] >= n_strata)) row_of[i] = -1;
             if (st[k] != s) continue;
             if (f[k]) {
                 const int slot = (ptr0 + rank) % capacity;
@@ -384,11 +389,26 @@
         __syncthreads();
         offset += total;
     }
-    propagate_span(T, cap, levels, capacity, ptr0, offset);
+    if (!(span_lds && propagate_span_lds(T, cap, levels, capacity, ptr0, offset, span_buf, span_edge)))
+        propagate_span_top(T, cap, levels, capacity, ptr0, offset, span_buf);
     if (t == 0) {
         ring_ptr[s] = (ptr0 + offset) % capacity;
         ring_size[s] = min(ring_size[s] + offset, capacity);
     }
+}
+
+template <int RANK_RPT>
+__global__ __launch_bounds__(UPD_THREADS) void lap_store_rank_kernel(float *tree, const float *maxp, int cap,
+                                                                     int levels, int capacity, int32_t *ring_ptr,
+                                                                     int32_t *ring_size, const int32_t *strata,
+                                                                     const uint8_t *active, int n, int32_t *row_of,
+                                                                     bool span_lds) {
+    __shared__ int wsum[UPD_THREADS / 64];
+    __shared__ int chunk_total;
+    __shared__ float span_buf[TOPN], span_edge[2 * SPAN_LEVELS];
+    store_rank<RANK_RPT>(stratum_tree(tree, blockIdx.x, cap), *maxp, blockIdx.x, gridDim.x, cap, levels, capacity,
+                         ring_ptr, ring_size, strata, active, n, row_of, wsum, &chunk_total, span_buf, span_edge,
+                         span_lds);
 }
 
 __device__ __forceinline__ long long mult_below(long long x, int E) { return (x + E - 1) / E; }
@@ -1312,13 +1332,20 @@
 constexpr int CHAIN_PAD = 0x40000000;
 constexpr int CHAIN_RNG0 = 640;
 
-__device__ __forceinline__ void lds_barrier() { asm volatile("s_waitcnt lgkmcnt(0)\n\ts_barrier" ::: "memory"); }
-
+struct RankNext {
+    const int32_t *strata;
+    const uint8_t *active;
+    int n;
+    int32_t *row_of, *ring_ptr;
+    bool span_lds;
+};
+
+template <bool RANK>
 __global__ __launch_bounds__(UPD_THREADS) void lap_update_sample_chain_kernel(
     float *tree, float *maxp, int cap, int levels, int capacity, const int32_t *idx_in,
     const float *__restrict__ prio, int batch, const int32_t *__restrict__ size, lap_storage_desc st, SampleRng rng,
     int32_t *idx_out, float *o_state, float *o_action, float *o_next, float *o_reward, float *o_not_done, TdPrio tp,
-    bool gather) {
+    bool gather, RankNext rk) {
     const int s = blockIdx.x, t = threadIdx.x;
     float *T = stratum_tree(tree, s, cap);
     __shared__ float red[UPD_THREADS / 64];
@@ -1340,6 +1367,13 @@
     const int me = idx_in[d];
     const float *pp = tp.td ? tp.td + 2 * d : prio + d;
     const float p0 = pp[0], p1 = pp[tp.td ? 1 : 0];
+    float q0 = 0.0f, q1 = 0.0f;
+    if constexpr (RANK) {
+        const long dq = min(t, (int)gridDim.x * batch - 1);
+        const float *qq = tp.td ? tp.td + 2 * dq : prio + dq;
+        q0 = qq[0];
+        q1 = qq[tp.td ? 1 : 0];
+    }
     constexpr int PER = TOPN_US / UPD_THREADS;
     float stage[PER];
 #pragma unroll
@@ -1484,6 +1518,23 @@
         *rng.counter = call + 1ull;
         *rng.ticket = 0u;
     }
+    if constexpr (RANK) {
+        static_assert(sizeof(top) == TOPN * sizeof(float) && sizeof(partner) >= 2 * SPAN_LEVELS * sizeof(float),
+                      "the span buffers alias top[] and partner[]");
+        __shared__ int wsum[UPD_THREADS / 64];
+        __shared__ int chunk_total;
+        float m = tp.td ? powf(fmaxf(fmaxf(q0, q1), tp.minp), tp.alpha) : q0;
+        for (int o = 32; o > 0; o >>= 1) m = fmaxf(m, __shfl_xor(m, o, 64));
+        if ((t & 63) == 0) red[t >> 6] = m;
+        __syncthreads();
+        m = red[0];
+#pragma unroll
+        for (int w = 1; w < UPD_THREADS / 64; ++w) m = fmaxf(m, red[w]);
+        const float pnew = fmaxf(m, __hip_atomic_load(maxp, __ATOMIC_RELAXED, __HIP_MEMORY_SCOPE_AGENT));
+        store_rank<4>(T, pnew, s, gridDim.x, cap, levels, capacity, rk.ring_ptr, const_cast<int32_t *>(size),
+                      rk.strata, rk.active, rk.n, rk.row_of, wsum, &chunk_total, top,
+                      reinterpret_cast<float *>(partner), rk.span_lds);
+    }
 }
 
 int rc(hipError_t e) { return e == hipSuccess ? EXO_OK : EXO_EDEVICE; }
@@ -1502,21 +1553,51 @@
     return on;
 }
 
+bool rank_span_lds() {
+    const char *e = getenv("EXO_LAP_RANK_LDS");
+    return !(e && e[0] == '0');
+}
+
+void launch_rank(const lap_tree_desc *t, int32_t *ring_ptr, int32_t *ring_size, const int32_t *strata,
+                 const uint8_t *active, int n, int32_t *row_of, void *stream) {
+    if (n > 4 * STORE_CHUNK)
+        hipLaunchKernelGGL(lap_store_rank_kernel<16>, dim3(t->n_strata), dim3(UPD_THREADS), 0, (hipStream_t)stream,
+                           t->tree, t->max_priority, t->cap, levels_of(t), t->capacity, ring_ptr, ring_size, strata,
+                           active, n, row_of, rank_span_lds());
+    else
+        hipLaunchKernelGGL(lap_store_rank_kernel<4>, dim3(t->n_strata), dim3(UPD_THREADS), 0, (hipStream_t)stream,
+                           t->tree, t->max_priority, t->cap, levels_of(t), t->capacity, ring_ptr, ring_size, strata,
+                           active, n, row_of, rank_span_lds());
+}
+
 void launch_update_sample(const lap_tree_desc *t, const lap_storage_desc *st, const int32_t *idx_in, const float *prio,
                           int batch, SampleRng rng, int32_t *idx_out, float *o_state, float *o_action, float *o_next,
-                          float *o_reward, float *o_not_done, TdPrio tp, bool gather, void *stream) {
+                          float *o_reward, float *o_not_done, TdPrio tp, bool gather, void *stream,
+                          const RankNext *rank = nullptr) {
     const char *e = getenv("EXO_LAP_CHAIN");
     const int levels = levels_of(t);
     const bool chain = !(e && e[0] == '0') && batch <= CHAIN_MAXB && levels >= 1 &&
                        lap_chain::global_levels(levels, TOPN_US) <= CHAIN_MAXG;
+    const char *f = getenv("EXO_LAP_RANK_FUSED");
+    if (chain && rank && !gather && !(f && f[0] == '0') && (long)t->n_strata * batch <= UPD_THREADS &&
+        rank->n <= 4 * STORE_CHUNK) {
+        hipLaunchKernelGGL(lap_update_sample_chain_kernel<true>, dim3(t->n_strata), dim3(UPD_THREADS), 0,
+                           (hipStream_t)stream, t->tree, t->max_priority, t->cap, levels, t->capacity, idx_in, prio,
+                           batch, st->size, *st, rng, idx_out, o_state, o_action, o_next, o_reward, o_not_done, tp,
+                           gather, *rank);
+        return;
+    }
     if (chain)
-        hipLaunchKernelGGL(lap_update_sample_chain_kernel, dim3(t->n_strata), dim3(UPD_THREADS), 0, (hipStream_t)stream,
-                           t->tree, t->max_priority, t->cap, levels, t->capacity, idx_in, prio, batch, st->size, *st,
-                           rng, idx_out, o_state, o_action, o_next, o_reward, o_not_done, tp, gather);
+        hipLaunchKernelGGL(lap_update_sample_chain_kernel<false>, dim3(t->n_strata), dim3(UPD_THREADS), 0,
+                           (hipStream_t)stream, t->tree, t->max_priority, t->cap, levels, t->capacity, idx_in, prio,
+                           batch, st->size, *st, rng, idx_out, o_state, o_action, o_next, o_reward, o_not_done, tp,
+                           gather, RankNext{});
     else
         hipLaunchKernelGGL(lap_update_sample_kernel, dim3(t->n_strata), dim3(UPD_THREADS), 0, (hipStream_t)stream,
                            t->tree, t->max_priority, t->cap, levels, t->capacity, idx_in, prio, batch, st->size, *st,
                            rng, idx_out, o_state, o_action, o_next, o_reward, o_not_done, tp, gather);
+    if (rank && hipGetLastError() == hipSuccess)
+        launch_rank(t, rank->ring_ptr, st->size, rank->strata, rank->active, rank->n, rank->row_of, stream);
 }
 
 int gather_after(const lap_tree_desc *t, const lap_storage_desc *st, int batch, const int32_t *idx, float *o_state,
@@ -1619,17 +1700,31 @@
                                done, action_scale);
         return rc(hipGetLastError());
     }
-    if (n > 4 * STORE_CHUNK)
-        hipLaunchKernelGGL(lap_store_rank_kernel<16>, dim3(t->n_strata), dim3(UPD_THREADS), 0, (hipStream_t)stream,
-                           t->tree, t->max_priority, t->cap, levels_of(t), t->capacity, st->ptr, st->size, strata,
-                           active, n, row_ws);
-    else
-        hipLaunchKernelGGL(lap_store_rank_kernel<4>, dim3(t->n_strata), dim3(UPD_THREADS), 0, (hipStream_t)stream,
-                           t->tree, t->max_priority, t->cap, levels_of(t), t->capacity, st->ptr, st->size, strata,
-                           active, n, row_ws);
+    launch_rank(t, st->ptr, st->size, strata, active, n, row_ws, stream);
     if (hipGetLastError() != hipSuccess) return EXO_EDEVICE;
     hipLaunchKernelGGL(lap_store_copy_kernel, dim3((n + 3) / 4), dim3(256), 0, (hipStream_t)stream, *st, state,
                        action, next_state, reward, done, action_scale, n, row_ws);
+    return rc(hipGetLastError());
+}
+
+int lap_store_rank(const lap_tree_desc *t, const lap_storage_desc *st, const int32_t *strata, const uint8_t *active,
+                   int32_t n, int32_t *row_of, void *stream) {
+    if (!valid(t) || !st || !st->ptr || !st->size || !strata || !row_of || n < 0) return EXO_EINVAL;
+    if (n == 0) return EXO_OK;
+    launch_rank(t, st->ptr, st->size, strata, active, n, row_of, stream);
+    return rc(hipGetLastError());
+}
+
+int lap_store_rows(const lap_storage_desc *st, const float *state, const float *action, const float *next_state,
+                   const float *reward, const uint8_t *done, float action_scale, int32_t n, const int32_t *row_of,
+                   void *stream) {
+    if (!st || !st->state || !st->action || !st->next_state || !st->reward || !st->not_done || st->state_dim <= 0 ||
+        st->action_dim <= 0 || !state || !action || !next_state || !reward || !done || !row_of || n < 0 ||
+        action_scale == 0.0f)
+        return EXO_EINVAL;
+    if (n == 0) return EXO_OK;
+    hipLaunchKernelGGL(lap_store_copy_kernel, dim3((n + 3) / 4), dim3(256), 0, (hipStream_t)stream, *st, state,
+                       action, next_state, reward, done, action_scale, n, row_of);
     return rc(hipGetLastError());
 }
 
@@ -1737,6 +1832,22 @@
     return rc(hipGetLastError());
 }
 
+int lap_update_sample_idx_rank(const lap_tree_desc *t, const lap_storage_desc *st, const int32_t *idx_in,
+                               const float *prio, const float *td, float alpha, float min_priority, float *prio_out,
+                               int32_t batch, uint64_t seed, uint32_t tag, unsigned long long *counter,
+                               uint32_t *ticket, int32_t *idx_out, const int32_t *strata, const uint8_t *active,
+                               int32_t n, int32_t *row_of_next, void *stream) {
+    if (!valid(t) || !st || !st->ptr || !st->size || !idx_in || (!prio && !td) || !counter || !ticket || !idx_out ||
+        batch <= 0 || batch > UPD_THREADS || !strata || !row_of_next || n <= 0)
+        return EXO_EINVAL;
+    const RankNext rk{strata, active, n, row_of_next, st->ptr, rank_span_lds()};
+    launch_update_sample(t, st, idx_in, td ? nullptr : prio, batch, SampleRng{seed, tag, counter, ticket}, idx_out,
+                         nullptr, nullptr, nullptr, nullptr, nullptr,
+                         td ? TdPrio{td, alpha, min_priority, prio_out} : TdPrio{nullptr, 0.f, 0.f, nullptr}, false,
+                         stream, &rk);
+    return rc(hipGetLastError());
+}
+
 int lap_gather_rows(const lap_tree_desc *t, const lap_storage_desc *st, int32_t batch, const int32_t *idx,
                     float *out_state, float *out_action, float *out_next_state, float *out_reward,
                     float *out_not_done, void *stream) {
diff --git a/a-deep-reinforcement-learning-enabled-soft-exoskeleton-for-parkinson-s-patients_amd/exo_amd/_native.py b/a-deep-reinforcement-learning-enabled-soft-exoskeleton-for-parkinson-s-patients_amd/exo_amd/_native.py
--- a/a-deep-reinforcement-learning-enabled-soft-exoskeleton-for-parkinson-s-patients_amd/exo_amd/_native.py
+++ b/a-deep-reinforcement-learning-enabled-soft-exoskeleton-for-parkinson-s-patients_amd/exo_amd/_native.py
@@ -152,6 +152,13 @@
                                         ctypes.c_uint32, c_void_p, c_void_p, c_void_p, c_void_p]),
     "lap_gather_rows": (c_int32, [c_void_p, c_void_p, c_int32, c_void_p, c_void_p, c_void_p, c_void_p, c_void_p,
                                   c_void_p, c_void_p]),
+    "lap_store_rank": (c_int32, [c_void_p, c_void_p, c_void_p, c_void_p, c_int32, c_void_p, c_void_p]),
+    "lap_store_rows": (c_int32, [c_void_p, c_void_p, c_void_p, c_void_p, c_void_p, c_void_p, ctypes.c_float, c_int32,
+                                 c_void_p, c_void_p]),
+    "lap_update_sample_idx_rank": (c_int32, [c_void_p, c_void_p, c_void_p, c_void_p, c_void_p, ctypes.c_float,
+                                             ctypes.c_float, c_void_p, c_int32, ctypes.c_uint64, ctypes.c_uint32,
+                                             c_void_p, c_void_p, c_void_p, c_void_p, c_void_p, c_int32, c_void_p,
+                                             c_void_p]),
     "lap_update_sample_td": (c_int32, [c_void_p, c_void_p, c_void_p, c_void_p, ctypes.c_float, ctypes.c_float,
                                        c_void_p, c_int32, ctypes.c_uint64, ctypes.c_uint32, c_void_p, c_void_p,
                                        c_void_p, c_void_p, c_void_p, c_void_p, c_void_p, c_void_p, c_void_p]),
diff --git a/a-deep-reinforcement-learning-enabled-soft-exoskeleton-for-parkinson-s-patients_amd/exo_amd/replay.py b/a-deep-reinforcement-learning-enabled-soft-exoskeleton-for-parkinson-s-patients_amd/exo_amd/replay.py
--- a/a-deep-reinforcement-learning-enabled-soft-exoskeleton-for-parkinson-s-patients_amd/exo_amd/replay.py
+++ b/a-deep-reinforcement-learning-enabled-soft-exoskeleton-for-parkinson-s-patients_amd/exo_amd/replay.py
@@ -60,6 +60,8 @@
         self._batch = (sn[0], torch.empty((B, action_dim), **f32), sn[1], torch.empty((B, 1), **f32),
                        torch.empty((B, 1), **f32))
         self._row_ws = None
+        self._row_pre = None
+        self.prerank_pending = None
         self._init_tree()
 
     def _stream(self):
@@ -99,6 +101,10 @@
 
     def add_batch(self, state, action, next_state, reward, done, strata, active=None):
         n = state.shape[0]
+        pre, self.prerank_pending = self.prerank_pending, None
+        if pre is not None and (pre[0] != n or pre[1] != strata.data_ptr() or active is not None):
+            raise RuntimeError("LAP.add_batch: the pending pre-ranked insert was ranked for other rows "
+                               f"(n {pre[0]}, all active, its strata tensor); got n {n}")
         if self._row_ws is None or self._row_ws.numel() < n:
             self._row_ws = torch.empty((n,), dtype=torch.int32, device=self.device)
 
@@ -118,6 +124,11 @@
         if active is not None:
             act = active.view(torch.uint8) if active.dtype == torch.bool else active.to(torch.uint8)
             act = act.contiguous()
+        if pre is not None:
+            nat.check(nat.lib().lap_store_rows(ctypes.byref(self._store), nat.ptr(st), nat.ptr(ac), nat.ptr(nx),
+                                               nat.ptr(rw), nat.ptr(dn), float(self.normalize_actions), n,
+                                               nat.ptr(self._row_pre[pre[2]]), self._stream()), "lap_store_rows")
+            return
         nat.check(nat.lib().lap_store_batch(ctypes.byref(self._desc), ctypes.byref(self._store), nat.ptr(st),
                                             nat.ptr(ac), nat.ptr(nx), nat.ptr(rw), nat.ptr(dn), nat.ptr(sr.contiguous()),
                                             nat.ptr(act), float(self.normalize_actions), n, nat.ptr(self._row_ws),
@@ -288,8 +299,50 @@
 
     fuse_update_sample = os.environ.get("EXO_LAP_FUSED", "1") != "0"
 
-    def update_priority_and_sample(self, priority, ind=None, slot=None, before_gather=None):
+    def store_rank(self, strata, row_of, active=None):
+        act = None
+        if active is not None:
+            act = (active.view(torch.uint8) if active.dtype == torch.bool else active.to(torch.uint8)).contiguous()
+        nat.check(nat.lib().lap_store_rank(ctypes.byref(self._desc), ctypes.byref(self._store), nat.ptr(strata),
+                                           nat.ptr(act), strata.numel(), nat.ptr(row_of), self._stream()),
+                  "lap_store_rank")
+
+    def prerank_buffers(self, n):
+        if self._row_pre is None or self._row_pre[0].numel() < n:
+            self._row_pre = [torch.empty((n,), dtype=torch.int32, device=self.device) for _ in range(2)]
+        return self._row_pre
+
+    def _prerank_args(self, prerank):
+        strata, n, parity = prerank
+        if self.prerank_pending is not None:
+            raise RuntimeError("LAP: a pre-ranked insert is already pending (its add_batch has not run)")
+        if strata.dtype != torch.int32 or not strata.is_contiguous() or strata.numel() != n:
+            raise ValueError("LAP: prerank needs a contiguous int32 strata tensor of n rows")
+        if not (self.device_rng and self.fuse_update_sample and self.batch_size <= 1024):
+            raise RuntimeError("LAP: prerank needs the device RNG and the fused update + sample")
+        rows = self.prerank_buffers(n)[int(parity) & 1]
+        self.prerank_pending = (int(n), strata.data_ptr(), int(parity) & 1)
+        return nat.ptr(strata), None, int(n), nat.ptr(rows)
+
+    def update_priority_and_sample(self, priority, ind=None, slot=None, before_gather=None, prerank=None):
         ind = self.ind if ind is None else ind
+        if prerank is not None:
+            pr = priority.detach().to(torch.float32).reshape(-1).contiguous()
+            assert pr.numel() == ind.numel()
+            batch, idx = self._slot(slot)
+            r = self._rng
+            rk = self._prerank_args(prerank)
+            nat.check(nat.lib().lap_update_sample_idx_rank(
+                ctypes.byref(self._desc), ctypes.byref(self._store), nat.ptr(ind), nat.ptr(pr), None, 0.0, 0.0, None,
+                ind.shape[1], r.seed, r.tag, r.counter_ptr, r.ticket_ptr, nat.ptr(idx), *rk, self._stream()),
+                "lap_update_sample_idx_rank")
+            if before_gather is not None:
+                before_gather()
+            nat.check(nat.lib().lap_gather_rows(ctypes.byref(self._desc), ctypes.byref(self._store), ind.shape[1],
+                                                nat.ptr(idx), *[nat.ptr(t) for t in batch], self._stream()),
+                      "lap_gather_rows")
+            self.ind = idx
+            return batch
         if not (self.device_rng and self.fuse_update_sample and self.batch_size <= 1024):
             self.update_priority(priority, ind)
             if before_gather is not None:
@@ -317,11 +370,22 @@
         self.ind = idx
         return batch
 
-    def update_priority_and_sample_td(self, td, alpha, min_priority, ind, slot, prio_out=None):
+    def update_priority_and_sample_td(self, td, alpha, min_priority, ind, slot, prio_out=None, prerank=None):
         if not (self.device_rng and self.batch_size <= 1024):
             raise RuntimeError("update_priority_and_sample_td: the device RNG and batch <= 1024 only")
         batch, idx = self._slot(slot)
         r = self._rng
+        if prerank is not None:
+            rk = self._prerank_args(prerank)
+            nat.check(nat.lib().lap_update_sample_idx_rank(
+                ctypes.byref(self._desc), ctypes.byref(self._store), nat.ptr(ind), None, nat.ptr(td), float(alpha),
+                float(min_priority), nat.ptr(prio_out), ind.shape[1], r.seed, r.tag, r.counter_ptr, r.ticket_ptr,
+                nat.ptr(idx), *rk, self._stream()), "lap_update_sample_idx_rank")
+            nat.check(nat.lib().lap_gather_rows(ctypes.byref(self._desc), ctypes.byref(self._store), ind.shape[1],
+                                                nat.ptr(idx), *[nat.ptr(t) for t in batch], self._stream()),
+                      "lap_gather_rows")
+            self.ind = idx
+            return batch
         nat.check(nat.lib().lap_update_sample_td(ctypes.byref(self._desc), ctypes.byref(self._store), nat.ptr(ind),
                                                  nat.ptr(td), float(alpha), float(min_priority), nat.ptr(prio_out),
                                                  ind.shape[1], r.seed, r.tag, r.counter_ptr, r.ticket_ptr,
@@ -335,6 +399,7 @@
 
     def reset_buffer(self):
         self.ptr = self.count = self.size = 0
+        self.prerank_pending = None
         for t in (self.state, self.action, self.next_state, self.reward, self.not_done):
             t.zero_()
         self.ptr_s.zero_()
diff --git a/a-deep-reinforcement-learning-enabled-soft-exoskeleton-for-parkinson-s-patients_amd/exo_amd/rollout.py b/a-deep-reinforcement-learning-enabled-soft-exoskeleton-for-parkinson-s-patients_amd/exo_amd/rollout.py
--- a/a-deep-reinforcement-learning-enabled-soft-exoskeleton-for-parkinson-s-patients_amd/exo_amd/rollout.py
+++ b/a-deep-reinforcement-learning-enabled-soft-exoskeleton-for-parkinson-s-patients_amd/exo_amd/rollout.py
@@ -222,6 +222,8 @@
             self.pink = PinkNoise.for_learner(agent.learner.fused, Ls)
             self._pink_stepped = torch.ones(self.n, dtype=torch.bool, device=self.device)
             self._pink_done = torch.zeros(self.n, dtype=torch.bool, device=self.device)
+        if self._prerank_ok():
+            agent.replay_buffer.prerank_buffers(self.n)
         if use_graphs and os.environ.get("EXO_GRAPH_CHECK", "1") != "0":
             graph_reductions_ok(self.device)
 
@@ -261,8 +263,8 @@
             self._select_done.record(torch.cuda.current_stream(self.device))
         nobs, rew, done, info = self.env.step(act, active=self.active, out=self._outs[self._cur],
                                               obs_cur=obs if self.budget else None)
-        ag.replay_buffer.add_batch(obs, act, nobs, rew, done, self.strata, self.active)
-        if self._early_on:
+        ag.replay_buffer.add_batch(obs, act, nobs, rew, done, self.strata, None if self._rk_in else self.active)
+        if self._early_on and not self._rk_in:
             self._ins_ev = torch.cuda.Event()
             self._ins_ev.record(torch.cuda.current_stream(self.device))
         if self.pink is None:
@@ -446,6 +448,21 @@
         rb = self.agent.replay_buffer
         return (EARLY_LAP and not self.dp and self._prefetching() and not self._us_after_critic()
                 and not self._pre_out and rb.device_rng and rb.fuse_update_sample and rb.batch_size <= 1024)
+
+    lap_prerank = os.environ.get("EXO_LAP_PRERANK", "auto")
+    _rk_in = _rk_out = _rk_next = False
+
+    def _prerank_ok(self):
+        return (self.lap_prerank == "1" and not isinstance(self, RefScheduleTrainer)
+                and self.episodes == "async" and not self.budget and not self.prefetch_targets
+                and self._early_lap())
+
+    def _rank_out(self, training_steps, steps_after):
+        return (self._prerank_ok() and self.iters > 0
+                and training_steps % self.agent.learner.hp.target_update_rate != 0 and steps_after >= 1)
+
+    def _set_pending(self, on, parity):
+        self.agent.replay_buffer.prerank_pending = (self.n, self.strata.data_ptr(), parity & 1) if on else None
 
     def _join_rollout(self):
         if self._br_pending is not None:
@@ -509,12 +526,15 @@
         if not self._mid_rollout and self._train_pout:
             rb.update_priority_and_sample(self._prio, self._ind, 1 - self._bslot)
         elif self._prefetching() and self._mid_rollout:
-            if self._br_pending is not None and self._ins_ev is not None:
-                torch.cuda.current_stream(self.device).wait_event(self._ins_ev)
-                rb.update_priority_and_sample(self._prio, self._ind, 1 - self._cur, before_gather=self._join_rollout)
+            pre = (self.strata, self.n, 1 - self._cur) if self._rk_out else None
+            if self._br_pending is not None and (self._rk_in or self._ins_ev is not None):
+                if not self._rk_in:
+                    torch.cuda.current_stream(self.device).wait_event(self._ins_ev)
+                rb.update_priority_and_sample(self._prio, self._ind, 1 - self._cur, before_gather=self._join_rollout,
+                                              prerank=pre)
             else:
                 self._join_rollout()
-                rb.update_priority_and_sample(self._prio, self._ind, 1 - self._cur)
+                rb.update_priority_and_sample(self._prio, self._ind, 1 - self._cur, prerank=pre)
             if self._pre_out:
                 b = rb._slot(1 - self._cur)[0]
                 self.agent.learner.prefetch_targets(b[0], b[1], b[2], 1 - self._cur)
@@ -591,7 +611,8 @@
 
     def _key(self, update_actor, rollout):
         if rollout:
-            return update_actor, self._cur, self._pre_in, self._pre_out
+            rk = ("rk", self._rk_in, self._rk_out) if self._rk_in or self._rk_out else ()
+            return (update_actor, self._cur, self._pre_in, self._pre_out) + rk
         if self._train_pin or self._train_pout:
             return "train", update_actor, self._train_pin, self._train_pout, self._bslot
         return "train", update_actor
@@ -604,6 +625,15 @@
         self._replay(update_actor, rollout)
 
     def _capture_graph(self, update_actor, rollout=True):
+        rb = self.agent.replay_buffer
+        pending = rb.prerank_pending
+        self._set_pending(rollout and self._rk_in, self._cur)
+        try:
+            self._capture_graph_parts(update_actor, rollout)
+        finally:
+            rb.prerank_pending = pending
+
+    def _capture_graph_parts(self, update_actor, rollout):
         s = torch.cuda.Stream(device=self.device)
         s.wait_stream(torch.cuda.current_stream(self.device))
         pool = None
@@ -676,8 +706,11 @@
                 and L.training_steps % L.hp.target_update_rate != 0
                 and (self.episodes == "async" or self.k + 1 < self.round_len))
 
+    _pair_rk = (False, False, False)
+
     def _pair_key(self, ua, ua2, overlap=False):
-        return ("pair", ua, ua2, self._cur) + (("overlap",) if overlap else ())
+        rk = (("rk",) + tuple(self._pair_rk)) if any(self._pair_rk) else ()
+        return ("pair", ua, ua2, self._cur) + (("overlap",) if overlap else ()) + rk
 
     def _run_pair(self, ua, ua2, overlap=False):
         g = self.graphs.get(self._pair_key(ua, ua2, overlap))
@@ -692,6 +725,7 @@
         s.wait_stream(torch.cuda.current_stream(self.device))
         g = new_graph()
         cur0 = self._cur
+        rk, rk_saved = self._pair_rk, (self._rk_in, self._rk_out, self.agent.replay_buffer.prerank_pending)
         keep = []
         if overlap and getattr(self, "_astream", None) is None:
             self._astream = torch.cuda.Stream(device=self.device)
@@ -702,6 +736,8 @@
                 with capture(g, stream=s), ForkJoinAudit(s):
                     for i, u in enumerate((ua, ua2)):
                         L.prefetch_actor = u
+                        self._rk_in, self._rk_out = rk[i], rk[i + 1]
+                        self._set_pending(self._rk_in, self._cur)
                         if overlap and i == 0:
                             self._actor_stream = self._astream
                         if overlap and i == 1:
@@ -725,6 +761,7 @@
         finally:
             self._actor_stream = self._overlap_wait = None
             L.before_critic_step = None
+            self._rk_in, self._rk_out, self.agent.replay_buffer.prerank_pending = rk_saved
         torch.cuda.current_stream(self.device).wait_stream(s)
         self._cur = cur0
         self.iters -= 1
@@ -753,9 +790,12 @@
             return 0
         pf = L.hp.policy_freq
         saved = (L.training_steps, L.prefetch_actor, self._pre_in, self._pre_out, self._cur, self.iters, self.k)
+        saved_rk = (self._rk_in, self._rk_out, self._pair_rk)
         made = 0
         try:
             self._pre_in = self._pre_out = False
+            self._rk_in = self._rk_out = False
+            self._pair_rk = (False, False, False)
             for _ in range(2):
                 L.training_steps += 1
                 ua = L.training_steps % pf == 0
@@ -766,6 +806,8 @@
                 self._cur ^= 1
                 self.iters += 1
             L.training_steps, self._cur, self.iters = saved[0], saved[4], saved[5]
+            if self._prerank_ok() and self._horizon is not None:
+                return made + self._prepare_walk()
             L.training_steps += 1
             ua, ua2 = L.training_steps % pf == 0, (L.training_steps + 1) % pf == 0
             if self._horizon is not None and self._horizon >= 2 and self._pair_ok():
@@ -777,7 +819,50 @@
         finally:
             (L.training_steps, L.prefetch_actor, self._pre_in, self._pre_out, self._cur, self.iters,
              self.k) = saved
+            self._rk_in, self._rk_out, self._pair_rk = saved_rk
         return made
+
+    def _prepare_walk(self, limit=100_000):
+        L = self.agent.learner
+        pf = L.hp.policy_freq
+        h, rk_next, made = self._horizon, self._rk_next, 0
+        for _ in range(limit):
+            if h <= 0:
+                break
+            L.training_steps += 1
+            ua = L.training_steps % pf == 0
+            L.prefetch_actor = ua
+            self._rk_in, self._rk_out = rk_next, self._rank_out(L.training_steps, h - 1)
+            self._rk_in = self._rk_in or self._rk_out
+            if self._pair_now(ua, h):
+                ua2 = (L.training_steps + 1) % pf == 0
+                overlap = self.overlap_pairs and ua and not ua2 and L.fused_train
+                self._pair_rk = (self._rk_in, self._rk_out, self._rank_out(L.training_steps + 1, h - 2))
+                if self._pair_key(ua, ua2, overlap) not in self.graphs:
+                    self._capture_pair(ua, ua2, overlap)
+                    made += 1
+                rk_next = self._pair_rk[2]
+                L.training_steps += 1
+                self.iters += 2
+                h -= 2
+            else:
+                if self._key(ua, True) not in self.graphs:
+                    self._capture_graph(ua)
+                    made += 1
+                rk_next = self._rk_out
+                self._cur ^= 1
+                self.iters += 1
+                h -= 1
+        return made
+
+    def _pair_now(self, update_actor, horizon):
+        L = self.agent.learner
+
+        def single(*base):
+            return any(k[:4] == base for k in self.graphs)
+        return (horizon is not None and horizon >= 2 and self._pair_ok()
+                and single(update_actor, self._cur, self._pre_in, self._pre_out)
+                and single((L.training_steps + 1) % L.hp.policy_freq == 0, 1 - self._cur, False, False))
 
     def step(self):
         ag = self.agent
@@ -799,18 +884,31 @@
         update_actor = L.training_steps % ag.hp.policy_freq == 0
         L.prefetch_actor = update_actor
         self._pre_in, self._pre_out = self._target_prefetch_flags()
+        after = -1 if horizon is None else horizon - 1
+        self._rk_in = self._rk_next
+        self._rk_out = self._rank_out(L.training_steps, after)
+        if self._rk_out and not self._rk_in and self.use_graphs and self.iters >= self.warmup_eager:
+            rb = ag.replay_buffer
+            rb.store_rank(self.strata, rb.prerank_buffers(self.n)[self._cur])
+            self._rk_in = True
+        self._set_pending(self._rk_in, self._cur)
         if not self.use_graphs or self.iters < self.warmup_eager:
             self._eager(update_actor)
-        elif (horizon is not None and horizon >= 2 and self._pair_ok() and self._key(update_actor, True) in self.graphs
-              and ((L.training_steps + 1) % ag.hp.policy_freq == 0, 1 - self._cur, False, False) in self.graphs):
+        elif self._pair_now(update_actor, horizon):
             ua2 = (L.training_steps + 1) % ag.hp.policy_freq == 0
+            self._pair_rk = (self._rk_in, self._rk_out, self._rank_out(L.training_steps + 1, after - 1))
             self._run_pair(update_actor, ua2,
                            overlap=self.overlap_pairs and update_actor and not ua2 and L.fused_train)
             self._pair_second = True
+            self._rk_out = self._pair_rk[2]
+            self._set_pending(self._rk_out, self._cur)
         elif self._key(update_actor, True) not in self.graphs:
             self._capture(update_actor)
         else:
             self._replay(update_actor)
+        if not self._pair_second:
+            self._set_pending(self._rk_out, 1 - self._cur)
+        self._rk_next = self._rk_out
         if self._pre_in or self._pre_out:
             if not isinstance(L._pre_ready, list):
                 L._pre_ready = [False, False]
diff --git a/include/exo_amd.h b/include/exo_amd.h
--- a/include/exo_amd.h
+++ b/include/exo_amd.h
@@ -153,6 +153,12 @@
                     const uint8_t *done_dev, const int32_t *strata_dev, const uint8_t *active_dev, float action_scale,
                     int32_t n, int32_t *row_ws_dev, void *stream);
 
+int lap_store_rank(const lap_tree_desc *t, const lap_storage_desc *st, const int32_t *strata_dev,
+                   const uint8_t *active_dev, int32_t n, int32_t *row_of_dev, void *stream);
+int lap_store_rows(const lap_storage_desc *st, const float *state_dev, const float *action_dev,
+                   const float *next_state_dev, const float *reward_dev, const uint8_t *done_dev, float action_scale,
+                   int32_t n, const int32_t *row_of_dev, void *stream);
+
 int lap_store_batch_ref(const lap_tree_desc *t, const lap_storage_desc *st, int64_t *ref_dev,
                         const float *state_dev, const float *action_dev, const float *next_state_dev,
                         const float *reward_dev, const uint8_t *done_dev, const int32_t *strata_dev,
@@ -196,6 +202,11 @@
 int lap_gather_rows(const lap_tree_desc *t, const lap_storage_desc *st, int32_t batch, const int32_t *idx,
                     float *out_state, float *out_action, float *out_next_state, float *out_reward,
                     float *out_not_done, void *stream);
+int lap_update_sample_idx_rank(const lap_tree_desc *t, const lap_storage_desc *st, const int32_t *idx_in,
+                               const float *prio, const float *td, float alpha, float min_priority, float *prio_out,
+                               int32_t batch, uint64_t seed, uint32_t tag, unsigned long long *counter,
+                               uint32_t *ticket, int32_t *idx_out, const int32_t *strata_dev,
+                               const uint8_t *active_dev, int32_t n, int32_t *row_of_next_dev, void *stream);
 int lap_update_sample_td(const lap_tree_desc *t, const lap_storage_desc *st, const int32_t *idx_in, const float *td,
                          float alpha, float min_priority, float *prio_out, int32_t batch, uint64_t seed, uint32_t tag,
                          unsigned long long *counter, uint32_t *ticket, int32_t *idx_out, float *out_state,
```

New measurement: 18.65 million (median of 6 runs). Within noise of the previous version (+0.6%).
